# PKU-Alignment/omnisafe

Measured on AMD Instinct MI355X. Metric: env-steps/sec (rollout+update), PPO-Lag SafetyPointGoal1, higher is better.
Workload: dtype f32

## Files before the change

### include/omnisafe_amd.h

```cpp
#ifndef OMNISAFE_AMD_H
#define OMNISAFE_AMD_H

#include <stddef.h>
#include <stdint.h>

#ifdef __cplusplus
extern "C" {
#endif

#define OSA_OK 0
#define OSA_EINVAL (-1)
#define OSA_EHIP (-2)
#define OSA_EUNSUPPORTED (-3)

#define OSA_EST_GAE 0
#define OSA_EST_GAE_RTG 1
#define OSA_EST_PLAIN 2
#define OSA_EST_VTRACE 3

const char* osa_strerror(int code);
int osa_version(void);
const char* osa_build_arch(void);
const char* osa_abi_digest(void);


int osa_buffer_store_step(int t, int N, int obs_dim, int act_dim,
                          const float* obs, int ld_obs_src, const float* act, int ld_act_src,
                          const float* reward, const float* cost, const float* value_r,
                          const float* value_c, const float* logp,
                          float* buf_obs, int ld_obs_buf, float* buf_act, int ld_act_buf,
                          float* buf_reward, float* buf_cost, float* buf_value_r, float* buf_value_c,
                          float* buf_logp, void* stream);

int osa_gae_scan(const float* reward, const float* cost, const float* value_r, const float* value_c,
                 const uint8_t* path_end, const float* boot_r, const float* boot_c, int T, int N,
                 double gamma, double lam, double lam_c, float penalty_coef, int estimator,
                 float* adv_r, float* adv_c, float* target_value_r, float* target_value_c,
                 float* discounted_ret, void* stream);

int osa_gae_scan_tiled(const float* reward, const float* cost, const float* value_r, const float* value_c,
                       const uint8_t* path_end, const float* boot_r, const float* boot_c, int T, int N,
                       double gamma, double lam, double lam_c, float penalty_coef, int estimator,
                       float* adv_r, float* adv_c, float* target_value_r, float* target_value_c,
                       float* discounted_ret, void* stream);
size_t osa_gae_chained_ws_doubles(int T, int N);
int osa_gae_chained_timed_out(const double* ws, int T, int N, int* out);
int osa_gae_scan_chained(const float* reward, const float* cost, const float* value_r, const float* value_c,
                         const uint8_t* path_end, const float* boot_r, const float* boot_c, int T, int N,
                         double gamma, double lam, double lam_c, float penalty_coef, int estimator,
                         float* adv_r, float* adv_c, float* target_value_r, float* target_value_c,
                         float* discounted_ret, double* ws, void* stream);

size_t osa_reduce_ws_bytes(void);
int osa_adv_stats_phase1(const float* adv_r, const float* adv_c, long M, double* ws, double* stats,
                         void* stream);
int osa_adv_stats_phase2(const float* adv_r, long M, double* ws, double* stats, void* stream);

int osa_buffer_get(int T, int N, int obs_dim, int act_dim,
                   const float* obs, int ld_obs, const float* act, int ld_act, const float* logp,
                   const float* target_value_r, const float* target_value_c, const float* adv_r,
                   const float* adv_c, const float* discounted_ret, double* stats,
                   int standardize_r, int standardize_c,
                   float* out_obs, int ld_out_obs, float* out_act, int ld_out_act, float* out_logp,
                   float* out_target_value_r, float* out_target_value_c, float* out_adv_r,
                   float* out_adv_c, float* out_discounted_ret, void* stream);


int osa_mlp_layout(int obs_dim, int act_dim, int hidden, int* out12);

int osa_policy_step(int obs_dim, int act_dim, int hidden, const float* params, const float* obs,
                    int ld_obs, int N, const float* eps, unsigned long long seed,
                    unsigned long long offset, const unsigned long long* offset_base, int deterministic,
                    int nets_mask, float* act, int ld_act, float* value_r, float* value_c, float* logp,
                    float* mean_out, int ld_mean, void* stream);

int osa_policy_step_scaled(int obs_dim, int act_dim, int hidden, const float* params, const float* obs,
                           int ld_obs, int N, const float* eps, unsigned long long seed,
                           unsigned long long offset, const unsigned long long* offset_base, int deterministic,
                           int nets_mask, float* act, int ld_act, float* value_r, float* value_c, float* logp,
                           float* mean_out, int ld_mean, float* act_env, int ld_env, const float* old_min,
                           const float* old_max, float min_action, float max_action, void* stream);

typedef struct osa_ppo_hparams {
  float clip;
  float entropy_coef;
  float critic_norm_coef;
  float max_grad_norm;
  float lr_actor;
  float lr_critic;
  float beta1, beta2, adam_eps;
  int use_critic_norm;
  int use_max_grad_norm;
  int use_cost;
  const float* lr_device;
} osa_ppo_hparams;

size_t osa_minibatch_ws_floats(int obs_dim, int act_dim, int hidden, int max_blocks);
int osa_ppo_minibatch(int obs_dim, int act_dim, int hidden, float* params, float* adam_m,
                      float* adam_v, int* adam_step, float* grads, const float* obs, int ld_obs,
                      const float* act, int ld_act, const float* logp, const float* target_value_r,
                      const float* target_value_c, const float* adv_r, const float* adv_c,
                      const long* idx, int B, const float* lagrange, const osa_ppo_hparams* hp,
                      int loss_kind, int mode, int nets_mask, int max_blocks, float* ws,
                      float* step_stats, void* stream);

typedef struct osa_surrogate_ext {
  const float* old_mean;
  int ld_old_mean;
  const float* old_log_std;
  float kl_coef;
  float kl_mask_eta;
  float ratio_scale;
  float cost_kappa;
  float cost_excess;
} osa_surrogate_ext;
int osa_ppo_minibatch_ext(int obs_dim, int act_dim, int hidden, float* params, float* adam_m,
                          float* adam_v, int* adam_step, float* grads, const float* obs, int ld_obs,
                          const float* act, int ld_act, const float* logp,
                          const float* target_value_r, const float* target_value_c,
                          const float* adv_r, const float* adv_c, const long* idx, int B,
                          const float* lagrange, const osa_ppo_hparams* hp, int loss_kind, int mode,
                          int nets_mask, int max_blocks, float* ws, float* step_stats,
                          const osa_surrogate_ext* ext, void* stream);

int osa_ppo_pass_supported(int obs_dim, int act_dim, int hidden);
int osa_ppo_pass(int obs_dim, int act_dim, int hidden, float* params, float* adam_m, float* adam_v,
                 int* adam_step, const float* obs, int ld_obs, const float* act, int ld_act,
                 const float* logp, const float* target_value_r, const float* target_value_c,
                 const float* adv_r, const float* adv_c, const long* perm, long M, int B,
                 const float* lagrange, const osa_ppo_hparams* hp, int loss_kind, int nets_mask,
                 float* step_stats, void* stream);
int osa_ppo_wide_pass_supported(int obs_dim, int act_dim, int hidden);
size_t osa_ppo_wide_pass_ws_floats(int obs_dim, int act_dim, int hidden);
int osa_ppo_wide_pass(int obs_dim, int act_dim, int hidden, float* params, float* adam_m, float* adam_v,
                      int* adam_step, const float* obs, int ld_obs, const float* act, int ld_act,
                      const float* logp, const float* target_value_r, const float* target_value_c,
                      const float* adv_r, const float* adv_c, const long* perm, long M, int B,
                      const float* lagrange, const osa_ppo_hparams* hp, int loss_kind, int nets_mask,
                      float* ws, float* step_stats, void* stream);
int osa_ppo_split_pass_supported(int obs_dim, int act_dim, int hidden);
size_t osa_ppo_split_pass_xch_floats(int obs_dim, int act_dim, int hidden);
int osa_ppo_split_pass(int obs_dim, int act_dim, int hidden, float* params, float* adam_m, float* adam_v,
                       int* adam_step, const float* obs, int ld_obs, const float* act, int ld_act,
                       const float* logp, const float* target_value_r, const float* target_value_c,
                       const float* adv_r, const float* adv_c, const long* perm, long M, int B,
                       const float* lagrange, const osa_ppo_hparams* hp, int loss_kind, int nets_mask,
                       float* xch, int local, float* step_stats, void* stream);
int osa_ppo_split_pass_timed_out(const float* xch, int* out);
int osa_ppo_split_pass_clear_flag(float* xch);
size_t osa_ppo_split_dp_xch_floats(int obs_dim, int act_dim, int hidden, int world);
size_t osa_ppo_split_dp_dpx_floats(int obs_dim, int act_dim, int hidden, int world);
int osa_ppo_split_dp_pass(int obs_dim, int act_dim, int hidden, float* params, float* adam_m, float* adam_v,
                          int* adam_step, const float* obs, int ld_obs, const float* act, int ld_act,
                          const float* logp, const float* target_value_r, const float* target_value_c,
                          const float* adv_r, const float* adv_c, const long* perm, long M, int B, int world,
                          const float* lagrange, const osa_ppo_hparams* hp, int loss_kind, int nets_mask,
                          float* xch, float* dpx, int place, float* step_stats, void* stream);
int osa_ppo_pass_ext(int obs_dim, int act_dim, int hidden, float* params, float* adam_m, float* adam_v,
                 int* adam_step, const float* obs, int ld_obs, const float* act, int ld_act,
                 const float* logp, const float* target_value_r, const float* target_value_c,
                 const float* adv_r, const float* adv_c, const long* perm, long M, int B,
                 const float* lagrange, const osa_ppo_hparams* hp, int loss_kind, int nets_mask,
                 float* step_stats, const osa_surrogate_ext* ext, void* stream);
typedef struct osa_pass_member {
  float* params;
  float* adam_m;
  float* adam_v;
  int* adam_step;
  const float* obs;
  int ld_obs;
  const float* act;
  int ld_act;
  const float* logp;
  const float* target_value_r;
  const float* target_value_c;
  const float* adv_r;
  const float* adv_c;
  const long* perm;
  long M;
  int B;
  const float* lagrange;
  osa_ppo_hparams hp;
  int loss_kind;
  int nets_mask;
  float* step_stats;
  int has_ext;
  osa_surrogate_ext ext;
} osa_pass_member;
size_t osa_ppo_pass_group_ws_bytes(int n);
int osa_ppo_pass_group(int obs_dim, int act_dim, int hidden, const osa_pass_member* members, int n, void* workspace,
                       size_t workspace_bytes, void* stream);

size_t osa_ppo_dp_ws_floats(int obs_dim, int act_dim, int hidden, int world);
int osa_ppo_dp_step(int obs_dim, int act_dim, int hidden, float* params, float* adam_m, float* adam_v,
                    int* adam_step, const float* obs, int ld_obs, const float* act, int ld_act,
                    const float* logp, const float* target_value_r, const float* target_value_c,
                    const float* adv_r, const float* adv_c, const long* perm, long M, int B, int world,
                    int step_index, const float* lagrange, const osa_ppo_hparams* hp,
                    const float* lr_dev, int loss_kind, int nets_mask, float* slabs,
                    float* step_stats, void* stream);
int osa_ppo_dp_end_pass(int* adam_step, int nets_mask, int nsteps, void* stream);
int osa_ppo_dp_step_phase(int obs_dim, int act_dim, int hidden, float* params, float* adam_m, float* adam_v,
                          int* adam_step, const float* obs, int ld_obs, const float* act, int ld_act,
                          const float* logp, const float* target_value_r, const float* target_value_c,
                          const float* adv_r, const float* adv_c, const long* perm, long M, int B, int world,
                          int step_index, const float* lagrange, const osa_ppo_hparams* hp,
                          const float* lr_dev, int loss_kind, int nets_mask, float* slabs,
                          float* step_stats, int phase, void* stream);

int osa_dp_exchange_alloc(size_t floats, float** out);
int osa_dp_exchange_free(float* p);
size_t osa_ppo_dp_pass_ws_floats(int obs_dim, int act_dim, int hidden, int world);
int osa_ppo_dp_pass(int obs_dim, int act_dim, int hidden, float* params, float* adam_m, float* adam_v,
                    int* adam_step, const float* obs, int ld_obs, const float* act, int ld_act,
                    const float* logp, const float* target_value_r, const float* target_value_c,
                    const float* adv_r, const float* adv_c, const long* perm, long M, int B, int world,
                    const float* lagrange, const osa_ppo_hparams* hp, int loss_kind, int nets_mask,
                    float* exchange, int* sync, float* step_stats, void* stream);
int osa_ppo_dp_pass_placed(int obs_dim, int act_dim, int hidden, float* params, float* adam_m, float* adam_v,
                    int* adam_step, const float* obs, int ld_obs, const float* act, int ld_act,
                    const float* logp, const float* target_value_r, const float* target_value_c,
                    const float* adv_r, const float* adv_c, const long* perm, long M, int B, int world,
                    const float* lagrange, const osa_ppo_hparams* hp, int loss_kind, int nets_mask,
                    float* exchange, int* sync, int local, float* step_stats, void* stream);

size_t osa_p2p_exchange_floats(int obs_dim, int act_dim, int hidden, int world);
int osa_p2p_exchange_alloc(size_t floats, float** out, void* ipc_handle64);
int osa_p2p_exchange_open(const void* ipc_handle64, float** out);
int osa_p2p_exchange_release(float* p);
int osa_p2p_exchange_timed_out(const float* own, int* flag);
int osa_ppo_p2p_pass(int obs_dim, int act_dim, int hidden, float* params, float* adam_m, float* adam_v,
                     int* adam_step, const float* obs, int ld_obs, const float* act, int ld_act,
                     const float* logp, const float* target_value_r, const float* target_value_c,
                     const float* adv_r, const float* adv_c, const long* perm, long M, int B, int world, int rank,
                     float* const* peers, unsigned seq0, double timeout_s, const float* lagrange,
                     const osa_ppo_hparams* hp, int loss_kind, int nets_mask, float* step_stats, void* stream);

int osa_ppo_chunked_pass(int obs_dim, int act_dim, int hidden, float* params, float* adam_m, float* adam_v,
                         int* adam_step, const float* obs, int ld_obs, const float* act, int ld_act,
                         const float* logp, const float* target_value_r, const float* target_value_c,
                         const float* adv_r, const float* adv_c, const long* perm, long M, int B,
                         const float* lagrange, const osa_ppo_hparams* hp, int loss_kind, int nets_mask,
                         float* exchange, int* sync, int local, float* step_stats, void* stream);
size_t osa_ppo_dp_chunked_pass_ws_floats(int obs_dim, int act_dim, int hidden, int B, int world);
int osa_ppo_dp_chunked_pass(int obs_dim, int act_dim, int hidden, float* params, float* adam_m, float* adam_v,
                            int* adam_step, const float* obs, int ld_obs, const float* act, int ld_act,
                            const float* logp, const float* target_value_r, const float* target_value_c,
                            const float* adv_r, const float* adv_c, const long* perm, long M, int B, int world,
                            const float* lagrange, const osa_ppo_hparams* hp, int loss_kind, int nets_mask,
                            float* exchange, int* sync, int local, float* step_stats, void* stream);

int osa_debug_set_clock_buffer(long long* dev_ptr);
int osa_debug_set_pass_clock_buffer(long long* dev_ptr);
int osa_debug_set_part_clock_buffer(long long* dev_ptr);

#define OSA_GMLP_MAX_LAYERS 8
typedef struct osa_gmlp_desc {
  int obs_dim, act_dim;
  int n_layers[3];
  int width[3][OSA_GMLP_MAX_LAYERS];
  int activation[3];
} osa_gmlp_desc;
int osa_gmlp_layout(const osa_gmlp_desc* desc, int* out);
size_t osa_gmlp_ws_floats(const osa_gmlp_desc* desc, long rows);
int osa_gmlp_policy_step(const osa_gmlp_desc* desc, const float* params, const float* obs, int ld_obs, long N,
                         const float* eps, unsigned long long seed, unsigned long long offset,
                         const unsigned long long* offset_base, int deterministic, int nets_mask, float* act,
                         int ld_act, float* value_r, float* value_c, float* logp, float* mean_out, int ld_mean,
                         float* act_env, int ld_env, const float* old_min, const float* old_max, float min_action,
                         float max_action, float* ws, size_t ws_floats, void* stream);
int osa_gmlp_minibatch(const osa_gmlp_desc* desc, float* params, float* adam_m, float* adam_v, int* adam_step,
                       float* grads, const float* obs, int ld_obs, const float* act, int ld_act, const float* logp,
                       const float* target_value_r, const float* target_value_c, const float* adv_r,
                       const float* adv_c, const long* idx, long B, const float* lagrange, const osa_ppo_hparams* hp,
                       int loss_kind, int mode, int nets_mask, const float* vec, float fvp_scale, float* ws,
                       size_t ws_floats, float* step_stats, void* stream);
int osa_gmlp_minibatch_ext(const osa_gmlp_desc* desc, float* params, float* adam_m, float* adam_v, int* adam_step,
                           float* grads, const float* obs, int ld_obs, const float* act, int ld_act, const float* logp,
                           const float* target_value_r, const float* target_value_c, const float* adv_r,
                           const float* adv_c, const long* idx, long B, const float* lagrange,
                           const osa_ppo_hparams* hp, int loss_kind, int mode, int nets_mask, const float* vec,
                           float fvp_scale, float* ws, size_t ws_floats, float* step_stats,
                           const osa_surrogate_ext* ext, void* stream);
int osa_gmlp_adam_apply(const osa_gmlp_desc* desc, float* params, float* adam_m, float* adam_v, int* adam_step,
                        float* grads, const osa_ppo_hparams* hp, int nets_mask, float* fin8x3, void* stream);
int osa_gmlp_actor_stats(const osa_gmlp_desc* desc, const float* actor_params, const float* obs, int ld_obs, long M,
                         const float* old_mean, int ld_old, const float* old_log_std, int kind, int reduce_mode,
                         const float* act, int ld_act, const float* logp, const float* adv_r, const float* adv_c,
                         const float* lagrange, float* mean_out, int ld_mean, float* ws, size_t ws_floats, float* out,
                         void* stream);

int osa_adam_apply(int obs_dim, int act_dim, int hidden, float* params, float* adam_m, float* adam_v,
                   int* adam_step, float* grads, const osa_ppo_hparams* hp, int nets_mask,
                   void* stream);

int osa_actor_kl(int obs_dim, int act_dim, int hidden, const float* actor_params, const float* obs,
                 int ld_obs, long M, const float* old_mean, int ld_old, const float* old_log_std,
                 int reduce_mode, float* mean_out, int ld_mean, double* ws, float* kl_out,
                 void* stream);


size_t osa_normalizer_ws_doubles(int N, int D);
int osa_normalizer_push(const float* x, int ld, int N, int D, const uint8_t* mask, float* mean,
                        float* sumsq, float* var, float* std_, long* count, double* ws,
                        void* stream);

int osa_normalizer_apply(const float* x, int ld_x, float* y, int ld_y, int N, int D,
                         const uint8_t* mask, const float* mean, const float* std_, const long* count,
                         float clip, void* stream);

int osa_action_scale(const float* act, int ld_act, float* out, int ld_out, int N, int act_dim,
                     const float* old_min, const float* old_max, float min_action, float max_action,
                     void* stream);

int osa_rollout_post_step(int N, int epoch_end, const float* reward, const float* cost,
                          const uint8_t* terminated, const uint8_t* truncated, const float* vnext_r,
// ... 80 lines not shown
```

### omnisafe_amd/_lib.py

```python
from __future__ import annotations

import ctypes as C
import os

import torch

from . import build as _build

_LIB = None
OSA_OK, OSA_EUNSUPPORTED = 0, -3

c_f32p = C.c_void_p
c_ptr = C.c_void_p

_I, _L, _F, _D, _P, _U = C.c_int, C.c_long, C.c_float, C.c_double, C.c_void_p, C.c_ulonglong
SIGNATURES: dict[str, tuple] = {
    'osa_strerror': (C.c_char_p, [_I]),
    'osa_version': (_I, []),
    'osa_build_arch': (C.c_char_p, []),
    'osa_abi_digest': (C.c_char_p, []),
    'osa_buffer_store_step': (_I, [_I, _I, _I, _I, _P, _I, _P, _I, _P, _P, _P, _P, _P, _P, _I, _P, _I,
                                   _P, _P, _P, _P, _P, _P]),
    'osa_gae_scan': (_I, [_P, _P, _P, _P, _P, _P, _P, _I, _I, _D, _D, _D, _F, _I, _P, _P, _P, _P, _P, _P]),
    'osa_gae_scan_tiled': (_I, [_P, _P, _P, _P, _P, _P, _P, _I, _I, _D, _D, _D, _F, _I, _P, _P, _P, _P, _P, _P]),
    'osa_gae_chained_ws_doubles': (C.c_size_t, [_I, _I]),
    'osa_gae_chained_timed_out': (_I, [_P, _I, _I, _P]),
    'osa_gae_scan_chained': (_I, [_P, _P, _P, _P, _P, _P, _P, _I, _I, _D, _D, _D, _F, _I, _P, _P, _P, _P, _P, _P, _P]),
    'osa_reduce_ws_bytes': (C.c_size_t, []),
    'osa_adv_stats_phase1': (_I, [_P, _P, _L, _P, _P, _P]),
    'osa_adv_stats_phase2': (_I, [_P, _L, _P, _P, _P]),
    'osa_buffer_get': (_I, [_I, _I, _I, _I, _P, _I, _P, _I, _P, _P, _P, _P, _P, _P, _P, _I, _I,
                            _P, _I, _P, _I, _P, _P, _P, _P, _P, _P, _P]),
    'osa_mlp_layout': (_I, [_I, _I, _I, _P]),
    'osa_policy_step': (_I, [_I, _I, _I, _P, _P, _I, _I, _P, _U, _U, _P, _I, _I, _P, _I, _P, _P, _P, _P, _I,
                             _P]),
    'osa_policy_step_scaled': (_I, [_I, _I, _I, _P, _P, _I, _I, _P, _U, _U, _P, _I, _I, _P, _I, _P, _P, _P, _P, _I,
                                    _P, _I, _P, _P, _F, _F, _P]),
    'osa_minibatch_ws_floats': (C.c_size_t, [_I, _I, _I, _I]),
    'osa_gmlp_layout': (_I, [_P, _P]),
    'osa_gmlp_ws_floats': (C.c_size_t, [_P, _L]),
    'osa_gmlp_policy_step': (_I, [_P, _P, _P, _I, _L, _P, _U, _U, _P, _I, _I, _P, _I, _P, _P, _P, _P, _I, _P, _I, _P,
                                  _P, _F, _F, _P, C.c_size_t, _P]),
    'osa_gmlp_minibatch': (_I, [_P, _P, _P, _P, _P, _P, _P, _I, _P, _I, _P, _P, _P, _P, _P, _P, _L, _P, _P, _I, _I,
                                _I, _P, _F, _P, C.c_size_t, _P, _P]),
    'osa_gmlp_minibatch_ext': (_I, [_P, _P, _P, _P, _P, _P, _P, _I, _P, _I, _P, _P, _P, _P, _P, _P, _L, _P, _P, _I, _I,
                                    _I, _P, _F, _P, C.c_size_t, _P, _P, _P]),
    'osa_gmlp_adam_apply': (_I, [_P, _P, _P, _P, _P, _P, _P, _I, _P, _P]),
    'osa_gmlp_actor_stats': (_I, [_P, _P, _P, _I, _L, _P, _I, _P, _I, _I, _P, _I, _P, _P, _P, _P, _P, _I, _P,
                                  C.c_size_t, _P, _P]),
    'osa_ppo_minibatch': (_I, [_I, _I, _I, _P, _P, _P, _P, _P, _P, _I, _P, _I, _P, _P, _P, _P, _P, _P,
                               _I, _P, _P, _I, _I, _I, _I, _P, _P, _P]),
    'osa_ppo_minibatch_ext': (_I, [_I, _I, _I, _P, _P, _P, _P, _P, _P, _I, _P, _I, _P, _P, _P, _P, _P, _P,
                                   _I, _P, _P, _I, _I, _I, _I, _P, _P, _P, _P]),
    'osa_episode_flush_ws_doubles': (C.c_size_t, [_L]),
    'osa_episode_flush': (_I, [_P, _P, _P, _P, _P, _L, _P, _P, _P, _P, _P, _P, _P, _P]),
    'osa_gather_mean': (_I, [_P, _P, _L, _P, _P]),
    'osa_saute_step': (_I, [_I, _P, _P, _P, _P, _P, _P, _F, _F, _P, _P, _P, _I, _P, _I, _I, _P, _P, _P]),
    'osa_debug_set_clock_buffer': (_I, [_P]),
    'osa_debug_set_pass_clock_buffer': (_I, [_P]),
    'osa_debug_set_part_clock_buffer': (_I, [_P]),
    'osa_ppo_pass_supported': (_I, [_I, _I, _I]),
    'osa_ppo_dp_end_pass': (_I, [_P, _I, _I, _P]),
    'osa_ppo_dp_ws_floats': (C.c_size_t, [_I, _I, _I, _I]),
    'osa_ppo_dp_pass_ws_floats': (C.c_size_t, [_I, _I, _I, _I]),
    'osa_shuffle_rows': (_I, [_P, _I, _L, _P, _P]),
    'osa_dp_exchange_alloc': (_I, [C.c_size_t, C.POINTER(C.c_void_p)]),
    'osa_dp_exchange_free': (_I, [_P]),
    'osa_ppo_dp_pass': (_I, [_I, _I, _I, _P, _P, _P, _P, _P, _I, _P, _I, _P, _P, _P, _P, _P, _P, _L, _I, _I,
                        _P, _P, _I, _I, _P, _P, _P, _P]),
    'osa_ppo_dp_pass_placed': (_I, [_I, _I, _I, _P, _P, _P, _P, _P, _I, _P, _I, _P, _P, _P, _P, _P, _P, _L, _I, _I,
                               _P, _P, _I, _I, _P, _P, _I, _P, _P]),
    'osa_ppo_chunked_pass': (_I, [_I, _I, _I, _P, _P, _P, _P, _P, _I, _P, _I, _P, _P, _P, _P, _P, _P, _L, _I,
                                  _P, _P, _I, _I, _P, _P, _I, _P, _P]),
    'osa_ppo_dp_chunked_pass_ws_floats': (C.c_size_t, [_I, _I, _I, _I, _I]),
    'osa_ppo_dp_chunked_pass': (_I, [_I, _I, _I, _P, _P, _P, _P, _P, _I, _P, _I, _P, _P, _P, _P, _P, _P, _L, _I, _I,
                                     _P, _P, _I, _I, _P, _P, _I, _P, _P]),
    'osa_p2p_exchange_floats': (C.c_size_t, [_I, _I, _I, _I]),
    'osa_p2p_exchange_alloc': (_I, [C.c_size_t, C.POINTER(C.c_void_p), _P]),
    'osa_p2p_exchange_open': (_I, [_P, C.POINTER(C.c_void_p)]),
    'osa_p2p_exchange_release': (_I, [_P]),
    'osa_p2p_exchange_timed_out': (_I, [_P, _P]),
    'osa_ppo_p2p_pass': (_I, [_I, _I, _I, _P, _P, _P, _P, _P, _I, _P, _I, _P, _P, _P, _P, _P, _P, _L, _I, _I, _I,
                              _P, C.c_uint, _D, _P, _P, _I, _I, _P, _P]),
    'osa_ppo_dp_step': (_I, [_I, _I, _I, _P, _P, _P, _P, _P, _I, _P, _I, _P, _P, _P, _P, _P, _P, _L, _I, _I,
                             _I, _P, _P, _P, _I, _I, _P, _P, _P]),
    'osa_ppo_dp_step_phase': (_I, [_I, _I, _I, _P, _P, _P, _P, _P, _I, _P, _I, _P, _P, _P, _P, _P, _P, _L, _I, _I, _I, _P, _P, _P, _I, _I, _P, _P, _I, _P]),
    'osa_ppo_pass': (_I, [_I, _I, _I, _P, _P, _P, _P, _P, _I, _P, _I, _P, _P, _P, _P, _P, _P, _L, _I,
                          _P, _P, _I, _I, _P, _P]),
    'osa_ppo_wide_pass_supported': (_I, [_I, _I, _I]),
    'osa_ppo_wide_pass_ws_floats': (C.c_size_t, [_I, _I, _I]),
    'osa_ppo_wide_pass': (_I, [_I, _I, _I, _P, _P, _P, _P, _P, _I, _P, _I, _P, _P, _P, _P, _P, _P, _L, _I,
                               _P, _P, _I, _I, _P, _P, _P]),
    'osa_ppo_split_pass_supported': (_I, [_I, _I, _I]),
    'osa_ppo_split_pass_xch_floats': (C.c_size_t, [_I, _I, _I]),
    'osa_ppo_split_pass': (_I, [_I, _I, _I, _P, _P, _P, _P, _P, _I, _P, _I, _P, _P, _P, _P, _P, _P, _L, _I,
                                _P, _P, _I, _I, _P, _I, _P, _P]),
    'osa_ppo_split_pass_timed_out': (_I, [_P, _P]),
    'osa_ppo_split_pass_clear_flag': (_I, [_P]),
    'osa_ppo_split_dp_xch_floats': (C.c_size_t, [_I, _I, _I, _I]),
    'osa_ppo_split_dp_dpx_floats': (C.c_size_t, [_I, _I, _I, _I]),
    'osa_ppo_split_dp_pass': (_I, [_I, _I, _I, _P, _P, _P, _P, _P, _I, _P, _I, _P, _P, _P, _P, _P, _P, _L, _I, _I,
                                   _P, _P, _I, _I, _P, _P, _I, _P, _P]),
    'osa_ppo_pass_ext': (_I, [_I, _I, _I, _P, _P, _P, _P, _P, _I, _P, _I, _P, _P, _P, _P, _P, _P, _L, _I,
                              _P, _P, _I, _I, _P, _P, _P]),
    'osa_ppo_pass_group_ws_bytes': (C.c_size_t, [_I]),
    'osa_ppo_pass_group': (_I, [_I, _I, _I, _P, _I, _P, C.c_size_t, _P]),
    'osa_adam_apply': (_I, [_I, _I, _I, _P, _P, _P, _P, _P, _P, _I, _P]),
    'osa_actor_fvp_raw': (_I, [_I, _I, _I, _P, _P, _P, _I, _L, _P, _I, _P, _P, _P]),
    'osa_fvp_finish': (_I, [_I, _P, _P, _F, _I, _I, _F, _P, _P]),
    'osa_cg_init': (_I, [_I, _P, _P, _P, _P, _P, _P]),
    'osa_cg_step': (_I, [_I, _P, _P, _P, _P, _P, _F, _F, _P]),
    'osa_vec_lincomb': (_I, [_I, _F, _P, _F, _P, _P, _P]),
    'osa_vec_dot': (_I, [_I, _P, _P, _P, _P]),
    'osa_actor_eval': (_I, [_I, _I, _I, _P, _P, _I, _L, _P, _I, _P, _P, _P, _P, _P, _I, _P, _P, _P, _P]),
    'osa_actor_kl': (_I, [_I, _I, _I, _P, _P, _I, _L, _P, _I, _P, _I, _P, _I, _P, _P, _P]),
    'osa_normalizer_ws_doubles': (C.c_size_t, [_I, _I]),
    'osa_normalizer_push': (_I, [_P, _I, _I, _I, _P, _P, _P, _P, _P, _P, _P, _P]),
    'osa_normalizer_apply': (_I, [_P, _I, _P, _I, _I, _I, _P, _P, _P, _P, _F, _P]),
    'osa_action_scale': (_I, [_P, _I, _P, _I, _I, _I, _P, _P, _F, _F, _P]),
    'osa_rollout_post_step': (_I, [_I, _I] + [_P] * 21),
    'osa_synth_env_step': (_I, [_U, _U, _P, _I, _I, _I, _F, _P, _P, _I, _P, _P, _P, _P, _P, _I, _I, _P]),
    'osa_reach_env_step': (_I, [_U, _U, _P, _I, _I, _I, _P, _P, _P, _I, _P, _I, _P, _P, _P, _P, _P, _I, _I, _P]),
    'osa_nav_env_step': (_I, [_U, _U, _P, _I, _I, _I, _I, _P, _P, _P, _I, _P, _I, _P, _P, _P, _P, _P, _I, _I, _P]),
    'osa_eval_episodes': (_I, [_I, _I, _I, _I, _I, _P, _P, _P, _P, _F, _P, _P, _F, _F, _U, _I, _F, _I, _I, _F, _F,
                               _I, _D, _D, _P, _P, _P, _P, _P]),
    'osa_eval_trace_floats': (_I, [_I, _I, _I, _I]),
}


class OsaError(RuntimeError):
    pass


def lib_path() -> str:
    return os.environ.get('OSA_LIB_PATH') or _build.LIB_PATH


def load(require_gpu: bool = False):
    global _LIB
    if _LIB is None:
        path = lib_path()
        own = path == _build.LIB_PATH

        def build(force: bool) -> None:
            try:
                _build.build_library(force=force, verbose=False)
            except Exception as exc:
                raise OsaError(
                    f'libomnisafe_amd.so is missing or stale and could not be built ({exc}); '
                    'run `python -m omnisafe_amd.build` -- there is no CPU fallback') from exc

        def digest(lib) -> str:
            try:
                lib.osa_abi_digest.restype = C.c_char_p
                return lib.osa_abi_digest().decode()
            except AttributeError:
                return 'none'

        if own and not os.path.exists(path):
            build(False)
        lib = C.CDLL(path)
        if own:
            want = _build.source_digest()
            if digest(lib) != want:
                import _ctypes

                _ctypes.dlclose(lib._handle)
                build(True)
                lib = C.CDLL(path)
                if digest(lib) != want:
                    raise OsaError(f'{path} was built from other sources (digest {digest(lib)}, expected '
                                   f'{want}); run `python -m omnisafe_amd.build --force`')
        for name, (res, args) in SIGNATURES.items():
            fn = getattr(lib, name)
            fn.restype = res
            fn.argtypes = args
        _LIB = lib
    if require_gpu and not torch.cuda.is_available():
        raise OsaError('omnisafe_amd needs an AMD GPU visible to torch (ROCm); there is no CPU fallback')
    return _LIB


def check(code: int, what: str = '') -> None:
    if code != 0:
        msg = load().osa_strerror(code).decode()
        raise OsaError(f'{what or "libomnisafe_amd"} failed: {msg} ({code})')


def ptr(t: torch.Tensor | None) -> int | None:
    if t is None:
        return None
    assert t.is_cuda, 'omnisafe_amd kernels take device tensors'
    return t.data_ptr()


_RAW_STREAM = getattr(torch._C, '_cuda_getCurrentRawStream', None)


def stream_ptr() -> int:
    if _RAW_STREAM is not None:
        return _RAW_STREAM(torch.cuda.current_device())
    return torch.cuda.current_stream().cuda_stream
```

### omnisafe_amd/csrc/buffer_kernels.hip

```cpp
#include "osa_common.h"

__global__ __launch_bounds__(256) void osa_store_step_kernel(
    int N, int obs_dim, int act_dim, const float* __restrict__ obs, int ld_os,
    const float* __restrict__ act, int ld_as, const float* __restrict__ reward,
    const float* __restrict__ cost, const float* __restrict__ value_r,
    const float* __restrict__ value_c, const float* __restrict__ logp, float* __restrict__ b_obs,
    int ld_ob, float* __restrict__ b_act, int ld_ab, float* __restrict__ b_reward,
    float* __restrict__ b_cost, float* __restrict__ b_value_r, float* __restrict__ b_value_c,
    float* __restrict__ b_logp) {
  const long gid = (long)blockIdx.x * blockDim.x + threadIdx.x;
  const long n_obs = (long)N * obs_dim, n_act = (long)N * act_dim;
  if (gid < n_obs) {
    const int n = (int)(gid / obs_dim), d = (int)(gid % obs_dim);
    b_obs[(long)n * ld_ob + d] = obs[(long)n * ld_os + d];
  }
  if (gid < n_act) {
    const int n = (int)(gid / act_dim), d = (int)(gid % act_dim);
    b_act[(long)n * ld_ab + d] = act[(long)n * ld_as + d];
  }
  if (gid < N) {
    b_reward[gid] = reward[gid];
    b_cost[gid] = cost[gid];
    b_value_r[gid] = value_r[gid];
    b_value_c[gid] = value_c[gid];
// ... 598 lines not shown
  __shared__ double red[17];
  double sa = 0.0, sb = 0.0;
  const long stride = (long)gridDim.x * blockDim.x;
  for (long i = (long)blockIdx.x * blockDim.x + threadIdx.x; i < M; i += stride) {
    sa += (double)a[i];
    sb += (double)b[i];
  }
  sa = osa_block_sum<OSA_RED_THREADS>(sa, red);
  sb = osa_block_sum<OSA_RED_THREADS>(sb, red);
  if (threadIdx.x == 0) {
    ws[2 * blockIdx.x] = sa;
    ws[2 * blockIdx.x + 1] = sb;
  }
}

__global__ __launch_bounds__(OSA_RED_THREADS) void osa_sum2_final_kernel(
    const double* __restrict__ ws, int nblk, long M, double* __restrict__ stats) {
  __shared__ double red[17];
  double sa = 0.0, sb = 0.0;
  for (int i = threadIdx.x; i < nblk; i += OSA_RED_THREADS) {
    sa += ws[2 * i];
    sb += ws[2 * i + 1];
  }
  sa = osa_block_sum<OSA_RED_THREADS>(sa, red);
  sb = osa_block_sum<OSA_RED_THREADS>(sb, red);
  if (threadIdx.x == 0) {
    stats[0] = sa;
    stats[1] = sb;
    stats[2] = (double)M;
  }
}

__global__ __launch_bounds__(OSA_RED_THREADS) void osa_sumsq_partial_kernel(
    const float* __restrict__ a, long M, const double* __restrict__ stats,
    double* __restrict__ ws) {
#pragma clang fp contract(off)
  __shared__ double red[17];
  const float mean = (float)stats[0] / (float)stats[2];
  double s = 0.0;
  const long stride = (long)gridDim.x * blockDim.x;
  for (long i = (long)blockIdx.x * blockDim.x + threadIdx.x; i < M; i += stride) {
    const float d = a[i] - mean;
    const float q = d * d;
    s += (double)q;
  }
  s = osa_block_sum<OSA_RED_THREADS>(s, red);
  if (threadIdx.x == 0) ws[blockIdx.x] = s;
}

__global__ __launch_bounds__(OSA_RED_THREADS) void osa_sumsq_final_kernel(
    const double* __restrict__ ws, int nblk, double* __restrict__ stats) {
  __shared__ double red[17];
  double s = 0.0;
  for (int i = threadIdx.x; i < nblk; i += OSA_RED_THREADS) s += ws[i];
  s = osa_block_sum<OSA_RED_THREADS>(s, red);
  if (threadIdx.x == 0) {
    stats[3] = s;
    stats[4] = (double)((float)stats[0] / (float)stats[2]);
    stats[5] = (double)((float)stats[1] / (float)stats[2]);
  }
}

struct OsaGetScalars {
  const float* src[6];
  float* dst[6];
  int op[6];
};

__global__ __launch_bounds__(256) void osa_get_scalars_kernel(OsaGetScalars p, int T, int N,
                                                              double* __restrict__ stats) {
#pragma clang fp contract(off)
  __shared__ float tile[64][65];
  const int n0 = blockIdx.x * 64, t0 = blockIdx.y * 64;
  const int tx = threadIdx.x & 63, ty = threadIdx.x >> 6;
  const float mean_r = (float)stats[4], mean_c = (float)stats[5];
  const float std_r = sqrtf((float)stats[3] / (float)stats[2]);
  if (blockIdx.x == 0 && blockIdx.y == 0 && threadIdx.x == 0) stats[6] = (double)std_r;
  const float denom = std_r + 1e-8f;
  float pre[6][16];
#pragma unroll
  for (int k = 0; k < 6; ++k) {
    const bool have = p.src[k] != nullptr && p.dst[k] != nullptr;
    const float* __restrict__ src = have ? p.src[k] : reinterpret_cast<const float*>(stats);
#pragma unroll
    for (int u = 0; u < 16; ++u) {
      const int t = t0 + ty + 4 * u, n = n0 + tx;
      const bool ok = have && t < T && n < N;
      pre[k][u] = src[ok ? (long)t * N + n : 0];
    }
  }
#pragma unroll
  for (int k = 0; k < 6; ++k) {
    const float* __restrict__ src = p.src[k];
    float* __restrict__ dst = p.dst[k];
    if (src == nullptr || dst == nullptr) continue;
    const int op = p.op[k];
    __syncthreads();
#pragma unroll
    for (int u = 0; u < 16; ++u) {
      const int tt = ty + 4 * u;
      const int t = t0 + tt, n = n0 + tx;
      if (t < T && n < N) {
        float v = pre[k][u];
        if (op == 1) v = (v - mean_r) / denom;
        else if (op == 2) v = v - mean_c;
        tile[tt][tx] = v;
      }
    }
    __syncthreads();
    for (int nn = ty; nn < 64; nn += 4) {
      const int n = n0 + nn, t = t0 + tx;
      if (t < T && n < N) dst[(long)n * T + t] = tile[tx][nn];
    }
  }
}

__global__ __launch_bounds__(256) void osa_get_rows_kernel(const float* __restrict__ src, int ld_src,
                                                           float* __restrict__ dst, int ld_dst,
                                                           int T, int N, int dim) {
  const long gid = (long)blockIdx.x * blockDim.x + threadIdx.x;
  const long total = (long)T * N * dim;
  if (gid >= total) return;
  const long row = gid / dim;
  const int d = (int)(gid - row * dim);
  const int n = (int)(row / T), t = (int)(row - (long)n * T);
  dst[row * ld_dst + d] = src[((long)t * N + n) * ld_src + d];
}

__global__ __launch_bounds__(256) void osa_get_rows_vec4_kernel(const float* __restrict__ src, int ld_src,
                                                                float* __restrict__ dst, int ld_dst,
                                                                unsigned T, unsigned N, unsigned dim4,
                                                                unsigned total4) {
  const unsigned gid = blockIdx.x * 256u + threadIdx.x;
  if (gid >= total4) return;
  const unsigned row = gid / dim4, q = gid - row * dim4;
  const unsigned n = row / T, t = row - n * T;
  const float4 v = *reinterpret_cast<const float4*>(src + ((size_t)t * N + n) * ld_src + 4 * q);
  *reinterpret_cast<float4*>(dst + (size_t)row * ld_dst + 4 * q) = v;
}

static void osa_launch_get_rows(const float* src, int ld_src, float* dst, int ld_dst, int T, int N, int dim,
                                hipStream_t st) {
  const long total = (long)T * N * dim;
  const bool vec = dim % 4 == 0 && ld_src % 4 == 0 && ld_dst % 4 == 0 && total / 4 < 2147483647L &&
                   (reinterpret_cast<uintptr_t>(src) & 15) == 0 && (reinterpret_cast<uintptr_t>(dst) & 15) == 0;
  if (vec) {
    const unsigned total4 = (unsigned)(total / 4);
    hipLaunchKernelGGL(osa_get_rows_vec4_kernel, dim3((total4 + 255) / 256), dim3(256), 0, st, src, ld_src, dst,
                       ld_dst, (unsigned)T, (unsigned)N, (unsigned)(dim / 4), total4);
  } else {
    hipLaunchKernelGGL(osa_get_rows_kernel, dim3((unsigned)((total + 255) / 256)), dim3(256), 0, st, src, ld_src,
                       dst, ld_dst, T, N, dim);
  }
}

extern "C" {

const char* osa_strerror(int code) {
  switch (code) {
    case OSA_OK: return "ok";
    case OSA_EINVAL: return "invalid argument";
    case OSA_EHIP: return "HIP runtime error";
    case OSA_EUNSUPPORTED: return "not implemented in libomnisafe_amd";
    default: return "unknown error";
  }
}
int osa_version(void) { return 1; }
const char* osa_build_arch(void) { return "gfx950"; }

int osa_buffer_store_step(int t, int N, int obs_dim, int act_dim, const float* obs, int ld_obs_src,
                          const float* act, int ld_act_src, const float* reward, const float* cost,
                          const float* value_r, const float* value_c, const float* logp,
                          float* buf_obs, int ld_obs_buf, float* buf_act, int ld_act_buf,
                          float* buf_reward, float* buf_cost, float* buf_value_r, float* buf_value_c,
                          float* buf_logp, void* stream) {
  OSA_REQUIRE(t >= 0 && N > 0 && obs_dim > 0 && act_dim > 0);
  OSA_REQUIRE(obs && act && reward && cost && value_r && value_c && logp);
  OSA_REQUIRE(buf_obs && buf_act && buf_reward && buf_cost && buf_value_r && buf_value_c && buf_logp);
  OSA_REQUIRE(ld_obs_src >= obs_dim && ld_obs_buf >= obs_dim && ld_act_src >= act_dim &&
              ld_act_buf >= act_dim);
  const long row = (long)t * N;
  const long work = (long)N * (obs_dim > act_dim ? obs_dim : act_dim);
  const int blocks = (int)((work + 255) / 256);
  hipLaunchKernelGGL(osa_store_step_kernel, dim3(blocks), dim3(256), 0, osa_stream(stream), N,
                     obs_dim, act_dim, obs, ld_obs_src, act, ld_act_src, reward, cost, value_r,
                     value_c, logp, buf_obs + row * ld_obs_buf, ld_obs_buf,
                     buf_act + row * ld_act_buf, ld_act_buf, buf_reward + row, buf_cost + row,
                     buf_value_r + row, buf_value_c + row, buf_logp + row);
  OSA_CHECK_LAUNCH();
  return OSA_OK;
}

int osa_gae_scan(const float* reward, const float* cost, const float* value_r, const float* value_c,
                 const uint8_t* path_end, const float* boot_r, const float* boot_c, int T, int N,
                 double gamma, double lam, double lam_c, float penalty_coef, int estimator,
                 float* adv_r, float* adv_c, float* target_value_r, float* target_value_c,
                 float* discounted_ret, void* stream) {
  OSA_REQUIRE(T > 0 && N > 0);
  OSA_REQUIRE(reward && cost && value_r && value_c && path_end && boot_r && boot_c);
  OSA_REQUIRE(adv_r && adv_c && target_value_r && target_value_c && discounted_ret);
  if (estimator < OSA_EST_GAE || estimator > OSA_EST_VTRACE) return OSA_EUNSUPPORTED;
  const float g32 = (float)gamma;
  const double d_g = gamma, d_r = gamma * lam, d_c = gamma * lam_c;
  const int threads = N >= 256 ? 256 : 64;
  const int blocks = (N + threads - 1) / threads;
  constexpr int U = 8;
#define OSA_GAE_LAUNCH(E)                                                                         \
  hipLaunchKernelGGL((osa_gae_scan_kernel<E, U>), dim3(blocks), dim3(threads), 0,                 \
                     osa_stream(stream), reward, cost, value_r, value_c, path_end, boot_r, boot_c, \
                     T, N, g32, d_g, d_r, d_c, penalty_coef, adv_r, adv_c, target_value_r,        \
                     target_value_c, discounted_ret)
  if (estimator == OSA_EST_GAE) OSA_GAE_LAUNCH(OSA_EST_GAE);
  else if (estimator == OSA_EST_GAE_RTG) OSA_GAE_LAUNCH(OSA_EST_GAE_RTG);
  else if (estimator == OSA_EST_PLAIN) OSA_GAE_LAUNCH(OSA_EST_PLAIN);
  else OSA_GAE_LAUNCH(OSA_EST_VTRACE);
#undef OSA_GAE_LAUNCH
  OSA_CHECK_LAUNCH();
  return OSA_OK;
}

int osa_gae_scan_tiled(const float* reward, const float* cost, const float* value_r, const float* value_c,
                       const uint8_t* path_end, const float* boot_r, const float* boot_c, int T, int N,
                       double gamma, double lam, double lam_c, float penalty_coef, int estimator,
                       float* adv_r, float* adv_c, float* target_value_r, float* target_value_c,
                       float* discounted_ret, void* stream) {
  OSA_REQUIRE(T > 0 && N > 0);
  OSA_REQUIRE(reward && cost && value_r && value_c && path_end && boot_r && boot_c);
  OSA_REQUIRE(adv_r && adv_c && target_value_r && target_value_c && discounted_ret);
  if (estimator < OSA_EST_GAE || estimator > OSA_EST_PLAIN) return OSA_EUNSUPPORTED;
  const float g32 = (float)gamma;
  const double d_g = gamma, d_r = gamma * lam, d_c = gamma * lam_c;
  constexpr int NB = 16;
  const int blocks = (N + NB - 1) / NB;
  int cus = 256, dev = 0;
  if (hipGetDevice(&dev) == hipSuccess) (void)hipDeviceGetAttribute(&cus, hipDeviceAttributeMultiprocessorCount, dev);
  bool wide_wg = blocks <= 2 * cus;
  if (const char* e = getenv("OSA_GAE_TILE_WAVES")) wide_wg = e[0] == '1';
#define OSA_GAE_TILE_LAUNCH(E)                                                                            \
  do {                                                                                                    \
    if (wide_wg)                                                                                          \
      hipLaunchKernelGGL((osa_gae_tile_scan_kernel<E, NB, 16>), dim3(blocks), dim3(1024), 0,              \
                         osa_stream(stream), reward, cost, value_r, value_c, path_end, boot_r, boot_c, T, \
                         N, g32, d_g, d_r, d_c, penalty_coef, adv_r, adv_c, target_value_r,               \
                         target_value_c, discounted_ret);                                                 \
    else                                                                                                  \
      hipLaunchKernelGGL((osa_gae_tile_scan_kernel<E, NB, 4>), dim3(blocks), dim3(256), 0,                \
                         osa_stream(stream), reward, cost, value_r, value_c, path_end, boot_r, boot_c, T, \
                         N, g32, d_g, d_r, d_c, penalty_coef, adv_r, adv_c, target_value_r,               \
                         target_value_c, discounted_ret);                                                 \
  } while (0)
  if (estimator == OSA_EST_GAE) OSA_GAE_TILE_LAUNCH(OSA_EST_GAE);
  else if (estimator == OSA_EST_GAE_RTG) OSA_GAE_TILE_LAUNCH(OSA_EST_GAE_RTG);
  else OSA_GAE_TILE_LAUNCH(OSA_EST_PLAIN);
#undef OSA_GAE_TILE_LAUNCH
  OSA_CHECK_LAUNCH();
  return OSA_OK;
}

size_t osa_gae_chained_ws_doubles(int T, int N) {
  if (T < 1 || N < 1) return 0;
  return (size_t)((T + OSA_GC_LEV - 1) / OSA_GC_LEV) * 10 * (size_t)N + 2;
}

int osa_gae_chained_timed_out(const double* ws, int T, int N, int* out) {
  OSA_REQUIRE(ws && out && T > 0 && N > 0);
  const size_t nws = osa_gae_chained_ws_doubles(T, N);
  return hipMemcpy(out, ws + (nws - 1), sizeof(int), hipMemcpyDeviceToHost) == hipSuccess ? OSA_OK : OSA_EHIP;
}

int osa_gae_scan_chained(const float* reward, const float* cost, const float* value_r, const float* value_c,
                         const uint8_t* path_end, const float* boot_r, const float* boot_c, int T, int N,
                         double gamma, double lam, double lam_c, float penalty_coef, int estimator,
                         float* adv_r, float* adv_c, float* target_value_r, float* target_value_c,
                         float* discounted_ret, double* ws, void* stream) {
  OSA_REQUIRE(T > 0 && N > 0 && ws);
  OSA_REQUIRE(reward && cost && value_r && value_c && path_end && boot_r && boot_c);
  OSA_REQUIRE(adv_r && adv_c && target_value_r && target_value_c && discounted_ret);
  if (estimator < OSA_EST_GAE || estimator > OSA_EST_PLAIN) return OSA_EUNSUPPORTED;
  const float g32 = (float)gamma;
  const double d_g = gamma, d_r = gamma * lam, d_c = gamma * lam_c;
  const int nlev = (T + OSA_GC_LEV - 1) / OSA_GC_LEV, nenvb = (N + 63) / 64;
  if ((long)nlev * nenvb > 2147483647L) return OSA_EUNSUPPORTED;
  hipStream_t st = osa_stream(stream);
  const size_t nws = osa_gae_chained_ws_doubles(T, N);
  if (hipMemsetAsync(ws, 0xFF, (nws - 2) * sizeof(double), st) != hipSuccess) return OSA_EHIP;
  unsigned int* ticket = reinterpret_cast<unsigned int*>(ws + (nws - 2));
  if (hipMemsetAsync(ticket, 0, sizeof(double), st) != hipSuccess) return OSA_EHIP;
#define OSA_GAE_CHAIN_LAUNCH(E)                                                                             \
  hipLaunchKernelGGL((osa_gae_chain_scan_kernel<E>), dim3(nlev * nenvb), dim3(64 * OSA_GC_NW), 0, st, reward, \
                     cost, value_r, value_c, path_end, boot_r, boot_c, T, N, g32, d_g, d_r, d_c, penalty_coef, \
                     adv_r, adv_c, target_value_r, target_value_c, discounted_ret, ws, nenvb, ticket)
  if (estimator == OSA_EST_GAE) OSA_GAE_CHAIN_LAUNCH(OSA_EST_GAE);
  else if (estimator == OSA_EST_GAE_RTG) OSA_GAE_CHAIN_LAUNCH(OSA_EST_GAE_RTG);
  else OSA_GAE_CHAIN_LAUNCH(OSA_EST_PLAIN);
#undef OSA_GAE_CHAIN_LAUNCH
  OSA_CHECK_LAUNCH();
  return OSA_OK;
}

size_t osa_reduce_ws_bytes(void) { return (size_t)OSA_RED_BLOCKS * 2 * sizeof(double); }

static int osa_red_blocks(long M) {
  long b = (M + (long)OSA_RED_THREADS * 4 - 1) / ((long)OSA_RED_THREADS * 4);
  if (b < 1) b = 1;
  if (b > OSA_RED_BLOCKS) b = OSA_RED_BLOCKS;
  return (int)b;
}

int osa_adv_stats_phase1(const float* adv_r, const float* adv_c, long M, double* ws, double* stats,
                         void* stream) {
  OSA_REQUIRE(adv_r && adv_c && ws && stats && M > 0);
  const int nblk = osa_red_blocks(M);
  hipLaunchKernelGGL(osa_sum2_partial_kernel, dim3(nblk), dim3(OSA_RED_THREADS), 0,
                     osa_stream(stream), adv_r, adv_c, M, ws);
  hipLaunchKernelGGL(osa_sum2_final_kernel, dim3(1), dim3(OSA_RED_THREADS), 0, osa_stream(stream),
                     ws, nblk, M, stats);
  OSA_CHECK_LAUNCH();
  return OSA_OK;
}

int osa_adv_stats_phase2(const float* adv_r, long M, double* ws, double* stats, void* stream) {
  OSA_REQUIRE(adv_r && ws && stats && M > 0);
  const int nblk = osa_red_blocks(M);
  hipLaunchKernelGGL(osa_sumsq_partial_kernel, dim3(nblk), dim3(OSA_RED_THREADS), 0,
                     osa_stream(stream), adv_r, M, stats, ws);
  hipLaunchKernelGGL(osa_sumsq_final_kernel, dim3(1), dim3(OSA_RED_THREADS), 0, osa_stream(stream),
                     ws, nblk, stats);
  OSA_CHECK_LAUNCH();
  return OSA_OK;
}

int osa_buffer_get(int T, int N, int obs_dim, int act_dim, const float* obs, int ld_obs,
                   const float* act, int ld_act, const float* logp, const float* target_value_r,
                   const float* target_value_c, const float* adv_r, const float* adv_c,
                   const float* discounted_ret, double* stats, int standardize_r, int standardize_c,
                   float* out_obs, int ld_out_obs, float* out_act, int ld_out_act, float* out_logp,
                   float* out_target_value_r, float* out_target_value_c, float* out_adv_r,
                   float* out_adv_c, float* out_discounted_ret, void* stream) {
  OSA_REQUIRE(T > 0 && N > 0 && stats);
  OsaGetScalars p;
  const float* srcs[6] = {logp, target_value_r, target_value_c, adv_r, adv_c, discounted_ret};
  float* dsts[6] = {out_logp, out_target_value_r, out_target_value_c, out_adv_r, out_adv_c,
                    out_discounted_ret};
  const int ops[6] = {0, 0, 0, standardize_r ? 1 : 0, standardize_c ? 2 : 0, 0};
  for (int k = 0; k < 6; ++k) {
    p.src[k] = srcs[k];
    p.dst[k] = dsts[k];
    p.op[k] = ops[k];
  }
  hipLaunchKernelGGL(osa_get_scalars_kernel, dim3((N + 63) / 64, (T + 63) / 64), dim3(256), 0,
                     osa_stream(stream), p, T, N, stats);
  if (obs && out_obs) {
    OSA_REQUIRE(obs_dim > 0 && ld_obs >= obs_dim && ld_out_obs >= obs_dim);
    osa_launch_get_rows(obs, ld_obs, out_obs, ld_out_obs, T, N, obs_dim, osa_stream(stream));
  }
  if (act && out_act) {
    OSA_REQUIRE(act_dim > 0 && ld_act >= act_dim && ld_out_act >= act_dim);
    osa_launch_get_rows(act, ld_act, out_act, ld_out_act, T, N, act_dim, osa_stream(stream));
  }
  OSA_CHECK_LAUNCH();
  return OSA_OK;
}

}
```

### omnisafe_amd/csrc/ppo_pass_body.h

```cpp
#pragma once
#include "mlp_device.h"

#ifndef OSA_PART_MARK
#define OSA_PART_MARK(k) do { } while (0)
#endif

#ifndef PSLD
#define PSLD 68
#endif
#define PSPAD (PSLD - 64)
#define PNSTAT 16

struct OsaPassArgs {
  OsaNet nd;
  float* params;
  float* adam_m;
  float* adam_v;
  int* adam_step;
  const float* obs;
  int ld_obs;
  const float* act;
  int ld_act;
  const float* logp;
  const float* tgt_r;
  const float* tgt_c;
  const float* adv_r;
  const float* adv_c;
  const long* perm;
  long M;
  int B;
  int nmb;
  const float* lagrange;
  OsaPassHp hp;
  int loss_kind;
  int nets_mask;
  float* stats;
  float* dp_slabs;
  int dp_world;
  int mb0;
  int* dp_sync;
  int part_stride;
  int part_tpw;
  const float* old_mean;
  int ld_old_mean;
  const float* old_log_std;
  float ext_kl_coef, ext_mask_eta, ext_ratio_scale, ext_cost_kappa, ext_cost_excess;
  int dp_uncached;
  int dp_local;
  int dp_chunk;
  int dp_ranks;
  int one_xcc;
  long long* dbg;
  float* p2p_peer[16];
  int p2p_rank;
  unsigned p2p_seq0;
  long long p2p_timeout;
  int p2p_fence;
};
#define OSA_P2P_HDR 256
#define OSA_P2P_STICKY 240

#ifdef OSA_PASS_CLOCKS
#define PTICK(k)                                      \
  do {                                                \
    if (a.dbg && tid == 0) {                          \
      const long long now_ = clock64();               \
      dbg_acc[k] += now_ - dbg_last;                  \
      dbg_last = now_;                                \
    }                                                 \
  } while (0)
#else
#define PTICK(k) do { } while (0)
#endif

__device__ __forceinline__ f32x4 osa_sym_sum(f32x4 a, float sa, f32x4 b, float sb) {
#pragma clang fp contract(off)
  const f32x4 pa = a * sa;
  const f32x4 pb = b * sb;
  return pa + pb;
}
__device__ __forceinline__ float osa_sym_sum1(float a, float sa, float b, float sb) {
#pragma clang fp contract(off)
  const float pa = a * sa;
  const float pb = b * sb;
  return pa + pb;
}

__device__ __forceinline__ void osa_store_sys(f32x4* p, f32x4 v) {
  asm volatile("global_store_dwordx4 %0, %1, off sc0 sc1" : : "v"(p), "v"(v) : "memory");
}
__device__ __forceinline__ void osa_store_sys(float* p, float v) {
  asm volatile("global_store_dword %0, %1, off sc0 sc1" : : "v"(p), "v"(v) : "memory");
}

__host__ __device__ constexpr int osa_pass_lds_floats(int KB, int OT) {
  return 64 * (16 * KB + PSPAD) + 64 * PSLD + 16 * OT * PSLD + 2 * 64 + 2 * 16 * OT + 4 * 64 * PSLD + 16 * KB * PSLD +
         2 * 16 * OT * PSLD + 64;
}
#ifndef OSA_PASS_W2T
#define OSA_PASS_W2T 1
#endif
__host__ __device__ constexpr bool osa_pass_has_w2t(int KB, int OT) {
  return OSA_PASS_W2T != 0 && (osa_pass_lds_floats(KB, OT) + 64 * PSLD) * 4 <= 160 * 1024;
}

template <int KB, int OT, bool MULTI, bool COOP, bool EXT, bool HIER, bool DPS, bool SO, bool P2P = false>
__device__ __forceinline__ void osa_ppo_pass_body(const OsaPassArgs& a, const int net, const int rk, const int pc0 = 0,
                                                  const int pn = 0) {
  static_assert(!P2P || (COOP && !HIER && !DPS && !EXT), "P2P is a form of the cooperative pass");
  extern __shared__ __attribute__((aligned(16))) float smem[];
  const OsaNet& nd = a.nd;
  constexpr bool coop = COOP;
#ifdef OSA_BODY_PART_ONLY
  constexpr bool dp = true, part = true, contig = true;
#else
  const bool dp = DPS && a.dp_slabs != nullptr && !coop;
  const bool part = DPS && MULTI && a.part_stride != 0;
  const bool contig = part && a.part_stride < 0;
#endif
  const bool chunked = COOP && a.dp_chunk != 0;
  const int nranks = (HIER && chunked && a.dp_ranks > 1) ? a.dp_ranks : 1;
  const int cw = chunked ? a.dp_world / nranks : 1;
  const int crank = chunked ? rk / cw : 0, cchunk = chunked ? rk - crank * cw : 0;
  const long roff = (part || P2P) ? 0 : (chunked ? (long)crank * a.M : (long)rk * a.M);
  const float* __restrict__ obs_p = a.obs + roff * a.ld_obs;
  const float* __restrict__ act_p = a.act + roff * a.ld_act;
  const float* __restrict__ logp_p = a.logp + roff;
  const float* __restrict__ advr_p = a.adv_r + roff;
  const float* __restrict__ advc_p = a.adv_c + roff;
  const long* __restrict__ perm_p = a.perm ? a.perm + roff : nullptr;
  constexpr int H = 64, HT = 4, OUTP = 16 * OT, INP = 16 * KB, W1LD = INP + PSPAD;
  float* sW1 = smem;
  float* sW2 = sW1 + H * W1LD;
  float* sW3 = sW2 + H * PSLD;
  float* sB1 = sW3 + OUTP * PSLD;
  float* sB2 = sB1 + H;
  float* sB3 = sB2 + H;
  float* sLS = sB3 + OUTP;
  float* sH1 = sLS + OUTP;
  float* sH2 = sH1 + H * PSLD;
  float* sZ1 = sH2 + H * PSLD;
  float* sZ2 = sZ1 + H * PSLD;
  float* sX = sZ2 + H * PSLD;
  float* sDO = sX + INP * PSLD;
  float* sDL = sDO + OUTP * PSLD;
  float* red = sDL + OUTP * PSLD;
  constexpr bool W2T = osa_pass_has_w2t(KB, OT);
  float* sW2T = red + 64;

#ifdef OSA_BODY_OPAQUE_TID
  int tid_ = threadIdx.x;
  asm volatile("" : "+v"(tid_));
  const int tid = tid_, lane = tid & 63, wave = tid >> 6, j = lane & 15, g = lane >> 4;
#else
  const int tid = threadIdx.x, lane = tid & 63, wave = tid >> 6, j = lane & 15, g = lane >> 4;
#endif
  const int i = j, cc = j;
  const int nchunk_all = MULTI ? (a.B + 63) / 64 : 1;
  const bool strided = part;
  const int cstride = part ? (contig ? 1 : a.part_stride) : 1;
  const int cfirst = part ? (contig ? pc0 : rk) : (chunked ? cchunk : 0);
  const int nchunk = strided ? (contig ? pn : (nchunk_all - cfirst + cstride - 1) / cstride) : nchunk_all;
  auto pos_ok = [&](long cidx) -> bool {
    const long mb = cidx / nchunk, ch = cfirst + (cidx - mb * nchunk) * cstride;
    const long inb = ch * 64 + 16 * wave + j;
    return (mb < a.mb0 + a.nmb) && (inb < a.B) && (mb * a.B + inb < a.M);
  };
  auto row_of = [&](long cidx) -> long {
    const long mb = cidx / nchunk, ch = cfirst + (cidx - mb * nchunk) * cstride;
    const long pc = pos_ok(cidx) ? mb * a.B + ch * 64 + 16 * wave + j : 0;
    return perm_p ? perm_p[pc] : pc;
  };
  const long cidx_first = (long)a.mb0 * nchunk;
  const long r0_first = row_of(cidx_first);
  const long r1_first = row_of(cidx_first + 1);
  const bool leader = tid == 192;
  const int P = nd.P;
  float* __restrict__ gp = a.params + (long)net * P;
  float* __restrict__ gm = a.adam_m + (long)net * P;
  float* __restrict__ gv = a.adam_v + (long)net * P;
  const bool critic = net != 0;
  const bool is_actor = !critic;
  const int out_dim = critic ? 1 : nd.act_dim;
  const bool small_out = SO || ((OT == 1) && out_dim <= 2);

#ifdef OSA_BODY_PART_ONLY
  constexpr bool VPRO = true;
#else
  constexpr bool VPRO = DPS;
#endif
  f32x4 w1v_[VPRO ? KB : 1], w2v_[VPRO ? 4 : 1], w3v_[VPRO ? OT : 1];
  float b1v_ = 0.f, b2v_ = 0.f, b3v_ = 0.f, lsv_ = 0.f;
  if constexpr (VPRO) {
#pragma unroll
    for (int q = 0; q < KB; ++q) w1v_[q] = *reinterpret_cast<const f32x4*>(gp + nd.oW1 + 4 * (tid + 256 * q));
#pragma unroll
    for (int q = 0; q < 4; ++q) w2v_[q] = *reinterpret_cast<const f32x4*>(gp + nd.oW2 + 4 * (tid + 256 * q));
#pragma unroll
    for (int q = 0; q < OT; ++q) w3v_[q] = *reinterpret_cast<const f32x4*>(gp + nd.oW3 + 4 * (tid + 256 * q));
    if (tid < H) {
      b1v_ = gp[nd.ob1 + tid];
      b2v_ = gp[nd.ob2 + tid];
    }
    if (tid < OUTP) {
      b3v_ = gp[nd.ob3 + tid];
      lsv_ = gp[nd.oLS + tid];
    }
  } else {
    for (int e = tid; e < H * INP; e += 256) sW1[(e / INP) * W1LD + (e % INP)] = gp[nd.oW1 + e];
    if (tid < H) {
      sB1[tid] = gp[nd.ob1 + tid];
      sB2[tid] = gp[nd.ob2 + tid];
    }
    if (tid < OUTP) {
      sB3[tid] = gp[nd.ob3 + tid];
      sLS[tid] = gp[nd.oLS + tid];
    }
  }
  OSA_PART_MARK(8);
  f32x4 m2[HT], v2[HT], m1[KB], v1[KB], m3[OT], v3[OT];
  float mb_ = 0.f, vb_ = 0.f;
  int boff = -1;
  float* sbias = sB1;
  if (tid < H) { boff = nd.ob1 + tid; sbias = sB1 + tid; }
  else if (tid < 2 * H) { boff = nd.ob2 + tid - H; sbias = sB2 + tid - H; }
  else if (tid < 2 * H + OUTP) { boff = nd.ob3 + tid - 2 * H; sbias = sB3 + tid - 2 * H; }
  else if (tid < 2 * H + 2 * OUTP) { boff = nd.oLS + tid - 2 * H - OUTP; sbias = sLS + tid - 2 * H - OUTP; }
  if (critic && boff >= nd.oLS) boff = -1;
#pragma unroll
  for (int ti = 0; ti < HT; ++ti)
#pragma unroll
    for (int r = 0; r < 4; ++r) {
      const int off = nd.oW2 + (16 * wave + 4 * g + r) * H + 16 * ti + cc;
      m2[ti][r] = dp ? 0.f : gm[off];
      v2[ti][r] = dp ? 0.f : gv[off];
    }
#pragma unroll
  for (int kb = 0; kb < KB; ++kb)
#pragma unroll
    for (int r = 0; r < 4; ++r) {
      const int off = nd.oW1 + (16 * wave + 4 * g + r) * INP + 16 * kb + cc;
      m1[kb][r] = dp ? 0.f : gm[off];
      v1[kb][r] = dp ? 0.f : gv[off];
    }
#pragma unroll
  for (int o = 0; o < OT; ++o)
#pragma unroll
    for (int r = 0; r < 4; ++r) {
      const int off = nd.oW3 + (16 * o + 4 * g + r) * H + 16 * wave + cc;
      m3[o][r] = dp ? 0.f : gm[off];
      v3[o][r] = dp ? 0.f : gv[off];
    }
  if (boff >= 0 && !dp) {
    mb_ = gm[boff];
    vb_ = gv[boff];
  }
  OSA_PART_MARK(9);
  const int step0 = dp ? 0 : a.adam_step[net];
  const float lr = critic ? a.hp.lr_critic : a.hp.lr_actor;
  const float beta1 = a.hp.beta1, beta2 = a.hp.beta2, aeps = a.hp.adam_eps;
  if (!dp) {
    for (int k = tid; k < a.nmb; k += 256) {
      const double t = (double)(step0 + k + 1);
      float* row = a.stats + (long)k * PNSTAT;
      row[10 + 2 * net] = (float)((double)lr / (1.0 - pow((double)beta1, t)));
      row[11 + 2 * net] = (float)(1.0 / sqrt(1.0 - pow((double)beta2, t)));
    }
  }
  const bool own_terms = !(chunked && cchunk != 0);
  const bool l2 = critic && a.hp.use_critic_norm && !part && own_terms;
  const float c2 = 2.f * a.hp.critic_norm_coef;
  float lam = 0.f;
  if (is_actor && a.lagrange) lam = *a.lagrange;
  const float inv_1p_lam = 1.f / (1.f + lam);
  constexpr bool vec_ok = true;
  const float* __restrict__ tgt = ((net == 1) ? a.tgt_r : a.tgt_c) + roff;

  struct Pre {
    f32x4 x[KB];
    float act[4 * OT];
    float logp, adv_r, adv_c, tgt;
    float old[EXT ? 4 * OT : 1];
    bool valid;
  };
  auto fetch_x = [&](long rr, Pre& q) {
    const float* xrow = obs_p + (int)rr * a.ld_obs;
#pragma unroll
    for (int kb = 0; kb < KB; ++kb) {
      const int col0 = 16 * kb + 4 * g;
      if (vec_ok) {
        const int cl = (col0 + 4 <= a.ld_obs) ? col0 : a.ld_obs - 4;
        q.x[kb] = *reinterpret_cast<const f32x4*>(xrow + cl);
      } else {
        const int last = nd.obs_dim - 1;
        q.x[kb].x = xrow[min(col0, last)];
        q.x[kb].y = xrow[min(col0 + 1, last)];
        q.x[kb].z = xrow[min(col0 + 2, last)];
        q.x[kb].w = xrow[min(col0 + 3, last)];
      }
    }
  };
  auto fetch_s = [&](long rr, Pre& q) {
    const int ri = (int)rr;
    if (is_actor) {
      const float* arow = act_p + ri * a.ld_act;
#pragma unroll
      for (int o = 0; o < OT; ++o)
#pragma unroll
        for (int r = 0; r < 4; ++r) q.act[4 * o + r] = arow[min(16 * o + 4 * g + r, nd.act_dim - 1)];
      q.logp = logp_p[ri];
      q.adv_r = advr_p[ri];
      q.adv_c = advc_p[ri];
      q.tgt = 0.f;
      if constexpr (EXT) {
        const float* orow = a.old_mean + roff * a.ld_old_mean + ri * a.ld_old_mean;
#pragma unroll
        for (int o = 0; o < OT; ++o)
#pragma unroll
          for (int r = 0; r < 4; ++r) q.old[4 * o + r] = orow[min(16 * o + 4 * g + r, nd.act_dim - 1)];
      }
    } else {
#pragma unroll
      for (int k = 0; k < 4 * OT; ++k) q.act[k] = 0.f;
      q.logp = q.adv_r = q.adv_c = 0.f;
      q.tgt = tgt[ri];
    }
  };
  bool cm[KB][4];
#pragma unroll
  for (int kb = 0; kb < KB; ++kb)
#pragma unroll
    for (int r = 0; r < 4; ++r) cm[kb][r] = (16 * kb + 4 * g + r) < nd.obs_dim;
  float dm[OT][4];
#pragma unroll
  for (int o = 0; o < OT; ++o)
#pragma unroll
    for (int r = 0; r < 4; ++r) dm[o][r] = (16 * o + 4 * g + r) < nd.act_dim ? 1.f : 0.f;
  OSA_PART_MARK(10);
  Pre cur;
  long cidx = cidx_first;
  {
    const long r0 = r0_first;
    fetch_x(r0, cur);
    fetch_s(r0, cur);
    cur.valid = pos_ok(cidx);
  }
  long row_nxt = r1_first;
  OSA_PART_MARK(11);
  if constexpr (VPRO) {
    if (tid < H) {
      sB1[tid] = b1v_;
      sB2[tid] = b2v_;
    }
    if (tid < OUTP) {
      sB3[tid] = b3v_;
      sLS[tid] = lsv_;
    }
#pragma unroll
    for (int q = 0; q < KB; ++q) {
      const int e4 = tid + 256 * q;
      *reinterpret_cast<f32x4*>(sW1 + (e4 / (INP / 4)) * W1LD + 4 * (e4 % (INP / 4))) = w1v_[q];
    }
#pragma unroll
    for (int q = 0; q < 4; ++q) {
      const int e4 = tid + 256 * q, row = e4 >> 4, c4 = e4 & 15;
      *reinterpret_cast<f32x4*>(sW2 + row * PSLD + 4 * c4) = w2v_[q];
      if constexpr (W2T) {
#pragma unroll
        for (int k = 0; k < 4; ++k) sW2T[(4 * c4 + k) * PSLD + row] = w2v_[q][k];
      }
    }
#pragma unroll
    for (int q = 0; q < OT; ++q) {
      const int e4 = tid + 256 * q;
      *reinterpret_cast<f32x4*>(sW3 + (e4 >> 4) * PSLD + 4 * (e4 & 15)) = w3v_[q];
    }
  } else {
    for (int e = tid; e < H * H; e += 256) sW2[(e >> 6) * PSLD + (e & 63)] = gp[nd.oW2 + e];
    if constexpr (W2T)
      for (int e = tid; e < H * H; e += 256) sW2T[(e & 63) * PSLD + (e >> 6)] = gp[nd.oW2 + e];
    for (int e = tid; e < OUTP * H; e += 256) sW3[(e >> 6) * PSLD + (e & 63)] = gp[nd.oW3 + e];
  }
  OSA_PART_MARK(12);
  __syncthreads();
  OSA_PART_MARK(4);
#ifdef OSA_PASS_CLOCKS
  long long dbg_acc[13] = {0, 0, 0, 0, 0, 0, 0, 0, 0, 0, 0, 0, 0};
  long long dbg_last = clock64();
#endif
  bool coop_dead = false;
  if constexpr (COOP) {
    if (a.dp_local) {
      if (threadIdx.x == 0) {
        const int xcc = __builtin_amdgcn_s_getreg(20 | (0 << 6) | (3 << 11)) & 7;
        __hip_atomic_fetch_or(a.dp_sync + 4 + net, 1 << xcc, __ATOMIC_RELAXED, __HIP_MEMORY_SCOPE_AGENT);
        const int expect = a.dp_world * __builtin_popcount(a.nets_mask & 7);
        int v = __hip_atomic_fetch_add(a.dp_sync + 7, 1, __ATOMIC_RELEASE, __HIP_MEMORY_SCOPE_AGENT) + 1;
        int spins = 0, why = 0;
        while (v < expect) {
          __builtin_amdgcn_s_sleep(1);
          v = __hip_atomic_load(a.dp_sync + 7, __ATOMIC_RELAXED, __HIP_MEMORY_SCOPE_AGENT);
          if (++spins > (1 << 21)) { why = 1; break; }
        }
        for (int n = 0; n < 3 && why == 0; ++n) {
          const int mask = __hip_atomic_load(a.dp_sync + 4 + n, __ATOMIC_ACQUIRE, __HIP_MEMORY_SCOPE_AGENT);
          if ((mask & (mask - 1)) != 0) why = 2;
        }
        if (why) __hip_atomic_store(a.dp_sync + 3, why, __ATOMIC_RELAXED, __HIP_MEMORY_SCOPE_AGENT);
        if (!why) why = __hip_atomic_load(a.dp_sync + 3, __ATOMIC_RELAXED, __HIP_MEMORY_SCOPE_AGENT);
        red[0] = (float)why;
      }
      __syncthreads();
      const bool bad_placement = red[0] != 0.f;
      __syncthreads();
      if (bad_placement) return;
    }
  }

  const float invB_full = 1.f / (float)a.B;
  for (int mb = a.mb0; mb < a.mb0 + a.nmb; ++mb) {
    const long mb_lo = (long)mb * a.B;
    const int Bcur = (int)(min(mb_lo + a.B, a.M) - mb_lo);
    float invB = invB_full;
    if (Bcur != a.B) invB = 1.f / (float)Bcur;
    f32x4 g2[HT], g1[KB], g3[OT];
#pragma unroll
    for (int ti = 0; ti < HT; ++ti) g2[ti] = (f32x4){0.f, 0.f, 0.f, 0.f};
#pragma unroll
    for (int kb = 0; kb < KB; ++kb) g1[kb] = (f32x4){0.f, 0.f, 0.f, 0.f};
#pragma unroll
    for (int o = 0; o < OT; ++o) g3[o] = (f32x4){0.f, 0.f, 0.f, 0.f};
    const float* __restrict__ bc_row = dp ? gp : a.stats + (long)(mb - a.mb0) * PNSTAT + 10 + 2 * net;
    const float step_size = bc_row[0], inv_bc2_sqrt = bc_row[1];
    float gb = 0.f, loss_part = 0.f, ratio_part = 0.f, ent_pre = 0.f;
    float cost_pen = 0.f;
    if (is_actor && leader) {
      for (int d = 0; d < nd.act_dim; ++d) ent_pre += 1.41893853320467274178f + sLS[d];
      ent_pre /= (float)nd.act_dim;
    }
    for (int ch = 0; ch < nchunk; ++ch, ++cidx) {
    PTICK(0);
    const bool valid = cur.valid;
    const int c = 16 * wave + j;
#define PUT_TILE(S, V, T)                                                           \
  _Pragma("unroll") for (int r_ = 0; r_ < 4; ++r_) (S)[(16 * (T) + 4 * g + r_) * PSLD + c] = (V)[r_]
#pragma unroll
    for (int r = 0; r < 4; ++r) cur.x[KB - 1][r] = cm[KB - 1][r] ? cur.x[KB - 1][r] : 0.f;
#pragma unroll
    for (int kb = 0; kb < KB; ++kb) PUT_TILE(sX, cur.x[kb], kb);
    f32x4 h1[HT], h2[HT], out[OT];
#pragma unroll
    for (int t = 0; t < HT; ++t) h1[t] = *reinterpret_cast<const f32x4*>(sB1 + 16 * t + 4 * g);
#pragma unroll
    for (int t = 0; t < HT; ++t) h2[t] = *reinterpret_cast<const f32x4*>(sB2 + 16 * t + 4 * g);
#pragma unroll
    for (int o = 0; o < OT; ++o) out[o] = *reinterpret_cast<const f32x4*>(sB3 + 16 * o + 4 * g);
#define OSA_SB() __builtin_amdgcn_sched_barrier(0)
    constexpr int NG1 = 2 * KB, NG = NG1 + 8 + 4;
    auto load_group = [&](int gi, f32x4 (&dst)[2]) {
      if (gi < NG1) {
        const int T0 = 2 * (gi / KB), kb = gi % KB;
        dst[0] = *reinterpret_cast<const f32x4*>(sW1 + (16 * T0 + i) * W1LD + 16 * kb + 4 * g);
        dst[1] = *reinterpret_cast<const f32x4*>(sW1 + (16 * (T0 + 1) + i) * W1LD + 16 * kb + 4 * g);
      } else if (gi < NG1 + 8) {
        const int q = gi - NG1, T0 = 2 * ((q >> 1) & 1), kb = 2 * (q >> 2) + (q & 1);
        dst[0] = *reinterpret_cast<const f32x4*>(sW2 + (16 * T0 + i) * PSLD + 16 * kb + 4 * g);
        dst[1] = *reinterpret_cast<const f32x4*>(sW2 + (16 * (T0 + 1) + i) * PSLD + 16 * kb + 4 * g);
      } else if (!small_out) {
        const int kb = gi - NG1 - 8;
#pragma unroll
        for (int o = 0; o < OT; ++o)
          dst[o] = *reinterpret_cast<const f32x4*>(sW3 + (16 * o + i) * PSLD + 16 * kb + 4 * g);
      }
    };
    auto mm_group = [&](int gi, const f32x4 (&w)[2]) {
      if (gi < NG1) {
        const int T0 = 2 * (gi / KB), kb = gi % KB;
#pragma unroll
        for (int s = 0; s < 4; ++s) {
          h1[T0] = OSA_MFMA(w[0][s], cur.x[kb][s], h1[T0]);
          h1[T0 + 1] = OSA_MFMA(w[1][s], cur.x[kb][s], h1[T0 + 1]);
        }
      } else if (gi < NG1 + 8) {
        const int q = gi - NG1, T0 = 2 * ((q >> 1) & 1), kb = 2 * (q >> 2) + (q & 1);
#pragma unroll
        for (int s = 0; s < 4; ++s) {
          h2[T0] = OSA_MFMA(w[0][s], h1[kb][s], h2[T0]);
          h2[T0 + 1] = OSA_MFMA(w[1][s], h1[kb][s], h2[T0 + 1]);
        }
      } else if (!small_out) {
        const int kb = gi - NG1 - 8;
#pragma unroll
        for (int o = 0; o < OT; ++o)
#pragma unroll
          for (int s = 0; s < 4; ++s) out[o] = OSA_MFMA(w[o][s], h2[kb][s], out[o]);
      }
    };
    f32x4 wq[2][2];
    load_group(0, wq[0]);
#pragma unroll
    for (int gi = 0; gi < NG; ++gi) {
      if (gi + 1 < NG) load_group(gi + 1, wq[(gi + 1) & 1]);
      OSA_SB();
      mm_group(gi, wq[gi & 1]);
      OSA_SB();
      if (gi == KB) {
        h1[0] = osa_tanh4(h1[0]);
        h1[1] = osa_tanh4(h1[1]);
      }
      if (gi == NG1 - 1) fetch_x(row_nxt, cur);
      if (gi == NG1 + 1) {
        PUT_TILE(sH1, h1[0], 0);
        PUT_TILE(sH1, h1[1], 1);
        h1[2] = osa_tanh4(h1[2]);
        h1[3] = osa_tanh4(h1[3]);
      }
      if (gi == NG1 + 6) {
        PUT_TILE(sH1, h1[2], 2);
        PUT_TILE(sH1, h1[3], 3);
        h2[0] = osa_tanh4(h2[0]);
        h2[1] = osa_tanh4(h2[1]);
      }
      if (gi == NG1 + 8) {
        PUT_TILE(sH2, h2[0], 0);
        PUT_TILE(sH2, h2[1], 1);
        h2[2] = osa_tanh4(h2[2]);
        h2[3] = osa_tanh4(h2[3]);
      }
    }
    PUT_TILE(sH2, h2[2], 2);
    PUT_TILE(sH2, h2[3], 3);
    if (small_out) {
      float p0 = 0.f, p1 = 0.f;
      f32x4 w0[HT], w1[HT];
#pragma unroll
      for (int t = 0; t < HT; ++t) {
        w0[t] = *reinterpret_cast<const f32x4*>(sW3 + 16 * t + 4 * g);
        w1[t] = *reinterpret_cast<const f32x4*>(sW3 + PSLD + 16 * t + 4 * g);
      }
      __builtin_amdgcn_sched_barrier(0);
#pragma unroll
      for (int t = 0; t < HT; ++t) {
#pragma unroll
        for (int r = 0; r < 4; ++r) {
          p0 = fmaf(w0[t][r], h2[t][r], p0);
          p1 = fmaf(w1[t][r], h2[t][r], p1);
        }
      }
      p0 = osa_sum_over_groups(p0);
      p1 = osa_sum_over_groups(p1);
      if (g == 0) {
        out[0][0] += p0;
        out[0][1] += p1;
      }
    }

    PTICK(1);
    f32x4 dO[OT], dLS[OT];
#pragma unroll
    for (int o = 0; o < OT; ++o) {
      dO[o] = (f32x4){0.f, 0.f, 0.f, 0.f};
      dLS[o] = (f32x4){0.f, 0.f, 0.f, 0.f};
    }
    if (is_actor) {
      float lp = 0.f;
      f32x4 zv[OT], ivar[OT];
#pragma unroll
      for (int o = 0; o < OT; ++o) {
        const f32x4 ls = *reinterpret_cast<const f32x4*>(sLS + 16 * o + 4 * g);
#pragma unroll
        for (int r = 0; r < 4; ++r) {
          const float dmr = dm[o][r];
          const float iv = __builtin_amdgcn_exp2f(ls[r] * -2.88539008177792681472f) * dmr;
          const float z = cur.act[4 * o + r] - out[o][r];
          zv[o][r] = z;
          ivar[o][r] = iv;
          lp += -0.5f * (z * z) * iv - ls[r] * dmr - 0.91893853320467274178f * dmr;
        }
      }
      lp = osa_sum_over_groups(lp);
      float kl = 0.f, mask = 1.f, mask_mean = 1.f, cost_w = 0.f;
      f32x4 dkl_mu[OT], dkl_ls[OT];
      if constexpr (EXT) {
#pragma unroll
        for (int o = 0; o < OT; ++o) {
          const f32x4 ls = *reinterpret_cast<const f32x4*>(sLS + 16 * o + 4 * g);
#pragma unroll
          for (int r = 0; r < 4; ++r) {
            const int d = min(16 * o + 4 * g + r, nd.act_dim - 1);
            const float ls0 = a.old_log_std[d], dl = ls[r] - ls0;
            const float q = __builtin_amdgcn_exp2f(dl * 1.44269504088896340736f), var_ratio = q * q;
            const float isd0 = __builtin_amdgcn_exp2f(ls0 * -1.44269504088896340736f);
            const float dmu = out[o][r] - cur.old[4 * o + r];
            const float u = dmu * isd0;
            kl += 0.5f * (var_ratio + u * u - 1.f - 2.f * dl) * dm[o][r];
            dkl_mu[o][r] = u * isd0 * dm[o][r];
            dkl_ls[o][r] = (var_ratio - 1.f) * dm[o][r];
          }
        }
        kl = osa_sum_over_groups(kl);
      }
      const float ratio = valid ? __builtin_amdgcn_exp2f((lp - cur.logp) * 1.44269504088896340736f) : 0.f;
      if constexpr (EXT) {
        if (a.ext_mask_eta >= 0.f || a.ext_cost_kappa > 0.f) {
          mask = (a.ext_mask_eta < 0.f || (valid && kl <= a.ext_mask_eta)) ? 1.f : 0.f;
          float pm = (valid && g == 0) ? mask : 0.f;
          float pc = (valid && g == 0) ? ratio * cur.adv_c : 0.f;
          pm = osa_wave_sum_dpp(pm);
          pc = osa_wave_sum_dpp(pc);
          __syncthreads();
          if (lane == 0) {
            red[4 * wave + 0] = pm;
            red[4 * wave + 1] = pc;
          }
          __syncthreads();
          const float tm = red[0] + red[4] + red[8] + red[12], tc = red[1] + red[5] + red[9] + red[13];
          if (a.ext_mask_eta >= 0.f) mask_mean = tm * invB;
          if (a.ext_cost_kappa > 0.f) {
            const float pen = tc * invB + a.ext_cost_excess;
            if (pen > 0.f) cost_w = a.ext_cost_kappa;
            cost_pen = a.ext_cost_kappa * fmaxf(pen, 0.f);
          }
          __syncthreads();
        }
      }
      {
        const float adv = (cur.adv_r - lam * cur.adv_c) * inv_1p_lam;
        float dratio, li;
        if (a.loss_kind == 0) {
          const float lo = 1.f - a.hp.clip, hi = 1.f + a.hp.clip;
          const float rc = fminf(fmaxf(ratio, lo), hi);
          const float s1 = ratio * adv, s2 = rc * adv;
          const bool inrange = ratio >= lo && ratio <= hi;
          li = -fminf(s1, s2);
          dratio = (s1 < s2 || inrange) ? -adv : 0.f;
        } else {
          li = -(ratio * adv);
          dratio = -adv;
        }
        float dklw = 0.f;
        if constexpr (EXT) {
          const float rs = a.ext_ratio_scale * mask_mean;
          li = li * rs + a.ext_kl_coef * kl * mask;
          dratio = dratio * rs + cost_w * cur.adv_c;
          dklw = valid ? a.ext_kl_coef * mask * invB : 0.f;
        }
        const float dlogp = valid ? dratio * ratio * invB : 0.f;
        if (g == 0 && valid) {
          loss_part += li;
          ratio_part += ratio;
        }
#pragma unroll
        for (int o = 0; o < OT; ++o) {
#pragma unroll
          for (int r = 0; r < 4; ++r) {
            const float z = zv[o][r], iv = ivar[o][r];
            dO[o][r] = dlogp * z * iv;
            dLS[o][r] = dlogp * (z * z * iv - dm[o][r]);
            if constexpr (EXT) {
              dO[o][r] += dklw * dkl_mu[o][r];
              dLS[o][r] += dklw * dkl_ls[o][r];
            }
          }
        }
      }
    } else if (valid) {
      const float diff = out[0][0] - cur.tgt;
      if (g == 0) {
        loss_part += diff * diff;
        dO[0][0] = 2.f * diff * invB;
      }
    }

    PTICK(2);
    fetch_s(row_nxt, cur);
    cur.valid = pos_ok(cidx + 1);
    row_nxt = row_of(cidx + 2);
#pragma unroll
    for (int o = 0; o < OT; ++o) {
      PUT_TILE(sDO, dO[o], o);
      PUT_TILE(sDL, dLS[o], o);
    }
    f32x4 z2[HT], z1[HT];
#pragma unroll
    for (int t = 0; t < HT; ++t) z2[t] = (f32x4){0.f, 0.f, 0.f, 0.f};
    float wt[2][4][HT];
    auto load_w2t = [&](int kb, float (&dst)[4][HT]) {
      if constexpr (W2T) {
#pragma unroll
        for (int t = 0; t < HT; ++t) {
          const f32x4 v = *reinterpret_cast<const f32x4*>(sW2T + (16 * t + i) * PSLD + 16 * kb + 4 * g);
#pragma unroll
          for (int s = 0; s < 4; ++s) dst[s][t] = v[s];
        }
      } else {
#pragma unroll
        for (int s = 0; s < 4; ++s)
#pragma unroll
          for (int t = 0; t < HT; ++t) dst[s][t] = sW2[(16 * kb + 4 * g + s) * PSLD + 16 * t + i];
      }
    };
    if (small_out) {
      const float d0 = __shfl(dO[0][0], j, 64), d1 = __shfl(dO[0][1], j, 64);
      load_w2t(0, wt[0]);
#pragma unroll
      for (int t = 0; t < HT; ++t) {
        const f32x4 w0 = *reinterpret_cast<const f32x4*>(sW3 + 16 * t + 4 * g);
        const f32x4 w1 = *reinterpret_cast<const f32x4*>(sW3 + PSLD + 16 * t + 4 * g);
        z2[t] = w0 * d0 + w1 * d1;
      }
    } else {
      float w3t[OT][4][HT];
#pragma unroll
      for (int o = 0; o < OT; ++o)
#pragma unroll
        for (int s = 0; s < 4; ++s)
#pragma unroll
          for (int t = 0; t < HT; ++t) w3t[o][s][t] = sW3[(16 * o + 4 * g + s) * PSLD + 16 * t + i];
      load_w2t(0, wt[0]);
      __builtin_amdgcn_sched_barrier(0);
#pragma unroll
      for (int o = 0; o < OT; ++o)
#pragma unroll
        for (int s = 0; s < 4; ++s)
#pragma unroll
          for (int t = 0; t < HT; ++t) z2[t] = OSA_MFMA(w3t[o][s][t], dO[o][s], z2[t]);
    }
#pragma unroll
    for (int t = 0; t < HT; ++t) {
      z2[t] = z2[t] * (1.f - h2[t] * h2[t]);
      PUT_TILE(sZ2, z2[t], t);
    }
#pragma unroll
    for (int t = 0; t < HT; ++t) z1[t] = (f32x4){0.f, 0.f, 0.f, 0.f};
#pragma unroll
    for (int kb = 0; kb < HT; ++kb) {
      if (kb + 1 < HT) load_w2t(kb + 1, wt[(kb + 1) & 1]);
      __builtin_amdgcn_sched_barrier(0);
#pragma unroll
      for (int s = 0; s < 4; ++s)
#pragma unroll
        for (int t = 0; t < HT; ++t) z1[t] = OSA_MFMA(wt[kb & 1][s][t], z2[kb][s], z1[t]);
      __builtin_amdgcn_sched_barrier(0);
    }
#pragma unroll
    for (int t = 0; t < HT; ++t) {
      z1[t] = z1[t] * (1.f - h1[t] * h1[t]);
      PUT_TILE(sZ1, z1[t], t);
    }
#undef PUT_TILE
    PTICK(3);
    __syncthreads();
    PTICK(4);
    {
      f32x4 a2[4], a1[4];
#pragma unroll
      for (int sb = 0; sb < 4; ++sb) {
        a2[sb] = *reinterpret_cast<const f32x4*>(sZ2 + (16 * wave + i) * PSLD + 16 * sb + 4 * g);
        a1[sb] = *reinterpret_cast<const f32x4*>(sZ1 + (16 * wave + i) * PSLD + 16 * sb + 4 * g);
      }
#pragma unroll
      for (int sb = 0; sb < 4; ++sb) {
        f32x4 b[HT];
#pragma unroll
        for (int ti = 0; ti < HT; ++ti)
          b[ti] = *reinterpret_cast<const f32x4*>(sH1 + (16 * ti + i) * PSLD + 16 * sb + 4 * g);
#pragma unroll
        for (int s = 0; s < 4; ++s)
#pragma unroll
          for (int ti = 0; ti < HT; ++ti) g2[ti] = OSA_MFMA(a2[sb][s], b[ti][s], g2[ti]);
      }
#pragma unroll
      for (int sb = 0; sb < 4; ++sb) {
        f32x4 b[KB];
#pragma unroll
        for (int kb = 0; kb < KB; ++kb)
          b[kb] = *reinterpret_cast<const f32x4*>(sX + (16 * kb + i) * PSLD + 16 * sb + 4 * g);
#pragma unroll
        for (int s = 0; s < 4; ++s)
#pragma unroll
          for (int kb = 0; kb < KB; ++kb) g1[kb] = OSA_MFMA(a1[sb][s], b[kb][s], g1[kb]);
      }
      if (small_out) {
        float q0 = 0.f, q1 = 0.f;
#pragma unroll
        for (int k = 0; k < 4; ++k) {
          const f32x4 hv = *reinterpret_cast<const f32x4*>(sH2 + (16 * wave + i) * PSLD + 16 * g + 4 * k);
          const f32x4 a0 = *reinterpret_cast<const f32x4*>(sDO + 16 * g + 4 * k);
          const f32x4 a1 = *reinterpret_cast<const f32x4*>(sDO + PSLD + 16 * g + 4 * k);
#pragma unroll
          for (int r = 0; r < 4; ++r) {
            q0 = fmaf(a0[r], hv[r], q0);
            q1 = fmaf(a1[r], hv[r], q1);
          }
        }
        q0 = osa_sum_over_groups(q0);
        q1 = osa_sum_over_groups(q1);
        if (g == 0) {
          g3[0][0] += q0;
          g3[0][1] += q1;
        }
      } else {
#pragma unroll
        for (int o = 0; o < OT; ++o) {
#pragma unroll
          for (int sb = 0; sb < 4; ++sb) {
            const f32x4 av = *reinterpret_cast<const f32x4*>(sDO + (16 * o + i) * PSLD + 16 * sb + 4 * g);
            const f32x4 b = *reinterpret_cast<const f32x4*>(sH2 + (16 * wave + i) * PSLD + 16 * sb + 4 * g);
            g3[o] = OSA_MFMA(av.x, b.x, g3[o]);
            g3[o] = OSA_MFMA(av.y, b.y, g3[o]);
            g3[o] = OSA_MFMA(av.z, b.z, g3[o]);
            g3[o] = OSA_MFMA(av.w, b.w, g3[o]);
          }
        }
      }
    }
    PTICK(5);
    {
      const float* srow = (tid < H) ? sZ1 + tid * PSLD
                          : (tid < 2 * H) ? sZ2 + (tid - H) * PSLD
                          : (tid < 2 * H + OUTP) ? sDO + (tid - 2 * H) * PSLD
                          : (tid < 2 * H + 2 * OUTP) ? sDL + (tid - 2 * H - OUTP) * PSLD
                                                     : sZ1;
      f32x4 q[16];
#pragma unroll
      for (int k = 0; k < 16; ++k) q[k] = *reinterpret_cast<const f32x4*>(srow + 4 * k);
      __builtin_amdgcn_sched_barrier(0);
      float rs = 0.f;
#pragma unroll
      for (int k = 0; k < 16; ++k) {
        rs += q[k].x;
        rs += q[k].y;
        rs += q[k].z;
        rs += q[k].w;
      }
      gb = (boff >= 0) ? ((MULTI && ch > 0) ? gb + rs : rs) : 0.f;
    }
    if (ch + 1 < nchunk) __syncthreads();
    if (ch == 0) OSA_PART_MARK(5);
    }
    OSA_PART_MARK(6);
    if (boff >= 0 && is_actor && boff >= nd.oLS && (boff - nd.oLS) < nd.act_dim && a.hp.entropy_coef != 0.f && own_terms &&
        !part)
      gb -= a.hp.entropy_coef / (float)nd.act_dim;
    f32x4 w2r[HT], w1r[KB], w3r[OT];
#pragma unroll
    for (int ti = 0; ti < HT; ++ti)
#pragma unroll
      for (int r = 0; r < 4; ++r) w2r[ti][r] = sW2[(16 * wave + 4 * g + r) * PSLD + 16 * ti + cc];
#pragma unroll
    for (int kb = 0; kb < KB; ++kb)
#pragma unroll
      for (int r = 0; r < 4; ++r) w1r[kb][r] = sW1[(16 * wave + 4 * g + r) * W1LD + 16 * kb + cc];
#pragma unroll
    for (int o = 0; o < OT; ++o)
#pragma unroll
      for (int r = 0; r < 4; ++r) w3r[o][r] = sW3[(16 * o + 4 * g + r) * PSLD + 16 * wave + cc];
    float wb = *sbias;
    wb = (boff >= 0) ? wb : 0.f;
    __builtin_amdgcn_sched_barrier(0);
    constexpr int NT = HT + KB + OT, XS = NT * 1024 + 256 + PNSTAT;
    float* __restrict__ xbase = nullptr;
    f32x4* __restrict__ xs4 = nullptr;
    const long p2p_off = P2P ? (long)OSA_P2P_HDR + (((long)((a.p2p_seq0 + (unsigned)(mb - a.mb0)) & 1u) * 3 + net) * a.dp_world) * XS : 0;
    if constexpr (P2P) {
      xbase = a.p2p_peer[a.p2p_rank] + p2p_off;
      xs4 = reinterpret_cast<f32x4*>(xbase + (long)rk * XS);
    } else if constexpr (coop) {
      xbase = a.dp_slabs + (((long)((mb - a.mb0) & 1) * 3 + net) * a.dp_world + (chunked ? crank * cw : 0)) * XS;
      xs4 = reinterpret_cast<f32x4*>(xbase + (long)(chunked ? cchunk : rk) * XS);
    }
    f32x4 acc_g = {0.f, 0.f, 0.f, 0.f}, acc_p = {0.f, 0.f, 0.f, 0.f};
#pragma unroll
    for (int ti = 0; ti < HT; ++ti) {
      const f32x4 w = w2r[ti];
      if (l2) g2[ti] = g2[ti] + w * c2;
      if constexpr (coop && !P2P) xs4[ti * 256 + tid] = g2[ti];
      acc_p = acc_p + w * w;
      acc_g = acc_g + g2[ti] * g2[ti];
    }
#pragma unroll
    for (int kb = 0; kb < KB; ++kb) {
      const f32x4 w = w1r[kb];
      if (l2) g1[kb] = g1[kb] + w * c2;
      if constexpr (coop && !P2P) xs4[(HT + kb) * 256 + tid] = g1[kb];
      acc_p = acc_p + w * w;
      acc_g = acc_g + g1[kb] * g1[kb];
    }
#pragma unroll
    for (int o = 0; o < OT; ++o) {
      const f32x4 w = w3r[o];
      if (l2) g3[o] = g3[o] + w * c2;
      if constexpr (coop && !P2P) xs4[(HT + KB + o) * 256 + tid] = g3[o];
      acc_p = acc_p + w * w;
      acc_g = acc_g + g3[o] * g3[o];
    }
    float gsq = (acc_g.x + acc_g.y) + (acc_g.z + acc_g.w);
    float psq = (acc_p.x + acc_p.y) + (acc_p.z + acc_p.w);
    if (boff >= 0) {
      if (l2) gb += c2 * wb;
      psq += wb * wb;
      gsq += gb * gb;
    }
    if constexpr (coop && !P2P) reinterpret_cast<float*>(xs4)[NT * 1024 + tid] = (boff >= 0) ? gb : 0.f;
    if constexpr (P2P) {
      for (int q = 1; q < a.dp_world; ++q) {
        int pr = a.p2p_rank + q;
        pr = pr >= a.dp_world ? pr - a.dp_world : pr;
        f32x4* __restrict__ d4 = reinterpret_cast<f32x4*>(a.p2p_peer[pr] + p2p_off + (long)rk * XS);
#pragma unroll
        for (int ti = 0; ti < HT; ++ti) osa_store_sys(d4 + ti * 256 + tid, g2[ti]);
#pragma unroll
        for (int kb = 0; kb < KB; ++kb) osa_store_sys(d4 + (HT + kb) * 256 + tid, g1[kb]);
#pragma unroll
        for (int o = 0; o < OT; ++o) osa_store_sys(d4 + (HT + KB + o) * 256 + tid, g3[o]);
        osa_store_sys(reinterpret_cast<float*>(d4) + NT * 1024 + tid, (boff >= 0) ? gb : 0.f);
      }
    }
    gsq = osa_wave_sum_dpp(gsq);
    psq = osa_wave_sum_dpp(psq);
    loss_part = osa_wave_sum_dpp(loss_part);
    ratio_part = osa_wave_sum_dpp(ratio_part);
    if (lane == 0) {
      red[4 * wave + 0] = gsq;
      red[4 * wave + 1] = psq;
      red[4 * wave + 2] = loss_part;
      red[4 * wave + 3] = ratio_part;
    }
    PTICK(6);
    __syncthreads();
    PTICK(7);
    const float t_gsq = red[0] + red[4] + red[8] + red[12];
    const float t_psq = red[1] + red[5] + red[9] + red[13];
    const float t_loss = red[2] + red[6] + red[10] + red[14];
    const float t_ratio = red[3] + red[7] + red[11] + red[15];
    const float total_norm = sqrtf(t_gsq);
    float coef = 1.f;
    if (a.hp.use_max_grad_norm) {
      coef = a.hp.max_grad_norm / (total_norm + 1e-6f);
      coef = coef > 1.f ? 1.f : coef;
    }
    if (dp) {
      float* __restrict__ slab = a.dp_slabs + ((long)net * a.dp_world + rk) * (P + PNSTAT);
      const float gs = (a.hp.use_max_grad_norm && !part) ? coef : 1.f;
#pragma unroll
      for (int ti = 0; ti < HT; ++ti)
#pragma unroll
        for (int r = 0; r < 4; ++r) slab[nd.oW2 + (16 * wave + 4 * g + r) * H + 16 * ti + cc] = g2[ti][r] * gs;
#pragma unroll
      for (int kb = 0; kb < KB; ++kb)
#pragma unroll
        for (int r = 0; r < 4; ++r) slab[nd.oW1 + (16 * wave + 4 * g + r) * INP + 16 * kb + cc] = g1[kb][r] * gs;
#pragma unroll
      for (int o = 0; o < OT; ++o)
#pragma unroll
        for (int r = 0; r < 4; ++r) slab[nd.oW3 + (16 * o + 4 * g + r) * H + 16 * wave + cc] = g3[o][r] * gs;
      if (boff >= 0) slab[boff] = gb * gs;
      if (critic && tid < OUTP) slab[nd.oLS + tid] = 0.f;
      if (leader && part) {
        slab[P + 0] = t_loss;
        slab[P + 1] = t_ratio;
      } else if (leader) {
        slab[P + 0] = t_loss * invB - (is_actor ? a.hp.entropy_coef * ent_pre : 0.f);
        slab[P + 1] = t_ratio * invB;
        slab[P + 2] = t_psq;
        slab[P + 3] = total_norm;
        slab[P + 4] = ent_pre;
      }
      return;
    }
    float st_loss = t_loss * invB, st_ratio = t_ratio * invB, st_psq = t_psq, st_norm = total_norm,
          st_ent = ent_pre;
    if (is_actor && own_terms) st_loss -= a.hp.entropy_coef * ent_pre;
    bool apply_clip = a.hp.use_max_grad_norm != 0;
    if constexpr (coop) {
      const int W = chunked ? cw : a.dp_world;
      const float gs = (apply_clip && !chunked) ? coef : 1.f;
      if constexpr (P2P) {
        if (wave == 3) {
          const float l_loss = __int_as_float(__builtin_amdgcn_readfirstlane(__float_as_int(st_loss)));
          const float l_ent = __int_as_float(__builtin_amdgcn_readfirstlane(__float_as_int(st_ent)));
          if (lane < a.dp_world) {
            float* tq = a.p2p_peer[lane] + p2p_off + (long)rk * XS + NT * 1024 + 256;
            osa_store_sys(reinterpret_cast<f32x4*>(tq), (f32x4){l_loss, st_ratio, st_psq, st_norm});
            osa_store_sys(tq + 4, l_ent);
            osa_store_sys(tq + 5, gs);
          }
        }
      } else if (leader) {
        float* t = reinterpret_cast<float*>(xs4) + NT * 1024 + 256;
        t[0] = st_loss; t[1] = st_ratio; t[2] = st_psq; t[3] = st_norm; t[4] = st_ent; t[5] = gs;
      }
      if constexpr (P2P) {
        if (a.p2p_fence) {
          __builtin_amdgcn_fence(__ATOMIC_RELEASE, "");
        } else {
          __builtin_amdgcn_fence(__ATOMIC_RELEASE, "workgroup");
          __builtin_amdgcn_s_waitcnt(0);
        }
        __syncthreads();
        PTICK(12);
        const unsigned target = a.p2p_seq0 + (unsigned)(mb - a.mb0) + 1u;
        if (tid < a.dp_world) {
          unsigned* theirs = reinterpret_cast<unsigned*>(a.p2p_peer[tid]) + 64 * net + a.p2p_rank;
          __hip_atomic_store(theirs, target, __ATOMIC_RELAXED, __HIP_MEMORY_SCOPE_SYSTEM);
          unsigned* own = reinterpret_cast<unsigned*>(a.p2p_peer[a.p2p_rank]);
          unsigned* mine = own + 64 * net + tid;
          if (!coop_dead) {
            long long t0 = 0;
            int spins = 0;
            while ((int)(__hip_atomic_load(mine, __ATOMIC_RELAXED, __HIP_MEMORY_SCOPE_SYSTEM) - target) < 0) {
              __builtin_amdgcn_s_sleep(1);
              if ((++spins & 1023) == 0) {
                const long long now = wall_clock64();
                if (t0 == 0) t0 = now;
                if (now - t0 > a.p2p_timeout ||
                    __hip_atomic_load(own + OSA_P2P_STICKY, __ATOMIC_RELAXED, __HIP_MEMORY_SCOPE_SYSTEM) != 0u) {
                  __hip_atomic_store(own + OSA_P2P_STICKY, 1u, __ATOMIC_RELAXED, __HIP_MEMORY_SCOPE_SYSTEM);
                  break;
                }
              }
            }
          }
        }
        __syncthreads();
        if (!coop_dead) coop_dead = __hip_atomic_load(reinterpret_cast<unsigned*>(a.p2p_peer[a.p2p_rank]) + OSA_P2P_STICKY,
                                                       __ATOMIC_RELAXED, __HIP_MEMORY_SCOPE_SYSTEM) != 0u;
        if (a.p2p_fence) __builtin_amdgcn_fence(__ATOMIC_ACQUIRE, "");
        else __builtin_amdgcn_fence(__ATOMIC_ACQUIRE, "agent");
      } else {
      if (a.dp_uncached || a.dp_local) {
        __builtin_amdgcn_fence(__ATOMIC_RELEASE, "workgroup");
        __builtin_amdgcn_s_waitcnt(0);
      } else {
        __builtin_amdgcn_fence(__ATOMIC_RELEASE, "agent");
      }
      __syncthreads();
      PTICK(12);
      if (tid == 0) {
        int* cnt = (nranks > 1) ? a.dp_sync + 8 + 16 * net + crank : a.dp_sync + net;
        const int target = W * (mb - a.mb0 + 1);
        int seen = __hip_atomic_fetch_add(cnt, 1, __ATOMIC_RELAXED, __HIP_MEMORY_SCOPE_AGENT) + 1;
        if (!coop_dead) {
          int spins = 0;
          while (seen < target) {
            __builtin_amdgcn_s_sleep(1);
            seen = __hip_atomic_load(cnt, __ATOMIC_RELAXED, __HIP_MEMORY_SCOPE_AGENT);
            if (++spins > (1 << 21)) {
              __hip_atomic_store(a.dp_sync + 3, 1, __ATOMIC_RELAXED, __HIP_MEMORY_SCOPE_AGENT);
              coop_dead = true;
              break;
            }
          }
        }
      }
      __syncthreads();
      __builtin_amdgcn_fence(__ATOMIC_ACQUIRE, "agent");
      }
      PTICK(10);
      f32x4 s2[HT], s1[KB], s3[OT];
      float sb_ = 0.f;
#pragma unroll
      for (int ti = 0; ti < HT; ++ti) s2[ti] = (f32x4){0.f, 0.f, 0.f, 0.f};
#pragma unroll
      for (int kb = 0; kb < KB; ++kb) s1[kb] = (f32x4){0.f, 0.f, 0.f, 0.f};
#pragma unroll
      for (int o = 0; o < OT; ++o) s3[o] = (f32x4){0.f, 0.f, 0.f, 0.f};
      if (W == 2) {
        const float* __restrict__ xr = xbase + (long)((chunked ? cchunk : rk) ^ 1) * XS;
        const f32x4* __restrict__ x4 = reinterpret_cast<const f32x4*>(xr);
        f32x4 t[NT];
#pragma unroll
        for (int q = 0; q < NT; ++q) t[q] = x4[q * 256 + tid];
        const float tb = xr[NT * 1024 + tid], tg = xr[NT * 1024 + 256 + 5];
#pragma unroll
        for (int ti = 0; ti < HT; ++ti) s2[ti] = osa_sym_sum(g2[ti], gs, t[ti], tg);
#pragma unroll
        for (int kb = 0; kb < KB; ++kb) s1[kb] = osa_sym_sum(g1[kb], gs, t[HT + kb], tg);
#pragma unroll
        for (int o = 0; o < OT; ++o) s3[o] = osa_sym_sum(g3[o], gs, t[HT + KB + o], tg);
        sb_ = osa_sym_sum1((boff >= 0) ? gb : 0.f, gs, tb, tg);
      } else {
      constexpr int RU = 4;
      for (int r0 = 0; r0 < W; r0 += RU) {
        f32x4 t[RU][NT];
        float tb[RU], tg[RU];
#pragma unroll
        for (int u = 0; u < RU; ++u) {
          int src = min(r0 + u, W - 1);
          if (P2P && src == rk) src = (src > 0) ? src - 1 : (W > 1 ? 1 : 0);
          const float* __restrict__ xr = xbase + (long)src * XS;
          const f32x4* __restrict__ x4 = reinterpret_cast<const f32x4*>(xr);
#pragma unroll
// ... 71 lines not shown
          const float* t0 = xbase + NT * 1024 + 256;
          st_loss = acc[0]; st_ratio = acc[1]; st_psq = t0[2]; st_norm = chunk_norm; st_ent = t0[4];
        } else {
          st_loss = acc[0] * invW; st_ratio = acc[1] * invW; st_psq = acc[2] * invW;
          st_norm = acc[3] * invW; st_ent = acc[4] * invW;
        }
      }
      if constexpr (HIER) {
        float* x2 = a.dp_slabs + (long)2 * 3 * a.dp_world * XS + (((long)((mb - a.mb0) & 1) * 3 + net) * nranks) * XS;
        f32x4* o4 = reinterpret_cast<f32x4*>(x2 + (long)crank * XS);
#pragma unroll
        for (int ti = 0; ti < HT; ++ti)
          if (ti % cw == cchunk) o4[ti * 256 + tid] = g2[ti];
#pragma unroll
        for (int kb = 0; kb < KB; ++kb)
          if ((HT + kb) % cw == cchunk) o4[(HT + kb) * 256 + tid] = g1[kb];
#pragma unroll
        for (int o = 0; o < OT; ++o)
          if ((HT + KB + o) % cw == cchunk) o4[(HT + KB + o) * 256 + tid] = g3[o];
        if (cchunk == 0) {
          float* row = x2 + (long)crank * XS + NT * 1024;
          row[tid] = (boff >= 0) ? gb : 0.f;
          if (leader) {
            float* t = row + 256;
            t[0] = st_loss; t[1] = st_ratio; t[2] = st_psq; t[3] = st_norm; t[4] = st_ent;
            t[5] = apply_clip ? coef : 1.f;
          }
        }
        if (a.dp_uncached || a.dp_local) {
          __builtin_amdgcn_fence(__ATOMIC_RELEASE, "workgroup");
          __builtin_amdgcn_s_waitcnt(0);
        } else {
          __builtin_amdgcn_fence(__ATOMIC_RELEASE, "agent");
        }
        __syncthreads();
        if (tid == 0) {
          int* cnt = a.dp_sync + net;
          const int target = a.dp_world * (mb - a.mb0 + 1);
          int seen = __hip_atomic_fetch_add(cnt, 1, __ATOMIC_RELAXED, __HIP_MEMORY_SCOPE_AGENT) + 1;
          if (!coop_dead) {
            int spins = 0;
            while (seen < target) {
              __builtin_amdgcn_s_sleep(1);
              seen = __hip_atomic_load(cnt, __ATOMIC_RELAXED, __HIP_MEMORY_SCOPE_AGENT);
              if (++spins > (1 << 21)) {
                __hip_atomic_store(a.dp_sync + 3, 1, __ATOMIC_RELAXED, __HIP_MEMORY_SCOPE_AGENT);
                coop_dead = true;
                break;
              }
            }
          }
        }
        __syncthreads();
        __builtin_amdgcn_fence(__ATOMIC_ACQUIRE, "agent");
#pragma unroll
        for (int ti = 0; ti < HT; ++ti) s2[ti] = (f32x4){0.f, 0.f, 0.f, 0.f};
#pragma unroll
        for (int kb = 0; kb < KB; ++kb) s1[kb] = (f32x4){0.f, 0.f, 0.f, 0.f};
#pragma unroll
        for (int o = 0; o < OT; ++o) s3[o] = (f32x4){0.f, 0.f, 0.f, 0.f};
        sb_ = 0.f;
        constexpr int RU2 = 4;
        for (int r0 = 0; r0 < nranks; r0 += RU2) {
          f32x4 t[RU2][NT];
          float tb[RU2], tg[RU2];
#pragma unroll
          for (int u = 0; u < RU2; ++u) {
            const float* __restrict__ xr = x2 + (long)min(r0 + u, nranks - 1) * XS;
            const f32x4* __restrict__ x4 = reinterpret_cast<const f32x4*>(xr);
#pragma unroll
            for (int q = 0; q < NT; ++q) t[u][q] = x4[q * 256 + tid];
            tb[u] = xr[NT * 1024 + tid];
            tg[u] = xr[NT * 1024 + 256 + 5];
          }
#pragma unroll
          for (int u = 0; u < RU2; ++u) {
            if (r0 + u < nranks) {
#pragma unroll
              for (int ti = 0; ti < HT; ++ti) s2[ti] = s2[ti] + t[u][ti] * tg[u];
#pragma unroll
              for (int kb = 0; kb < KB; ++kb) s1[kb] = s1[kb] + t[u][HT + kb] * tg[u];
#pragma unroll
              for (int o = 0; o < OT; ++o) s3[o] = s3[o] + t[u][HT + KB + o] * tg[u];
              sb_ += tb[u] * tg[u];
            }
          }
        }
        const float invR = 1.f / (float)nranks;
#pragma unroll
        for (int ti = 0; ti < HT; ++ti) g2[ti] = s2[ti] * invR;
#pragma unroll
        for (int kb = 0; kb < KB; ++kb) g1[kb] = s1[kb] * invR;
#pragma unroll
        for (int o = 0; o < OT; ++o) g3[o] = s3[o] * invR;
        gb = sb_ * invR;
        apply_clip = false;
        if (leader && rk == 0) {
          float acc[5] = {0.f, 0.f, 0.f, 0.f, 0.f};
          for (int r = 0; r < nranks; ++r) {
            const float* t = x2 + (long)r * XS + NT * 1024 + 256;
            for (int k = 0; k < 5; ++k) acc[k] += t[k];
          }
          st_loss = acc[0] * invR; st_ratio = acc[1] * invR; st_psq = acc[2] * invR;
          st_norm = acc[3] * invR; st_ent = acc[4] * invR;
        }
      }
    }
    const float gscale = apply_clip ? coef : 1.f;
    auto put_w2 = [&](int ti, f32x4 w) {
#pragma unroll
      for (int r = 0; r < 4; ++r) sW2[(16 * wave + 4 * g + r) * PSLD + 16 * ti + cc] = w[r];
      if constexpr (W2T) *reinterpret_cast<f32x4*>(sW2T + (16 * ti + cc) * PSLD + 16 * wave + 4 * g) = w;
    };
    auto put_w1 = [&](int kb, f32x4 w) {
#pragma unroll
      for (int r = 0; r < 4; ++r) sW1[(16 * wave + 4 * g + r) * W1LD + 16 * kb + cc] = w[r];
    };
    auto put_w3 = [&](int o, f32x4 w) {
#pragma unroll
      for (int r = 0; r < 4; ++r) sW3[(16 * o + 4 * g + r) * PSLD + 16 * wave + cc] = w[r];
    };
#pragma unroll
    for (int ti = 0; ti < HT; ++ti) {
      {
        f32x4 w = w2r[ti];
        w = osa_adam_update4(g2[ti] * gscale, m2[ti], v2[ti], w, beta1, beta2, step_size, inv_bc2_sqrt, aeps);
        put_w2(ti, w);
      }
    }
#pragma unroll
    for (int kb = 0; kb < KB; ++kb) {
      {
        f32x4 w = w1r[kb];
        w = osa_adam_update4(g1[kb] * gscale, m1[kb], v1[kb], w, beta1, beta2, step_size, inv_bc2_sqrt, aeps);
        put_w1(kb, w);
      }
    }
#pragma unroll
    for (int o = 0; o < OT; ++o) {
      {
        f32x4 w = w3r[o];
        w = osa_adam_update4(g3[o] * gscale, m3[o], v3[o], w, beta1, beta2, step_size, inv_bc2_sqrt, aeps);
        put_w3(o, w);
      }
    }
    {
      float nb = wb;
      if (boff >= 0) {
        float mv_ = mb_, vv_ = vb_;
        nb = osa_adam_update(gb * gscale, mv_, vv_, wb, beta1, beta2, step_size, inv_bc2_sqrt, aeps);
        *sbias = nb;
        mb_ = mv_;
        vb_ = vv_;
      }
    }
    PTICK(8);
    if (leader && (P2P || rk == 0)) {
      float* st = a.stats + (long)(mb - a.mb0) * PNSTAT;
      if (is_actor) {
        st[2] = st_loss;
        st[3] = st_ratio;
        st[4] = st_ent;
        st[7] = st_norm;
        if constexpr (EXT) {
          if (a.ext_cost_kappa > 0.f) st[10] = cost_pen;
        }
      } else {
        st[net - 1] = st_loss;
        st[4 + net] = st_psq;
        st[7 + net] = st_norm;
      }
    }
    __syncthreads();
    PTICK(9);
  }
#ifdef OSA_PASS_CLOCKS
  if (a.dbg && tid == 0 && (P2P || rk == 0))
    for (int k = 0; k < 13; ++k) a.dbg[net * 16 + k] = dbg_acc[k];
#endif
  if (!P2P && rk != 0) return;
  for (int e = tid; e < H * INP; e += 256) gp[nd.oW1 + e] = sW1[(e / INP) * W1LD + (e % INP)];
  for (int e = tid; e < H * H; e += 256) gp[nd.oW2 + e] = sW2[(e >> 6) * PSLD + (e & 63)];
  for (int e = tid; e < OUTP * H; e += 256) gp[nd.oW3 + e] = sW3[(e >> 6) * PSLD + (e & 63)];
  if (tid < H) {
    gp[nd.ob1 + tid] = sB1[tid];
    gp[nd.ob2 + tid] = sB2[tid];
  }
  if (tid < OUTP) {
    gp[nd.ob3 + tid] = sB3[tid];
    if (!critic) gp[nd.oLS + tid] = sLS[tid];
  }
#pragma unroll
  for (int ti = 0; ti < HT; ++ti)
#pragma unroll
      for (int r = 0; r < 4; ++r) {
        const int off = nd.oW2 + (16 * wave + 4 * g + r) * H + 16 * ti + cc;
        gm[off] = m2[ti][r];
        gv[off] = v2[ti][r];
      }
#pragma unroll
  for (int kb = 0; kb < KB; ++kb)
#pragma unroll
      for (int r = 0; r < 4; ++r) {
        const int off = nd.oW1 + (16 * wave + 4 * g + r) * INP + 16 * kb + cc;
        gm[off] = m1[kb][r];
        gv[off] = v1[kb][r];
      }
#pragma unroll
  for (int o = 0; o < OT; ++o)
#pragma unroll
      for (int r = 0; r < 4; ++r) {
        const int off = nd.oW3 + (16 * o + 4 * g + r) * H + 16 * wave + cc;
        gm[off] = m3[o][r];
        gv[off] = v3[o][r];
      }
  if (boff >= 0) {
    gm[boff] = mb_;
    gv[boff] = vb_;
  }
  if (tid == 0) a.adam_step[net] = step0 + a.nmb;
  (void)out_dim;
}


#include <type_traits>

static inline size_t osa_pass_lds_bytes(int KB, int OT) {
  const size_t fl = (size_t)osa_pass_lds_floats(KB, OT) + (osa_pass_has_w2t(KB, OT) ? 64 * PSLD : 0);
  return fl * sizeof(float);
}

template <int I = 0, class F>
static int osa_pass_shapes(int KB, int OT, F&& f) {
  if constexpr (I == 12) {
    return OSA_EUNSUPPORTED;
  } else {
    constexpr int K = I % 6 + 1, O = I / 6 + 1;
    if (KB == K && OT == O) return f(std::integral_constant<int, K>{}, std::integral_constant<int, O>{});
    return osa_pass_shapes<I + 1>(KB, OT, f);
  }
}

template <int OT, class F>
static int osa_pass_so(const OsaNet& nd, F&& f) {
  if constexpr (OT == 1) {
    if (nd.act_dim <= 2) return f(std::true_type{});
  }
  return f(std::false_type{});
}

template <auto K, bool COOP = false, class A>
static int osa_launch_pass_kernel(const A& a, const OsaNet& nd, dim3 grid, hipStream_t stream) {
  static OsaPerDeviceOnce attr_set;
  const size_t lds = osa_pass_lds_bytes(nd.KB, nd.OUTP / 16);
  if (lds > 160 * 1024) return OSA_EUNSUPPORTED;
  if (attr_set.need()) {
    if (hipFuncSetAttribute(reinterpret_cast<const void*>(K), hipFuncAttributeMaxDynamicSharedMemorySize,
                            160 * 1024) != hipSuccess)
      return OSA_EHIP;
    attr_set.set();
  }
  if constexpr (COOP) {
    static bool coop_refused = getenv("OSA_DP_PLAIN_LAUNCH") != nullptr && getenv("OSA_DP_PLAIN_LAUNCH")[0] == '1';
    if (!coop_refused) {
      A arg = a;
      void* kargs[] = {&arg};
      const hipError_t e =
          hipLaunchCooperativeKernel(reinterpret_cast<const void*>(K), grid, dim3(256), kargs, (unsigned)lds, stream);
      if (e == hipSuccess) return OSA_OK;
      (void)hipGetLastError();
      if (e == hipErrorCooperativeLaunchTooLarge) return OSA_EUNSUPPORTED;
      coop_refused = true;
    }
    int per_cu = 0, dev = 0, cus = 0;
    if (hipOccupancyMaxActiveBlocksPerMultiprocessor(&per_cu, reinterpret_cast<const void*>(K), 256, lds) !=
            hipSuccess ||
        hipGetDevice(&dev) != hipSuccess ||
        hipDeviceGetAttribute(&cus, hipDeviceAttributeMultiprocessorCount, dev) != hipSuccess)
      return OSA_EHIP;
    if ((long)per_cu * cus < (long)grid.x * grid.y) return OSA_EUNSUPPORTED;
  }
  hipLaunchKernelGGL(K, grid, dim3(256), lds, stream, a);
  return hipGetLastError() == hipSuccess ? OSA_OK : OSA_EHIP;
}

template <auto K, bool COOP = false>
static int osa_launch_pass_kernel(const OsaPassArgs& a, dim3 grid, hipStream_t stream) {
  return osa_launch_pass_kernel<K, COOP>(a, a.nd, grid, stream);
}

static inline int osa_plain_pass_args(OsaPassArgs& a, bool* extended, int obs_dim, int act_dim, int hidden,
                                      float* params, float* adam_m, float* adam_v, int* adam_step, const float* obs,
                                      int ld_obs, const float* act, int ld_act, const float* logp,
                                      const float* target_value_r, const float* target_value_c, const float* adv_r,
                                      const float* adv_c, const long* perm, long M, int B, const float* lagrange,
                                      const osa_ppo_hparams* hp, int loss_kind, int nets_mask, float* step_stats,
                                      const osa_surrogate_ext* ext) {
  OSA_REQUIRE(params && adam_m && adam_v && adam_step && obs && act && logp && hp && step_stats);
  OSA_REQUIRE(target_value_r && target_value_c && adv_r && adv_c && M > 0 && B > 0);
  OSA_REQUIRE(ld_obs >= obs_dim && ld_act >= act_dim);
  if (!osa_rows_ok(obs, ld_obs, (double)M, ld_act)) return OSA_EUNSUPPORTED;
  a = OsaPassArgs{};
  a.ext_ratio_scale = 1.f; a.ext_mask_eta = -1.f;
  osa_fill_operands(a, obs_dim, act_dim, hidden, params, adam_m, adam_v, adam_step, obs, ld_obs, act, ld_act, logp,
                    target_value_r, target_value_c, adv_r, adv_c, lagrange, hp, loss_kind, nets_mask, step_stats);
  a.perm = perm; a.M = M; a.B = B; a.nmb = (int)((M + B - 1) / B);
  a.dp_world = 1;
  *extended = false;
  if (ext) {
    if (B > 64) return OSA_EUNSUPPORTED;
    const bool need_old = ext->kl_coef != 0.f || ext->kl_mask_eta >= 0.f;
// ... 12 lines not shown
```

### omnisafe_amd/csrc/ppo_pass_kernel.hip

```cpp
#include "ppo_pass_body.h"

template <int KB, int OT, bool MULTI, bool COOP, bool EXT, bool HIER = false, bool DPS = false, bool SO = false>
__global__ __launch_bounds__(256, 1) void osa_ppo_pass_kernel(OsaPassArgs a) {
  int net_ = blockIdx.x, rk_ = blockIdx.y;
  if constexpr (!COOP) {
    if (a.one_xcc) {
      if (blockIdx.x & 7) return;
      net_ = blockIdx.x >> 3;
    }
  }
  if constexpr (COOP) {
    if (a.dp_local == 1) {
      net_ = blockIdx.x & 7;
      rk_ = blockIdx.x >> 3;
      if (net_ >= 3) return;
    }
  }
  const int net = net_, rk = rk_;
  if (!((a.nets_mask >> net) & 1)) return;
  osa_ppo_pass_body<KB, OT, MULTI, COOP, EXT, HIER, DPS, SO>(a, net, rk);
}

static long long* g_osa_pass_dbg = nullptr;

long long* osa_pass_dbg_ptr() { return g_osa_pass_dbg; }

template <int KB, int OT, bool MULTI, bool COOP = false, bool EXT = false, bool HIER = false, bool DPS = false,
          bool SO = false>
static int osa_launch_pass(const OsaPassArgs& a, hipStream_t stream, int grid_y = 1) {
  const dim3 grid = (COOP && a.dp_local == 1) ? dim3(8 * grid_y) : ((!COOP && a.one_xcc) ? dim3(17) : dim3(3, grid_y));
  return osa_launch_pass_kernel<osa_ppo_pass_kernel<KB, OT, MULTI, COOP, EXT, HIER, DPS, SO>, COOP>(a, grid, stream);
}

template <int KB, int OT, bool MULTI, bool COOP = false, bool EXT = false, bool HIER = false>
static int osa_launch_pass_so(const OsaPassArgs& a, hipStream_t stream, int grid_y = 1) {
  return osa_pass_so<OT>(a.nd, [&](auto SO) {
    return osa_launch_pass<KB, OT, MULTI, COOP, EXT, HIER, false, SO>(a, stream, grid_y);
  });
}

extern "C" {

int osa_debug_set_pass_clock_buffer(long long* dev_ptr) {
  g_osa_pass_dbg = dev_ptr;
  return OSA_OK;
}

int osa_ppo_pass_supported(int obs_dim, int act_dim, int hidden) {
  if (hidden != 64 || obs_dim < 1 || act_dim < 1 || act_dim > 32) return 0;
  const int KB = (obs_dim + 15) / 16, OT = (act_dim + 15) / 16;
  return (KB <= 6 && OT <= 2 && osa_pass_lds_bytes(KB, OT) <= 160 * 1024) ? 1 : 0;
}

int osa_ppo_pass(int obs_dim, int act_dim, int hidden, float* params, float* adam_m, float* adam_v,
                 int* adam_step, const float* obs, int ld_obs, const float* act, int ld_act,
                 const float* logp, const float* target_value_r, const float* target_value_c,
                 const float* adv_r, const float* adv_c, const long* perm, long M, int B,
                 const float* lagrange, const osa_ppo_hparams* hp, int loss_kind, int nets_mask,
                 float* step_stats, void* stream) {
  return osa_ppo_pass_ext(obs_dim, act_dim, hidden, params, adam_m, adam_v, adam_step, obs, ld_obs, act, ld_act,
                          logp, target_value_r, target_value_c, adv_r, adv_c, perm, M, B, lagrange, hp,
                          loss_kind, nets_mask, step_stats, nullptr, stream);
}

int osa_ppo_pass_ext(int obs_dim, int act_dim, int hidden, float* params, float* adam_m, float* adam_v,
                 int* adam_step, const float* obs, int ld_obs, const float* act, int ld_act,
                 const float* logp, const float* target_value_r, const float* target_value_c,
                 const float* adv_r, const float* adv_c, const long* perm, long M, int B,
                 const float* lagrange, const osa_ppo_hparams* hp, int loss_kind, int nets_mask,
                 float* step_stats, const osa_surrogate_ext* ext, void* stream) {
  if (!osa_ppo_pass_supported(obs_dim, act_dim, hidden)) return OSA_EUNSUPPORTED;
  OsaPassArgs a;
  bool extended = false;
  const int rc = osa_plain_pass_args(a, &extended, obs_dim, act_dim, hidden, params, adam_m, adam_v, adam_step, obs,
                                     ld_obs, act, ld_act, logp, target_value_r, target_value_c, adv_r, adv_c, perm, M,
                                     B, lagrange, hp, loss_kind, nets_mask, step_stats, ext);
  if (rc != OSA_OK) return rc;
  a.dbg = g_osa_pass_dbg;
  {
    static const bool one = !(getenv("OSA_PASS_ONE_XCC") && getenv("OSA_PASS_ONE_XCC")[0] == '0');
    a.one_xcc = one ? 1 : 0;
  }
  const int KB = a.nd.KB, OT = a.nd.OUTP / 16;
  hipStream_t st = osa_stream(stream);
  if (extended)
    return osa_pass_shapes(KB, OT, [&](auto K, auto O) { return osa_launch_pass_so<K, O, false, false, true>(a, st); });
  return osa_pass_shapes(KB, OT, [&](auto K, auto O) {
    return (B > 64) ? osa_launch_pass_so<K, O, true>(a, st) : osa_launch_pass_so<K, O, false>(a, st);
  });
}

}

__global__ __launch_bounds__(256) void osa_dp_apply_kernel(OsaNet nd, float* params, float* adam_m,
                                                           float* adam_v, const int* adam_step,
                                                           const float* slabs, int W, OsaPassHp hp,
                                                           const float* lr_dev, int nets_mask,
                                                           float* stats, int step_index) {
  const int net = blockIdx.y;
  if (!((nets_mask >> net) & 1)) return;
  const int P = nd.P, SW = P + PNSTAT;
  const bool critic = net != 0;
  const float* __restrict__ sl = slabs + (long)net * W * SW;
  const int e = blockIdx.x * blockDim.x + threadIdx.x;
  const int step = adam_step[net] + step_index + 1;
  const float lr = lr_dev ? lr_dev[critic ? 1 : 0] : (critic ? hp.lr_critic : hp.lr_actor);
  const double bc1 = -expm1((double)step * log((double)hp.beta1));
  const double bc2 = -expm1((double)step * log((double)hp.beta2));
  const float step_size = (float)((double)lr / bc1);
  const float inv_bc2_sqrt = (float)(1.0 / sqrt(bc2));
  const float invW = 1.f / (float)W;
  if (e < P) {
    float g = 0.f;
    for (int r = 0; r < W; ++r) g += sl[(long)r * SW + e];
    g *= invW;
    if (critic && e >= nd.oLS) g = 0.f;
    const long o = (long)net * P + e;
    float mv = adam_m[o], vv = adam_v[o];
    params[o] = osa_adam_update(g, mv, vv, params[o], hp.beta1, hp.beta2, step_size, inv_bc2_sqrt, hp.adam_eps);
    adam_m[o] = mv;
    adam_v[o] = vv;
  }
  if (blockIdx.x == 0 && threadIdx.x < 5) {
    const int k = threadIdx.x;
    float t = 0.f;
    for (int r = 0; r < W; ++r) t += sl[(long)r * SW + P + k];
    t *= invW;
    if (net == 0) {
      if (k == 0) stats[2] = t;
      if (k == 1) stats[3] = t;
      if (k == 4) stats[4] = t;
      if (k == 3) stats[7] = t;
    } else {
      if (k == 0) stats[net - 1] = t;
      if (k == 2) stats[4 + net] = t;
      if (k == 3) stats[7 + net] = t;
    }
  }
}

__global__ void osa_dp_step_count_kernel(int* adam_step, int nets_mask, int nsteps) {
  const int net = threadIdx.x;
  if (net < 3 && ((nets_mask >> net) & 1)) adam_step[net] += nsteps;
}

extern "C" {

size_t osa_ppo_dp_ws_floats(int obs_dim, int act_dim, int hidden, int world) {
  if (!osa_ppo_pass_supported(obs_dim, act_dim, hidden) || world < 1) return 0;
  const OsaNet nd = osa_make_net(obs_dim, act_dim, hidden);
  return (size_t)3 * world * (nd.P + PNSTAT);
}

int osa_ppo_dp_step(int obs_dim, int act_dim, int hidden, float* params, float* adam_m, float* adam_v,
                    int* adam_step, const float* obs, int ld_obs, const float* act, int ld_act,
                    const float* logp, const float* target_value_r, const float* target_value_c,
                    const float* adv_r, const float* adv_c, const long* perm, long M, int B, int world,
                    int step_index, const float* lagrange, const osa_ppo_hparams* hp,
                    const float* lr_dev, int loss_kind, int nets_mask, float* slabs,
                    float* step_stats, void* stream) {
  return osa_ppo_dp_step_phase(obs_dim, act_dim, hidden, params, adam_m, adam_v, adam_step, obs, ld_obs, act, ld_act,
                               logp, target_value_r, target_value_c, adv_r, adv_c, perm, M, B, world, step_index,
                               lagrange, hp, lr_dev, loss_kind, nets_mask, slabs, step_stats, 0, stream);
}

int osa_ppo_dp_step_phase(int obs_dim, int act_dim, int hidden, float* params, float* adam_m, float* adam_v,
                          int* adam_step, const float* obs, int ld_obs, const float* act, int ld_act,
                          const float* logp, const float* target_value_r, const float* target_value_c,
                          const float* adv_r, const float* adv_c, const long* perm, long M, int B, int world,
                          int step_index, const float* lagrange, const osa_ppo_hparams* hp,
                          const float* lr_dev, int loss_kind, int nets_mask, float* slabs,
                          float* step_stats, int phase, void* stream) {
  if (!osa_ppo_pass_supported(obs_dim, act_dim, hidden)) return OSA_EUNSUPPORTED;
  OSA_REQUIRE(phase >= 0 && phase <= 2);
  if (phase == 2) {
    OSA_REQUIRE(params && adam_m && adam_v && adam_step && hp && step_stats && slabs && world >= 1 && step_index >= 0);
    const OsaNet nd = osa_make_net(obs_dim, act_dim, hidden);
    OsaPassHp h = {};
    osa_copy_hparams(h, hp);
    hipLaunchKernelGGL(osa_dp_apply_kernel, dim3((nd.P + 255) / 256, 3), dim3(256), 0, osa_stream(stream), nd, params,
                       adam_m, adam_v, adam_step, slabs, world, h, lr_dev, nets_mask & (hp->use_cost ? 7 : 3), step_stats,
                       step_index);
    return hipGetLastError() == hipSuccess ? OSA_OK : OSA_EHIP;
  }
  OSA_REQUIRE(params && adam_m && adam_v && adam_step && obs && act && logp && hp && step_stats && slabs);
  OSA_REQUIRE(target_value_r && target_value_c && adv_r && adv_c && M > 0 && B > 0 && world >= 1);
  OSA_REQUIRE(ld_obs >= obs_dim && ld_act >= act_dim && step_index >= 0 && (long)step_index * B < M);
  if (!osa_rows_ok(obs, ld_obs, (double)M * world)) return OSA_EUNSUPPORTED;
  OsaPassArgs a = {};
  a.ext_ratio_scale = 1.f; a.ext_mask_eta = -1.f;
  osa_fill_operands(a, obs_dim, act_dim, hidden, params, adam_m, adam_v, adam_step, obs, ld_obs, act, ld_act, logp,
                    target_value_r, target_value_c, adv_r, adv_c, lagrange, hp, loss_kind, nets_mask, step_stats);
  a.perm = perm; a.M = M; a.B = B; a.nmb = 1;
  a.dp_slabs = slabs; a.dp_world = world; a.mb0 = step_index;
  const int KB = a.nd.KB, OT = a.nd.OUTP / 16;
  hipStream_t st = osa_stream(stream);
  const int rc = osa_pass_shapes(KB, OT, [&](auto K, auto O) {
    return (B > 64) ? osa_launch_pass<K, O, true, false, false, false, true>(a, st, world)
                    : osa_launch_pass<K, O, false, false, false, false, true>(a, st, world);
  });
  if (rc != OSA_OK || phase == 1) return rc;
  hipLaunchKernelGGL(osa_dp_apply_kernel, dim3((a.nd.P + 255) / 256, 3), dim3(256), 0, st, a.nd, params,
                     adam_m, adam_v, adam_step, slabs, world, a.hp, lr_dev, a.nets_mask, step_stats,
                     step_index);
  return hipGetLastError() == hipSuccess ? OSA_OK : OSA_EHIP;
}

static const int OSA_MAX_XCH = 1024;
static char* g_xch_base[OSA_MAX_XCH];
static size_t g_xch_bytes[OSA_MAX_XCH];

bool osa_is_exchange_ptr(const void* p) {
  const char* c = static_cast<const char*>(p);
  for (int k = 0; k < OSA_MAX_XCH; ++k)
    if (g_xch_base[k] && c >= g_xch_base[k] && c < g_xch_base[k] + g_xch_bytes[k]) return true;
  return false;
}

int osa_dp_exchange_alloc(size_t floats, float** out) {
  OSA_REQUIRE(out != nullptr && floats > 0);
  void* p = nullptr;
  if (hipExtMallocWithFlags(&p, floats * sizeof(float), hipDeviceMallocUncached) != hipSuccess || !p) {
    (void)hipGetLastError();
    return OSA_EUNSUPPORTED;
  }
  if (hipMemset(p, 0, floats * sizeof(float)) != hipSuccess) return OSA_EHIP;
  for (int k = 0; k < OSA_MAX_XCH; ++k)
    if (!g_xch_base[k]) {
      g_xch_base[k] = static_cast<char*>(p);
      g_xch_bytes[k] = floats * sizeof(float);
      *out = static_cast<float*>(p);
      return OSA_OK;
    }
  (void)hipFree(p);
  return OSA_EUNSUPPORTED;
}

// ... 154 lines not shown
```

### omnisafe_amd/update.py

```python
from __future__ import annotations

import ctypes as C
import os

import numpy as np
import torch

from . import _lib
from . import distributed as dist
from .models import ConstraintActorCritic, HParams, PassMember, SurrogateExt

NSTAT = 16


_PLACEMENT = {'local_ok': None}


def _local_arg() -> int:
    return 3 if os.environ.get('OSA_DEBUG_PLACEMENT') == 'wrong' else 1


class PPOUpdater:
    def __init__(self, ac: ConstraintActorCritic, *, batch_size: int, update_iters: int,
                 target_kl: float, kl_early_stop: bool, clip: float = 0.2, entropy_coef: float = 0.0,
                 use_critic_norm: bool = True, critic_norm_coef: float = 0.001,
                 use_max_grad_norm: bool = True, max_grad_norm: float = 40.0, use_cost: bool = True,
                 loss_kind: int = 0, max_blocks: int = 256, update_actor: bool = True,
                 persistent: bool = True, dp_mode: str = 'replicated', seed: int = 0,
                 update_critics: bool = True, ext: SurrogateExt | None = None) -> None:
        self.ac = ac
        self.ext = ext
        self.general = bool(getattr(ac, 'general', False))
        if self.general and ext is not None and int(batch_size) > 256 and (ext.kl_mask_eta >= 0 or ext.cost_kappa > 0):
            raise NotImplementedError('FOCOPS / P3O on general networks: batch_size <= 256')
        self.update_critics = update_critics
        self.lib = _lib.load(require_gpu=True)
        self.batch_size, self.update_iters = int(batch_size), int(update_iters)
        self.target_kl, self.kl_early_stop = float(target_kl), bool(kl_early_stop)
        self.loss_kind = loss_kind
        self.update_actor = update_actor
        self.persistent = persistent
        self.persistent_max_batch = 512
        self.dp_mode = dp_mode
        self._mode = 'allreduce' if dp_mode == 'p2p' else dp_mode
        self._p2p: dict = {}
        self.seed = int(seed)
        self._dp: dict = {}
        self._ar_k = 0
        self.hp = HParams(clip=clip, entropy_coef=entropy_coef, critic_norm_coef=critic_norm_coef,
                          max_grad_norm=max_grad_norm, lr_actor=0.0, lr_critic=0.0, beta1=0.9,
                          beta2=0.999, adam_eps=1e-8, use_critic_norm=int(use_critic_norm),
                          use_max_grad_norm=int(use_max_grad_norm), use_cost=int(use_cost))
        self.max_blocks = int(max_blocks)
        dev = ac.device
        nws = self.lib.osa_minibatch_ws_floats(ac.obs_dim, ac.act_dim, ac.hidden, self.max_blocks)
        self._ws = torch.zeros(max(nws, 1), dtype=torch.float32, device=dev)
        self._kl_ws = torch.empty(1024, dtype=torch.float64, device=dev)
        self._kl = torch.zeros(1, dtype=torch.float32, device=dev)
        self._old_mean: torch.Tensor | None = None
        self._old_log_std = torch.zeros(ac.layout.OUTP, dtype=torch.float32, device=dev)
        self._stats: torch.Tensor | None = None
        self.profile_events: list | None = None
        self.last_path: str | None = None
        self.generator: torch.Generator | None = None
        self.pass_submit = None
        self.last_group = 0
        self._graphed_pass = False
        self._use_wide = False
        self._split_xch: int | None = None
        self._split_tried = False
        self._chunk: dict = {}
        self._ug: dict = {}
        self._split_local = False
        self._split_verified = False
        self._split_buf = None
        self._repl_wide = False

    def _chunk_ok(self, data: dict) -> bool:
        B = self.batch_size
        ck = self._chunk
        if ck.get('off') or self.ext is not None or B <= 64 or os.environ.get('OSA_CHUNKED_PASS', '1') == '0':
            return False
        W = (B + 63) // 64
        if ck.get('W') != W:
            ac = self.ac
            cus = torch.cuda.get_device_properties(ac.device).multi_processor_count
            if W > cus // 8:
                ck['off'] = True
                return False
            n = self.lib.osa_ppo_dp_pass_ws_floats(ac.obs_dim, ac.act_dim, ac.hidden, W)
            ck.update(W=W, xch=torch.zeros(max(n, 1), dtype=torch.float32, device=ac.device),
                      sync=torch.zeros(8, dtype=torch.int32, device=ac.device),
                      local=0 if _PLACEMENT['local_ok'] is False else 1, verified=False)
        return True

    def check_chunk_sync(self) -> None:
        ck = self._chunk
        if 'sync' in ck and int(ck['sync'][3]) != 0:
            raise _lib.OsaError('osa_ppo_chunked_pass: ' + (
                'the workgroups of a network were not placed on one XCC' if int(ck['sync'][3]) == 2
                else 'a cooperating workgroup never arrived') + ' (results invalid); set OSA_CHUNKED_PASS=0')

    def _split_alloc(self) -> None:
        if self._split_tried:
            return
        self._split_tried = True
        ac = self.ac
        if os.environ.get('OSA_WIDE_SPLIT', '1') == '0' or not bool(
                self.lib.osa_ppo_split_pass_supported(ac.obs_dim, ac.act_dim, ac.hidden)):
            return
        n = self.lib.osa_ppo_split_pass_xch_floats(ac.obs_dim, ac.act_dim, ac.hidden)
        self._split_local = os.environ.get('OSA_WIDE_SPLIT', 'local') != 'spread' and _PLACEMENT['local_ok'] is not False
        if self._split_local:
            self._split_buf = torch.zeros(max(n, 1), dtype=torch.float32, device=ac.device)
            self._split_xch = self._split_buf.data_ptr()
            return
        p = C.c_void_p()
        if self.lib.osa_dp_exchange_alloc(max(n, 1), C.byref(p)) == _lib.OSA_OK and p.value:
            self._split_xch = p.value

    def _split_free(self) -> None:
        if self._split_xch and not getattr(self, '_split_local', False):
            self.lib.osa_dp_exchange_free(C.c_void_p(self._split_xch))
        self._split_xch = None
        self._split_buf = None

    def check_split_sync(self) -> None:
        if self._split_xch:
            flag = C.c_int(0)
            _lib.check(self.lib.osa_ppo_split_pass_timed_out(C.c_void_p(self._split_xch), C.byref(flag)),
                       'osa_ppo_split_pass_timed_out')
            if flag.value:
                raise _lib.OsaError('osa_ppo_split_pass: ' + (
                    'the workgroups of a network were not placed on one XCC; set OSA_WIDE_SPLIT=spread'
                    if flag.value == 2 else 'a cooperating workgroup never arrived') + ' (results invalid)')

    def _nets_mask(self) -> int:
        m = (0b110 if self.hp.use_cost else 0b010) if self.update_critics else 0
        return m | (1 if self.update_actor else 0)

    def _operands(self, data: dict, perm: torch.Tensor | None, M: int | None, B: int) -> tuple:
        ac = self.ac
        head = (ac.obs_dim, ac.act_dim, ac.hidden, _lib.ptr(ac.params), _lib.ptr(ac.adam_m), _lib.ptr(ac.adam_v),
                _lib.ptr(ac.adam_step))
        rows = (_lib.ptr(data['obs']), data['obs'].stride(0), _lib.ptr(data['act']), data['act'].stride(0),
                _lib.ptr(data['logp']), _lib.ptr(data['target_value_r']), _lib.ptr(data['target_value_c']),
                _lib.ptr(data['adv_r']), _lib.ptr(data['adv_c']), _lib.ptr(perm))
        if M is None:
            return head + (_lib.ptr(ac.grads),) + rows + (B,)
        return head + rows + (M, B)

    def _profile_begin(self) -> tuple | None:
        if self.profile_events is None:
            return None
        ev = (torch.cuda.Event(enable_timing=True), torch.cuda.Event(enable_timing=True))
        ev[0].record()
        return ev

    def _profile_end(self, ev: tuple | None, name: str, rows: int) -> None:
        if ev is not None:
            ev[1].record()
            self.profile_events.append((name, rows, ev))

    @staticmethod
    def _placement_verified(read_flag, timeout_msg: str) -> bool:
        torch.cuda.synchronize()
        flag = read_flag()
        if flag == 1:
            raise _lib.OsaError(timeout_msg)
        if flag != 0:
            _PLACEMENT['local_ok'] = False
            return False
        return True

    def shuffles(self, rows: int, M: int, out: torch.Tensor | None = None,
                 generator: torch.Generator | None = None) -> torch.Tensor:
        dev = self.ac.device
        if generator is None:
            generator = self.generator
        if os.environ.get('OSA_SHUFFLE', 'bijection') == 'sort':
            keys = torch.randint(0, 1 << 62, (rows, M), generator=generator, device=dev, dtype=torch.int64)
            p = keys.argsort(dim=1)
            if out is None:
                return p
            out.copy_(p.reshape(out.shape))
            return out
        seeds = torch.randint(0, 1 << 62, (rows,), generator=generator, device=dev, dtype=torch.int64)
        if out is None:
            out = torch.empty((rows, M), dtype=torch.int64, device=dev)
        assert out.is_contiguous() and out.numel() == rows * M
        _lib.check(self.lib.osa_shuffle_rows(_lib.ptr(seeds), rows, M, _lib.ptr(out), _lib.stream_ptr()),
                   'osa_shuffle_rows')
        return out

    def _graph_pass_ok(self, M: int) -> bool:
        nmb = (M + self.batch_size - 1) // self.batch_size
        dp_graph = (dist.collectives_active() and self._mode == 'allreduce' and not self.general and nmb <= 1100
                    and dist.graph_capturable())
        return ((self.batch_size >= 2048 or (self.general and nmb <= 256) or dp_graph) and self.ext is None
                and (not dist.collectives_active() or dist.graph_capturable())
                and os.environ.get('OSA_UPDATE_GRAPH', '1') != '0' and not self._ug.get('failed', False))

    def _graph_pass(self, data: dict, perm: torch.Tensor | None, lagrange: torch.Tensor, stats_rows: torch.Tensor,
                    passes: int = 1) -> None:
        ac, B = self.ac, self.batch_size
        M = data['obs'].shape[0]
        nmb = (M + B - 1) // B
        hp = self.hp
        if dist.collectives_active() and self._allreduce_fast_ok(data, B):
            self._ar_slab()
        key = (M, B, passes, tuple(int(data[k].data_ptr()) for k in ('obs', 'act', 'logp', 'target_value_r',
                                                                     'target_value_c', 'adv_r', 'adv_c')),
               int(lagrange.data_ptr()),
               self._nets_mask(), self.loss_kind, self.max_blocks, dist.collectives_active(),
               tuple(int(t.data_ptr()) for t in (ac.params, ac.adam_m, ac.adam_v, ac.adam_step, ac.grads, self._ws)),
               int(ac.gmlp_ws(B)[0].data_ptr()) if self.general else 0,
               (self._mode, os.environ.get('OSA_ALLREDUCE_FAST', '1'),
                int(self._ar_slab_t.data_ptr()) if getattr(self, '_ar_slab_t', None) is not None else 0),
               (data['obs'].stride(0), data['act'].stride(0)),
# ... 47 lines not shown
                    st['failed'], st['graph'] = True, None
                    enqueue()
        finally:
            hp.lr_device = None
            self.profile_events = pe
        self._profile_end(ev, 'gm_gemm_kernel' if self.general else 'osa_mb_grad_kernel', passes * M)
        stats_rows.copy_(st['stats'])
        self._graphed_pass = st['graph'] is not None

    def _allreduce_fast_ok(self, data: dict, B: int) -> bool:
        obs = data['obs']
        return (self._mode == 'allreduce' and not self.general and self.ext is None and self.loss_kind in (0, 1)
                and self.batch_size <= self.persistent_max_batch and obs.stride(0) % 4 == 0 and obs.data_ptr() % 16 == 0
                and os.environ.get('OSA_ALLREDUCE_FAST', '1') != '0'
                and bool(self.lib.osa_ppo_pass_supported(self.ac.obs_dim, self.ac.act_dim, self.ac.hidden)))

    def _ar_slab(self) -> torch.Tensor:
        if getattr(self, '_ar_slab_t', None) is None:
            n = self.lib.osa_ppo_dp_ws_floats(self.ac.obs_dim, self.ac.act_dim, self.ac.hidden, 1)
            self._ar_slab_t = torch.zeros(n, dtype=torch.float32, device=self.ac.device)
        return self._ar_slab_t

    def _ar_end_pass(self) -> None:
        if self._ar_k:
            _lib.check(self.lib.osa_ppo_dp_end_pass(_lib.ptr(self.ac.adam_step),
                                                    self._nets_mask() & (7 if self.hp.use_cost else 3), self._ar_k,
                                                    _lib.stream_ptr()), 'osa_ppo_dp_end_pass')
            self._ar_k = 0

    def minibatch(self, data: dict, idx: torch.Tensor | None, B: int, lagrange: torch.Tensor,
                  stats_row: torch.Tensor) -> None:
        ac, lib, st = self.ac, self.lib, _lib.stream_ptr()
        dp = dist.collectives_active()
        mode = 1 if dp else 0
        ev = self._profile_begin()
        if self.general:
            ws, nws = ac.gmlp_ws(B)
            gext = None
            if self.ext is not None:
                self.ext.old_mean = self._old_mean.data_ptr()
                self.ext.ld_old_mean = self._old_mean.stride(0)
                self.ext.old_log_std = self._old_log_std.data_ptr()
                gext = C.byref(self.ext)
            _lib.check(lib.osa_gmlp_minibatch_ext(
                C.byref(ac.desc), _lib.ptr(ac.params), _lib.ptr(ac.adam_m), _lib.ptr(ac.adam_v),
                _lib.ptr(ac.adam_step), _lib.ptr(ac.grads), _lib.ptr(data['obs']), data['obs'].stride(0),
                _lib.ptr(data['act']), data['act'].stride(0), _lib.ptr(data['logp']),
                _lib.ptr(data['target_value_r']), _lib.ptr(data['target_value_c']), _lib.ptr(data['adv_r']),
                _lib.ptr(data['adv_c']), _lib.ptr(idx), B, _lib.ptr(lagrange), C.byref(self.hp), self.loss_kind,
                mode, self._nets_mask(), None, 0.0, _lib.ptr(ws), nws, _lib.ptr(stats_row), gext, st),
                'osa_gmlp_minibatch_ext')
            self._profile_end(ev, 'gm_gemm_kernel', B)
            if dp:
                dist.all_reduce_avg_(ac.grads)
                _lib.check(lib.osa_gmlp_adam_apply(C.byref(ac.desc), _lib.ptr(ac.params), _lib.ptr(ac.adam_m),
                                                   _lib.ptr(ac.adam_v), _lib.ptr(ac.adam_step), _lib.ptr(ac.grads),
                                                   C.byref(self.hp), self._nets_mask(), _lib.ptr(ac._gfin), st),
                           'osa_gmlp_adam_apply')
            return
        if dp and self._allreduce_fast_ok(data, B):
            slab = self._ar_slab()
            args = self._operands(data, idx, B, self.batch_size) + (1,)
            tail = (_lib.ptr(lagrange), C.byref(self.hp), self.hp.lr_device, self.loss_kind, self._nets_mask(),
                    _lib.ptr(slab), _lib.ptr(stats_row))
            _lib.check(lib.osa_ppo_dp_step_phase(*args, 0, *tail, 1, st), 'osa_ppo_dp_step_phase(grad)')
            self._profile_end(ev, 'osa_ppo_pass_kernel', B)
            dist.all_reduce_avg_(slab)
            _lib.check(lib.osa_ppo_dp_step_phase(*args, self._ar_k, *tail, 2, st), 'osa_ppo_dp_step_phase(apply)')
            self._ar_k += 1
            return
        ext = None
        if self.ext is not None:
            self.ext.old_mean = self._old_mean.data_ptr()
            self.ext.ld_old_mean = self._old_mean.stride(0)
            self.ext.old_log_std = self._old_log_std.data_ptr()
            ext = C.byref(self.ext)
        _lib.check(lib.osa_ppo_minibatch_ext(
            *self._operands(data, idx, None, B), _lib.ptr(lagrange), C.byref(self.hp), self.loss_kind, mode,
            self._nets_mask(), self.max_blocks, _lib.ptr(self._ws), _lib.ptr(stats_row), ext, st),
            'osa_ppo_minibatch_ext')
        self._profile_end(ev, 'osa_mb_grad_kernel', B)
        if dp:
            dist.all_reduce_avg_(ac.grads)
            _lib.check(lib.osa_adam_apply(ac.obs_dim, ac.act_dim, ac.hidden, _lib.ptr(ac.params),
                                          _lib.ptr(ac.adam_m), _lib.ptr(ac.adam_v),
                                          _lib.ptr(ac.adam_step), _lib.ptr(ac.grads), C.byref(self.hp),
                                          self._nets_mask(), st), 'osa_adam_apply')

    def run_pass(self, data: dict, perm: torch.Tensor, lagrange: torch.Tensor,
                 stats_rows: torch.Tensor) -> None:
        M = data['obs'].shape[0]
        ops = self._operands(data, perm, M, self.batch_size)
        ev = self._profile_begin()
        if self._use_wide and self._split_xch:
            rc = self.lib.osa_ppo_split_pass(
                *ops, _lib.ptr(lagrange), C.byref(self.hp), self.loss_kind, self._nets_mask(), C.c_void_p(self._split_xch),
                (1 if self._split_verified else _local_arg()) if self._split_local else 0, _lib.ptr(stats_rows),
                _lib.stream_ptr())
            if rc == _lib.OSA_EUNSUPPORTED:
                self._split_free()
            else:
                _lib.check(rc, 'osa_ppo_split_pass')
                if self._split_local and not self._split_verified:
                    if not self._placement_verified(
                            lambda: int(self._split_buf.view(torch.int32)[96]),
                            'osa_ppo_split_pass: a cooperating workgroup never arrived at the placement check '
                            '(device shared with another long-running kernel?)'):
                        self._split_free()
                        self._split_tried = False
                        self._split_alloc()
                        return self.run_pass(data, perm, lagrange, stats_rows)
                    self._split_verified = _PLACEMENT['local_ok'] = True
                self.last_path = 'persistent-wide-split'
                self._profile_end(ev, 'osa_wide_split_kernel', M)
                return
        if self._use_wide:
            _lib.check(self.lib.osa_ppo_wide_pass(
                *ops, _lib.ptr(lagrange), C.byref(self.hp), self.loss_kind, self._nets_mask(), _lib.ptr(self._wide_ws),
                _lib.ptr(stats_rows), _lib.stream_ptr()), 'osa_ppo_wide_pass')
            self._profile_end(ev, 'osa_wide_pass_kernel', M)
            return
        if self._chunk_ok(data):
            ck = self._chunk
            rc = self.lib.osa_ppo_chunked_pass(
                *ops, _lib.ptr(lagrange), C.byref(self.hp), self.loss_kind, self._nets_mask(), _lib.ptr(ck['xch']),
                _lib.ptr(ck['sync']),
                (1 if ck.get('verified') else _local_arg()) if ck.get('local', 1) else 0, _lib.ptr(stats_rows),
                _lib.stream_ptr())
            if rc == _lib.OSA_EUNSUPPORTED:
                ck['off'] = True
            else:
                _lib.check(rc, 'osa_ppo_chunked_pass')
                if ck.get('local', 1) and not ck.get('verified'):
                    if not self._placement_verified(
                            lambda: int(ck['sync'][3]),
                            'osa_ppo_chunked_pass: a cooperating workgroup never arrived at the placement check '
                            '(device shared with another long-running kernel?)'):
                        ck['sync'].zero_()
                        ck['local'] = 0
                        return self.run_pass(data, perm, lagrange, stats_rows)
                    ck['verified'] = _PLACEMENT['local_ok'] = True
                self.last_path = 'persistent-chunked'
                self._profile_end(ev, 'osa_ppo_pass_kernel', M)
                return
        ext = None
        if self.ext is not None:
            self.ext.old_mean = self._old_mean.data_ptr()
            self.ext.ld_old_mean = self._old_mean.stride(0)
            self.ext.old_log_std = self._old_log_std.data_ptr()
            ext = C.byref(self.ext)
        if self.pass_submit is not None:
            self.last_group = int(self.pass_submit(self, self._pass_member(ops, lagrange, stats_rows)))
        else:
            _lib.check(self.lib.osa_ppo_pass_ext(
                *ops, _lib.ptr(lagrange), C.byref(self.hp), self.loss_kind, self._nets_mask(), _lib.ptr(stats_rows),
                ext, _lib.stream_ptr()), 'osa_ppo_pass_ext')
        self._profile_end(ev, 'osa_ppo_pass_kernel', M)

    def _pass_member(self, ops: tuple, lagrange: torch.Tensor, stats_rows: torch.Tensor) -> PassMember:
        m = PassMember()
        (m.params, m.adam_m, m.adam_v, m.adam_step, m.obs, m.ld_obs, m.act, m.ld_act, m.logp, m.target_value_r,
         m.target_value_c, m.adv_r, m.adv_c, m.perm, m.M, m.B) = ops[3:]
        m.lagrange, m.loss_kind, m.nets_mask, m.step_stats = _lib.ptr(lagrange), self.loss_kind, self._nets_mask(), \
            _lib.ptr(stats_rows)
        C.memmove(C.byref(m.hp), C.byref(self.hp), C.sizeof(self.hp))
        m.has_ext = int(self.ext is not None)
        if self.ext is not None:
            C.memmove(C.byref(m.ext), C.byref(self.ext), C.sizeof(self.ext))
        return m

    def _p2p_ok(self, data: dict) -> bool:
        obs = data['obs']
        return (self.dp_mode == 'p2p' and not self.general and self.ext is None and self.loss_kind in (0, 1)
                and self.persistent and self.batch_size <= self.persistent_max_batch and dist.world_size() <= 16
                and obs.stride(0) % 4 == 0 and obs.data_ptr() % 16 == 0 and not self._p2p.get('off')
                and bool(self.lib.osa_ppo_pass_supported(self.ac.obs_dim, self.ac.act_dim, self.ac.hidden)))

    def _p2p_setup(self) -> bool:
        import torch.distributed as tdist

        ac, lib, st = self.ac, self.lib, self._p2p
        W, rank = dist.world_size(), dist.rank()
        if st.get('W') == W and st.get('peers') is not None:
            return True
        self._p2p_free()
        n = lib.osa_p2p_exchange_floats(ac.obs_dim, ac.act_dim, ac.hidden, W)
        own, handle = C.c_void_p(), (C.c_ubyte * 64)()
        ok = n > 0 and lib.osa_p2p_exchange_alloc(n, C.byref(own), handle) == _lib.OSA_OK and bool(own.value)
        handles: list = [None] * W
        if W > 1:
            tdist.all_gather_object(handles, bytes(handle) if ok else None)
        else:
            handles[0] = bytes(handle) if ok else None
        ok = all(h is not None for h in handles)
        ptrs = [None] * W
        opened = []
        if ok:
            for q in range(W):
                if q == rank:
                    ptrs[q] = own.value
                    continue
                pq = C.c_void_p()
                buf = (C.c_ubyte * 64).from_buffer_copy(handles[q])
                if lib.osa_p2p_exchange_open(buf, C.byref(pq)) != _lib.OSA_OK or not pq.value:
                    ok = False
                    break
                ptrs[q] = pq.value
                opened.append(pq.value)
        flag = torch.tensor([1.0 if ok else 0.0], device=ac.device if dist.graph_capturable() else 'cpu')
        if W > 1:
            tdist.all_reduce(flag, op=tdist.ReduceOp.MIN)
        if float(flag) < 1.0:
            for pq in opened:
                lib.osa_p2p_exchange_release(C.c_void_p(pq))
            if own.value:
                lib.osa_p2p_exchange_release(own)
            st['off'] = True
            import warnings

            warnings.warn('omnisafe_amd: the peer-exchange buffers could not be allocated / mapped on every rank '
                          '(hipIpc refused); dp_mode falls back to the per-step all-reduce', RuntimeWarning)
            return False
        st.update(W=W, own=own.value, opened=opened, peers=(C.c_void_p * W)(*ptrs), seq=0,
                  timeout=float(os.environ.get('OSA_P2P_TIMEOUT_S', '20')))
        return True

    def _p2p_free(self) -> None:
        st = self._p2p
        for pq in st.get('opened', []):
            self.lib.osa_p2p_exchange_release(C.c_void_p(pq))
        if st.get('own'):
            self.lib.osa_p2p_exchange_release(C.c_void_p(st['own']))
        for k in ('own', 'opened', 'peers', 'W'):
            st.pop(k, None)

    def check_p2p_sync(self) -> None:
        st = self._p2p
        if st.get('own'):
            flag = C.c_int(0)
            _lib.check(self.lib.osa_p2p_exchange_timed_out(C.c_void_p(st['own']), C.byref(flag)),
                       'osa_p2p_exchange_timed_out')
            if flag.value:
                raise _lib.OsaError('osa_ppo_p2p_pass: a peer rank never arrived at an optimiser step within '
                                    f"{st['timeout']} s (results invalid); set OSA_DP_MODE=allreduce")

    def run_pass_p2p(self, data: dict, perm: torch.Tensor, lagrange: torch.Tensor, stats_rows: torch.Tensor) -> None:
        st = self._p2p
        M = data['obs'].shape[0]
        nmb = (M + self.batch_size - 1) // self.batch_size
        ev = self._profile_begin()
        _lib.check(self.lib.osa_ppo_p2p_pass(
            *self._operands(data, perm, M, self.batch_size), st['W'], dist.rank(), st['peers'],
            st['seq'] & 0xFFFFFFFF, st['timeout'], _lib.ptr(lagrange), C.byref(self.hp), self.loss_kind,
            self._nets_mask(), _lib.ptr(stats_rows), _lib.stream_ptr()), 'osa_ppo_p2p_pass')
        st['seq'] += nmb
        self._profile_end(ev, 'osa_ppo_p2p_pass_kernel', M)

    _DP_KEYS = ('obs', 'act', 'logp', 'target_value_r', 'target_value_c', 'adv_r', 'adv_c')

    def gather_for_replicated(self, data: dict, W: int) -> dict:
        M = data['obs'].shape[0]
        st = self._dp
        if st.get('M') != M or st.get('W') != W:
            self._dp_free()
            st.clear()
            st.update(M=M, W=W, graph=None)
            st['data'] = {k: torch.empty((W * M,) + tuple(data[k].shape[1:]), dtype=torch.float32,
                                         device=self.ac.device) for k in self._DP_KEYS}
        for k in self._DP_KEYS:
            dist.all_gather_rows(data[k], out=st['data'][k])
        return st['data']

    def _dp_state(self, M: int, W: int, nmb: int) -> dict:
        ac, st = self.ac, self._dp
        if st.get('M') != M or st.get('W') != W:
            self._dp_free()
            st.clear()
            st.update(M=M, W=W, graph=None)
        if 'perm' not in st:
            dev = ac.device
            st['perm'] = torch.zeros(W, M, dtype=torch.int64, device=dev)
            st['pass_stats'] = torch.zeros(nmb, NSTAT, dtype=torch.float32, device=dev)
            st['slabs'] = torch.empty(self.lib.osa_ppo_dp_ws_floats(ac.obs_dim, ac.act_dim, ac.hidden, W),
                                      dtype=torch.float32, device=dev)
            st['lr'] = torch.zeros(2, dtype=torch.float32, device=dev)
            st['gen'] = torch.Generator(device=dev)
            st['gen'].manual_seed(self.seed + 7919)
            st['graph'] = None
        return st

    def _dp_enqueue_pass(self, data_all: dict, M: int, W: int, lagrange: torch.Tensor, st: dict, nmb: int) -> None:
        ac, lib = self.ac, self.lib
        ops = self._operands(data_all, st['perm'], M, self.batch_size)
        for k in range(nmb):
            _lib.check(lib.osa_ppo_dp_step(
                *ops, W, k, _lib.ptr(lagrange), C.byref(self.hp), _lib.ptr(st['lr']), self.loss_kind,
                self._nets_mask(), _lib.ptr(st['slabs']), _lib.ptr(st['pass_stats'][k]), _lib.stream_ptr()),
                'osa_ppo_dp_step')
        _lib.check(lib.osa_ppo_dp_end_pass(_lib.ptr(ac.adam_step), self._nets_mask() & (7 if self.hp.use_cost else 3),
                                           nmb, _lib.stream_ptr()), 'osa_ppo_dp_end_pass')

    def _dp_free(self) -> None:
        self._split_free()
        st = self._dp
        if st.get('xch') is None and st.get('xch_ptr'):
            self.lib.osa_dp_exchange_free(st['xch_ptr'])
        st.pop('xch_ptr', None)
        if st.get('wide_xch'):
            self.lib.osa_dp_exchange_free(C.c_void_p(st['wide_xch']))
        st.pop('wide_xch', None)
# ... 110 lines not shown
            flag = C.c_int(0)
            _lib.check(self.lib.osa_ppo_split_pass_timed_out(C.c_void_p(st['wide_xch']), C.byref(flag)),
                       'osa_ppo_split_pass_timed_out')
            if flag.value:
                raise _lib.OsaError('osa_ppo_split_dp_pass: a cooperating workgroup never arrived (results invalid); '
                                    'set OSA_DP_MODE=allreduce')

    def check_dp_sync(self) -> None:
        st = self._dp
        if 'sync' in st and int(st['sync'][3]) != 0:
            if int(st['sync'][3]) == 2:
                raise RuntimeError('osa_ppo_dp_pass_placed: the workgroups of a network were not placed on one XCC '
                                   '(results invalid); set OSA_DP_XCH=uncached')
            raise RuntimeError('osa_ppo_dp_pass: a peer workgroup timed out (workgroups not co-resident?); '
                               'set OSA_DP_MODE=replicated-steps')

    def check_reduce_sync(self) -> None:
        if int(self._ws.view(torch.int32)[-5]) != 0:
            raise RuntimeError('osa_ppo_minibatch: the workgroups of the slab reduction did not all arrive '
                               '(device shared with another long-running kernel?)')

    def run_pass_replicated(self, data_all: dict, M: int, W: int, lagrange: torch.Tensor,
                            stats_rows: torch.Tensor, perms_all: torch.Tensor | None = None,
                            use_graph: bool = True, coop: bool | None = None) -> None:
        ac = self.ac
        nmb = (M + self.batch_size - 1) // self.batch_size
        st = self._dp_state(M, W, nmb)
        if perms_all is not None:
            st['perm'].copy_(perms_all.reshape(W, M))
        else:
            self.shuffles(W, M, out=st['perm'], generator=st['gen'])
        if self._repl_wide:
            ev = self._profile_begin()
            self._wide_dp_pass(data_all, M, W, lagrange, st)
            self._profile_end(ev, 'osa_wide_split_kernel', W * M)
            stats_rows.copy_(st['pass_stats'][:stats_rows.shape[0]])
            return
        if coop is None:
            coop = self.dp_mode != 'replicated-steps'
        if coop:
            ev = self._profile_begin()
            if self._dp_coop_pass(data_all, M, W, lagrange, st):
                self._profile_end(ev, 'osa_ppo_dp_pass', W * M)
                stats_rows.copy_(st['pass_stats'][:stats_rows.shape[0]])
                return
        st['lr'][0] = float(self.hp.lr_actor)
        st['lr'][1] = float(self.hp.lr_critic)
        key = (M, W, nmb, self._nets_mask(), int(lagrange.data_ptr()), data_all['obs'].data_ptr())
        ev = self._profile_begin()
        graph_ok = use_graph and not st.get('graph_failed', False) and st.get('warm', False)
        if graph_ok and (st.get('graph') is None or st.get('graph_key') != key):
            try:
                g = torch.cuda.CUDAGraph()
                with torch.cuda.graph(g):
                    self._dp_enqueue_pass(data_all, M, W, lagrange, st, nmb)
                st['graph'], st['graph_key'] = g, key
            except Exception:
                st['graph_failed'], st['graph'] = True, None
                graph_ok = False
        if graph_ok and st.get('graph') is not None:
            st['graph'].replay()
        else:
            self._dp_enqueue_pass(data_all, M, W, lagrange, st, nmb)
            st['warm'] = True
        self._profile_end(ev, 'osa_ppo_dp_step', W * M)
        stats_rows.copy_(st['pass_stats'][:stats_rows.shape[0]])

    def _aligned_rows(self, data: dict) -> dict:
        obs = data['obs']
        if obs.stride(0) % 4 == 0 and obs.data_ptr() % 16 == 0 and obs.stride(1) == 1:
            return data
        M, D = obs.shape
        pad = torch.zeros(M, (D + 3) // 4 * 4, dtype=torch.float32, device=obs.device)
        pad[:, :D].copy_(obs)
        out = dict(data)
        out['obs'] = pad[:, :D]
        return out

    def snapshot_old_distribution(self, obs: torch.Tensor) -> None:
        ac, M = self.ac, obs.shape[0]
        if self._old_mean is None or self._old_mean.shape[0] != M:
            self._old_mean = torch.empty(M, ac.act_dim, dtype=torch.float32, device=ac.device)
        if self.general:
            ws, nws = ac.gmlp_ws(M)
            _lib.check(self.lib.osa_gmlp_actor_stats(
                C.byref(ac.desc), _lib.ptr(ac.params[0]), _lib.ptr(obs), obs.stride(0), M, None, 0, None, 0, 0, None, 0,
                None, None, None, None, _lib.ptr(self._old_mean), ac.act_dim, _lib.ptr(ws), nws, None,
                _lib.stream_ptr()), 'osa_gmlp_actor_stats(snapshot)')
        else:
            _lib.check(self.lib.osa_actor_kl(ac.obs_dim, ac.act_dim, ac.hidden, _lib.ptr(ac.params[0]),
                                             _lib.ptr(obs), obs.stride(0), M, None, 0, None, 0,
                                             _lib.ptr(self._old_mean), ac.act_dim, None, None,
                                             _lib.stream_ptr()), 'osa_actor_kl(snapshot)')
        lay = ac.layout
        self._old_log_std[:lay.act_dim].copy_(ac.params[0, lay.oLS:lay.oLS + lay.act_dim])

    def kl(self, obs: torch.Tensor, reduce_mode: int = 0) -> torch.Tensor:
        ac, M = self.ac, obs.shape[0]
        if self.general:
            ws, nws = ac.gmlp_ws(M)
            _lib.check(self.lib.osa_gmlp_actor_stats(
                C.byref(ac.desc), _lib.ptr(ac.params[0]), _lib.ptr(obs), obs.stride(0), M, _lib.ptr(self._old_mean),
                ac.act_dim, _lib.ptr(self._old_log_std), 0, reduce_mode, None, 0, None, None, None, None, None, 0,
                _lib.ptr(ws), nws, _lib.ptr(self._kl), _lib.stream_ptr()), 'osa_gmlp_actor_stats(kl)')
            dist.all_reduce_avg_(self._kl)
            return self._kl
        _lib.check(self.lib.osa_actor_kl(ac.obs_dim, ac.act_dim, ac.hidden, _lib.ptr(ac.params[0]),
                                         _lib.ptr(obs), obs.stride(0), M, _lib.ptr(self._old_mean),
                                         ac.act_dim, _lib.ptr(self._old_log_std), reduce_mode, None, 0,
                                         _lib.ptr(self._kl_ws), _lib.ptr(self._kl), _lib.stream_ptr()),
                   'osa_actor_kl')
        dist.all_reduce_avg_(self._kl)
        return self._kl

    def run(self, data: dict, lagrange: torch.Tensor, perms=None, actor_lr: float | None = None,
            critic_lr: float | None = None) -> dict:
        ac = self.ac
        self.hp.lr_actor = float(actor_lr if actor_lr is not None else (ac.actor_lr or 0.0))
        self.hp.lr_critic = float(critic_lr if critic_lr is not None else ac.critic_lr)
        obs = data['obs']
        M, B = obs.shape[0], self.batch_size
        nmb = (M + B - 1) // B
        total = self.update_iters * nmb
        if self._stats is None or self._stats.shape[0] < total:
            self._stats = torch.zeros(total, NSTAT, dtype=torch.float32, device=ac.device)
        stats = self._stats
        if self.update_actor:
            self.snapshot_old_distribution(obs)
        update_counts, final_kl, step = 0, 0.0, 0
        kl_dev = None
        self.last_group = 0
        self._pass_fn = None
        self._graphed_pass = False
        pmb = self.persistent_max_batch if self._chunk.get('off') or self.ext is not None or os.environ.get(
            'OSA_CHUNKED_PASS', '1') == '0' else max(self.persistent_max_batch, 1024)
        if (self.persistent and not self.general and (self.ext is None or B <= 64) and not dist.collectives_active()
                and B <= pmb and bool(
                self.lib.osa_ppo_pass_supported(ac.obs_dim, ac.act_dim, ac.hidden))):
            self._pass_fn = ('osa_ppo_pass_kernel', self.lib.osa_ppo_pass)
        self._use_wide = False
        if (self._pass_fn is None and self.persistent and not self.general and self.ext is None
                and not dist.collectives_active() and B <= 64 and self.loss_kind in (0, 1)
                and bool(self.lib.osa_ppo_wide_pass_supported(ac.obs_dim, ac.act_dim, ac.hidden))):
            self._pass_fn = ('osa_wide_pass_kernel', self.lib.osa_ppo_wide_pass)
            self._use_wide = True
            if getattr(self, '_wide_ws', None) is None:
                n = self.lib.osa_ppo_wide_pass_ws_floats(ac.obs_dim, ac.act_dim, ac.hidden)
                self._wide_ws = torch.empty(n, dtype=torch.float32, device=ac.device)
            self._split_alloc()
        use_pass = self._pass_fn is not None
        W = dist.world_size()
        if not self.general:
            data = self._aligned_rows(data)
        use_p2p = dist.collectives_active() and self._p2p_ok(data) and self._p2p_setup()
        self._mode = 'allreduce' if self.dp_mode == 'p2p' else self.dp_mode
        use_repl = (dist.collectives_active() and not self.general and self.ext is None and self.update_critics
                    and self.dp_mode in ('replicated', 'replicated-steps') and B <= self.persistent_max_batch and bool(
            self.lib.osa_ppo_pass_supported(ac.obs_dim, ac.act_dim, ac.hidden)))
        self._repl_wide = (not use_repl and not self.general and dist.collectives_active() and self.update_critics
                           and self.dp_mode in ('replicated', 'replicated-steps') and self._wide_dp_fits(W))
        use_repl = use_repl or self._repl_wide
        if use_repl:
            gathered = self._aligned_rows(self.gather_for_replicated(data, W))
        self.last_path = ('replicated-wide-split' if self._repl_wide else 'replicated') if use_repl else (
            ('persistent-wide' if self._use_wide else 'persistent') if use_pass else ('p2p' if use_p2p else 'per-step'))
        all_perms = None
        whole = (perms is None and not use_repl and not use_pass and not use_p2p and self._graph_pass_ok(M)
                 and not (self.update_actor and self.kl_early_stop)
                 and self.update_iters * nmb * (16 if self.general else 1) <= 1024
                 and os.environ.get('OSA_UPDATE_GRAPH_WHOLE', '1') != '0')
        if whole:
            self._graph_pass(data, None, lagrange, stats[:total], passes=self.update_iters)
            step, update_counts = total, self.update_iters
            last_perm = self._ug['perm'][(self.update_iters - 1) * M:]
            if self.update_actor:
                kl_dev = self.kl(obs)
        elif perms is None and not use_repl:
            all_perms = self.shuffles(self.update_iters, M)
        for i in range(0 if whole else self.update_iters):
            if use_repl:
                perm = None
            elif perms is not None:
                perm = torch.as_tensor(perms[i]).to(ac.device, torch.int64)
            else:
                perm = all_perms[i]
            if use_repl:
                pa = None if perms is None else torch.as_tensor(perms[i]).to(ac.device, torch.int64)
                self.run_pass_replicated(gathered, M, W, lagrange, stats[step:step + nmb], perms_all=pa)
                step += nmb
            elif use_pass:
                self.run_pass(data, perm, lagrange, stats[step:step + nmb])
                step += nmb
            elif use_p2p:
                self.run_pass_p2p(data, perm, lagrange, stats[step:step + nmb])
                step += nmb
            elif self._graph_pass_ok(M):
                self._graph_pass(data, perm, lagrange, stats[step:step + nmb])
                step += nmb
            else:
                for s in range(0, M, B):
                    nb = min(B, M - s)
                    self.minibatch(data, perm[s:s + nb], nb, lagrange, stats[step])
                    step += 1
                self._ar_end_pass()
            update_counts += 1
            last_perm = self._dp['perm'][dist.rank()] if use_repl else perm
            if self.update_actor and (self.kl_early_stop or i == self.update_iters - 1):
                kl_dev = self.kl(obs)
                if self.kl_early_stop:
                    final_kl = float(kl_dev)
                    if use_repl:
                        self.check_dp_sync()
                        self.check_wide_dp_sync()
                    if use_p2p:
                        self.check_p2p_sync()
                    if final_kl > self.target_kl:
                        break
        if use_repl:
            self.check_dp_sync()
            self.check_wide_dp_sync()
        if use_p2p:
            self.check_p2p_sync()
        if not use_repl and not use_pass and not use_p2p and B > 64 and not self.general:
            self.check_reduce_sync()
        if use_p2p:
            pass
        elif not use_repl and not use_pass and B >= 2048 and dist.collectives_active() and self.ext is None:
            self.last_path = 'dp-large-batch-graph' if getattr(self, '_graphed_pass', False) else 'dp-large-batch'
        elif (not use_repl and not use_pass and dist.collectives_active() and self._mode == 'allreduce'
              and getattr(self, '_graphed_pass', False)):
            self.last_path = 'allreduce-graph'
        if self.general:
            self.last_path = 'general-' + self.last_path
        if self._use_wide:
            self.check_split_sync()
        if self.last_path == 'persistent-chunked':
            self.check_chunk_sync()
        used = stats[:step]
        out = {'stop_iter': update_counts, 'steps': step, 'stats': used,
               'last_minibatch': last_perm[(nmb - 1) * B:M]}
        if self.update_actor:
            out['kl'] = float(kl_dev) if kl_dev is not None else final_kl
        return out

    @staticmethod
    def summarize(run_out: dict, critic_norm_coef: float, use_critic_norm: bool) -> dict:
        s = run_out['stats'].cpu().numpy().astype(np.float64)
        coef = critic_norm_coef if use_critic_norm else 0.0
        loss_r = s[:, 0] + coef * s[:, 5]
        loss_c = s[:, 1] + coef * s[:, 6]
        return {
            'Loss/Loss_reward_critic': float(loss_r.mean()), 'Loss/Loss_cost_critic': float(loss_c.mean()),
            'Loss/Loss_pi': float(s[:, 2].mean()), 'Train/PolicyRatio': float(s[:, 3].mean()),
            'Train/PolicyRatio/Std': float(s[:, 3].std()) if len(s) > 1 else 0.0,
            'Train/Entropy': float(s[:, 4].mean()),
            'per_step': {'loss_r': loss_r, 'loss_c': loss_c, 'loss_pi': s[:, 2], 'ratio_mean': s[:, 3],
                         'entropy': s[:, 4]},
        }
```

Baseline: 177,900.

## Pack per-row PPO pass inputs into aligned records and add fast-path bias/logstd handling

Adds a pack kernel that gathers obs, action, logp, advantages and targets into one 16-byte-aligned record per row. The persistent PPO pass kernel gets a REC variant that reads these records with vector loads instead of several scattered arrays. For the single-chunk small-output path it also precomputes log-std terms in shared memory, computes bias gradients with register tree reductions instead of a shared-memory row sweep, and skips the sqrt in grad-norm clipping when the squared norm is clearly below the threshold. This costs one extra pack launch and buffer per update, and adds template variants and code complexity.

```diff
diff --git a/include/omnisafe_amd.h b/include/omnisafe_amd.h
--- a/include/omnisafe_amd.h
+++ b/include/omnisafe_amd.h
@@ -162,6 +162,17 @@
                  const float* adv_r, const float* adv_c, const long* perm, long M, int B,
                  const float* lagrange, const osa_ppo_hparams* hp, int loss_kind, int nets_mask,
                  float* step_stats, const osa_surrogate_ext* ext, void* stream);
+int osa_pass_record_ld(int obs_dim, int act_dim);
+int osa_pack_pass_rows(int obs_dim, int act_dim, const float* obs, int ld_obs, const float* act, int ld_act,
+                       const float* logp, const float* adv_r, const float* adv_c, const float* target_value_r,
+                       const float* target_value_c, long M, float* rec, int ld_rec, void* stream);
+int osa_ppo_pass_packed(int obs_dim, int act_dim, int hidden, float* params, float* adam_m, float* adam_v,
+                        int* adam_step, const float* obs, int ld_obs, const float* act, int ld_act,
+                        const float* logp, const float* target_value_r, const float* target_value_c,
+                        const float* adv_r, const float* adv_c, const long* perm, long M, int B,
+                        const float* lagrange, const osa_ppo_hparams* hp, int loss_kind, int nets_mask,
+                        float* step_stats, const osa_surrogate_ext* ext, const float* rec, int ld_rec,
+                        void* stream);
 typedef struct osa_pass_member {
   float* params;
   float* adam_m;
diff --git a/omnisafe_amd/_lib.py b/omnisafe_amd/_lib.py
--- a/omnisafe_amd/_lib.py
+++ b/omnisafe_amd/_lib.py
@@ -103,6 +103,10 @@
                                    _P, _P, _I, _I, _P, _P, _I, _P, _P]),
     'osa_ppo_pass_ext': (_I, [_I, _I, _I, _P, _P, _P, _P, _P, _I, _P, _I, _P, _P, _P, _P, _P, _P, _L, _I,
                               _P, _P, _I, _I, _P, _P, _P]),
+    'osa_pass_record_ld': (_I, [_I, _I]),
+    'osa_pack_pass_rows': (_I, [_I, _I, _P, _I, _P, _I, _P, _P, _P, _P, _P, _L, _P, _I, _P]),
+    'osa_ppo_pass_packed': (_I, [_I, _I, _I, _P, _P, _P, _P, _P, _I, _P, _I, _P, _P, _P, _P, _P, _P, _L, _I,
+                                 _P, _P, _I, _I, _P, _P, _P, _I, _P]),
     'osa_ppo_pass_group_ws_bytes': (C.c_size_t, [_I]),
     'osa_ppo_pass_group': (_I, [_I, _I, _I, _P, _I, _P, C.c_size_t, _P]),
     'osa_adam_apply': (_I, [_I, _I, _I, _P, _P, _P, _P, _P, _P, _I, _P]),
diff --git a/omnisafe_amd/csrc/buffer_kernels.hip b/omnisafe_amd/csrc/buffer_kernels.hip
--- a/omnisafe_amd/csrc/buffer_kernels.hip
+++ b/omnisafe_amd/csrc/buffer_kernels.hip
@@ -774,6 +774,40 @@
     hipLaunchKernelGGL(osa_get_rows_kernel, dim3((unsigned)((total + 255) / 256)), dim3(256), 0, st, src, ld_src,
                        dst, ld_dst, T, N, dim);
   }
+}
+
+__global__ __launch_bounds__(256) void osa_pack_pass_rows_kernel(int obs_dim, int act_dim, const float* __restrict__ obs,
+                                                                 int ld_obs, const float* __restrict__ act, int ld_act,
+                                                                 const float* __restrict__ logp,
+                                                                 const float* __restrict__ adv_r,
+                                                                 const float* __restrict__ adv_c,
+                                                                 const float* __restrict__ tgt_r,
+                                                                 const float* __restrict__ tgt_c, long M,
+                                                                 float* __restrict__ rec, int ld_rec) {
+  const int nq = ld_rec / 4, oq = nq - 2;
+  const long gid = (long)blockIdx.x * 256 + threadIdx.x;
+  if (gid >= M * nq) return;
+  const long r = gid / nq;
+  const int q = (int)(gid - r * nq);
+  float4 v = {0.f, 0.f, 0.f, 0.f};
+  if (q < oq) {
+    const float* x = obs + r * ld_obs;
+    const int c = 4 * q;
+    v.x = x[c];
+    if (c + 1 < obs_dim) v.y = x[c + 1];
+    if (c + 2 < obs_dim) v.z = x[c + 2];
+    if (c + 3 < obs_dim) v.w = x[c + 3];
+  } else if (q == oq) {
+    v.x = act[r * ld_act];
+    if (act_dim > 1) v.y = act[r * ld_act + 1];
+    v.z = logp[r];
+    v.w = adv_r[r];
+  } else {
+    v.x = adv_c[r];
+    v.y = tgt_r[r];
+    v.z = tgt_c[r];
+  }
+  *reinterpret_cast<float4*>(rec + r * ld_rec + 4 * q) = v;
 }
 
 extern "C" {
@@ -952,6 +986,21 @@
   return OSA_OK;
 }
 
+int osa_pack_pass_rows(int obs_dim, int act_dim, const float* obs, int ld_obs, const float* act, int ld_act,
+                       const float* logp, const float* adv_r, const float* adv_c, const float* target_value_r,
+                       const float* target_value_c, long M, float* rec, int ld_rec, void* stream) {
+  OSA_REQUIRE(obs && act && logp && adv_r && adv_c && target_value_r && target_value_c && rec && M > 0);
+  OSA_REQUIRE(obs_dim >= 1 && ld_obs >= obs_dim && act_dim >= 1 && ld_act >= act_dim);
+  if (act_dim > 2) return OSA_EUNSUPPORTED;
+  OSA_REQUIRE(ld_rec == ((obs_dim + 3) & ~3) + 8 && (reinterpret_cast<uintptr_t>(rec) & 15) == 0);
+  const long quads = M * (ld_rec / 4);
+  hipLaunchKernelGGL(osa_pack_pass_rows_kernel, dim3((unsigned)((quads + 255) / 256)), dim3(256), 0,
+                     osa_stream(stream), obs_dim, act_dim, obs, ld_obs, act, ld_act, logp, adv_r, adv_c,
+                     target_value_r, target_value_c, M, rec, ld_rec);
+  OSA_CHECK_LAUNCH();
+  return OSA_OK;
+}
+
 int osa_buffer_get(int T, int N, int obs_dim, int act_dim, const float* obs, int ld_obs,
                    const float* act, int ld_act, const float* logp, const float* target_value_r,
                    const float* target_value_c, const float* adv_r, const float* adv_c,
diff --git a/omnisafe_amd/csrc/ppo_pass_body.h b/omnisafe_amd/csrc/ppo_pass_body.h
--- a/omnisafe_amd/csrc/ppo_pass_body.h
+++ b/omnisafe_amd/csrc/ppo_pass_body.h
@@ -56,6 +56,8 @@
   unsigned p2p_seq0;
   long long p2p_timeout;
   int p2p_fence;
+  const float* rec;
+  int ld_rec;
 };
 #define OSA_P2P_HDR 256
 #define OSA_P2P_STICKY 240
@@ -93,6 +95,12 @@
   asm volatile("global_store_dword %0, %1, off sc0 sc1" : : "v"(p), "v"(v) : "memory");
 }
 
+__device__ __forceinline__ void osa_put_ls_terms(float* t, int d, float ls, bool real) {
+  t[d] = __builtin_amdgcn_exp2f(ls * -2.88539008177792681472f);
+  t[2 + d] = -ls - 0.91893853320467274178f;
+  t[4 + d] = real ? 1.41893853320467274178f + ls : 0.f;
+}
+
 __host__ __device__ constexpr int osa_pass_lds_floats(int KB, int OT) {
   return 64 * (16 * KB + PSPAD) + 64 * PSLD + 16 * OT * PSLD + 2 * 64 + 2 * 16 * OT + 4 * 64 * PSLD + 16 * KB * PSLD +
          2 * 16 * OT * PSLD + 64;
@@ -104,10 +112,16 @@
   return OSA_PASS_W2T != 0 && (osa_pass_lds_floats(KB, OT) + 64 * PSLD) * 4 <= 160 * 1024;
 }
 
-template <int KB, int OT, bool MULTI, bool COOP, bool EXT, bool HIER, bool DPS, bool SO, bool P2P = false>
+template <int KB, int OT, bool MULTI, bool COOP, bool EXT, bool HIER, bool DPS, bool SO, bool P2P = false,
+          bool REC = false>
 __device__ __forceinline__ void osa_ppo_pass_body(const OsaPassArgs& a, const int net, const int rk, const int pc0 = 0,
                                                   const int pn = 0) {
   static_assert(!P2P || (COOP && !HIER && !DPS && !EXT), "P2P is a form of the cooperative pass");
+  constexpr bool FAST = SO && !MULTI && !COOP && !DPS;
+  static_assert(!REC || (FAST && !EXT), "packed records: plain single-chunk pass, small outputs, plain surrogate");
+  constexpr bool LS_TAB = FAST;
+  constexpr bool BIAS_REG = FAST;
+  constexpr bool CLIP_FAST = FAST;
   extern __shared__ __attribute__((aligned(16))) float smem[];
   const OsaNet& nd = a.nd;
   constexpr bool coop = COOP;
@@ -216,6 +230,9 @@
       sB3[tid] = gp[nd.ob3 + tid];
       sLS[tid] = gp[nd.oLS + tid];
     }
+    if constexpr (LS_TAB) {
+      if (tid < 2) osa_put_ls_terms(red + 16, tid, gp[nd.oLS + tid], tid < nd.act_dim);
+    }
   }
   OSA_PART_MARK(8);
   f32x4 m2[HT], v2[HT], m1[KB], v1[KB], m3[OT], v3[OT];
@@ -226,6 +243,14 @@
   else if (tid < 2 * H) { boff = nd.ob2 + tid - H; sbias = sB2 + tid - H; }
   else if (tid < 2 * H + OUTP) { boff = nd.ob3 + tid - 2 * H; sbias = sB3 + tid - 2 * H; }
   else if (tid < 2 * H + 2 * OUTP) { boff = nd.oLS + tid - 2 * H - OUTP; sbias = sLS + tid - 2 * H - OUTP; }
+  if constexpr (BIAS_REG) {
+    boff = -1;
+    sbias = sB1;
+    if (g == 0) { boff = nd.ob1 + 16 * wave + i; sbias = sB1 + 16 * wave + i; }
+    else if (g == 1) { boff = nd.ob2 + 16 * wave + i; sbias = sB2 + 16 * wave + i; }
+    else if (wave == 0 && g == 2) { boff = nd.ob3 + i; sbias = sB3 + i; }
+    else if (wave == 0) { boff = nd.oLS + i; sbias = sLS + i; }
+  }
   if (critic && boff >= nd.oLS) boff = -1;
 #pragma unroll
   for (int ti = 0; ti < HT; ++ti)
@@ -283,7 +308,19 @@
     float old[EXT ? 4 * OT : 1];
     bool valid;
   };
+  const int P4 = (nd.obs_dim + 3) & ~3;
+  const int rec_pair = P4 + 4 + (net == 2 ? 2 : 0);
   auto fetch_x = [&](long rr, Pre& q) {
+    if constexpr (REC) {
+      const float* xrow = a.rec + (int)rr * a.ld_rec;
+#pragma unroll
+      for (int kb = 0; kb < KB; ++kb) {
+        const int col0 = 16 * kb + 4 * g;
+        const int cl = (col0 + 4 <= P4) ? col0 : P4 - 4;
+        q.x[kb] = *reinterpret_cast<const f32x4*>(xrow + cl);
+      }
+      return;
+    }
     const float* xrow = obs_p + (int)rr * a.ld_obs;
 #pragma unroll
     for (int kb = 0; kb < KB; ++kb) {
@@ -302,6 +339,15 @@
   };
   auto fetch_s = [&](long rr, Pre& q) {
     const int ri = (int)rr;
+    if constexpr (REC) {
+      const float* srow = a.rec + ri * a.ld_rec;
+      const f32x4 s0 = *reinterpret_cast<const f32x4*>(srow + P4);
+      const float2 s1 = *reinterpret_cast<const float2*>(srow + rec_pair);
+      q.act[0] = s0.x; q.act[1] = s0.y; q.act[2] = 0.f; q.act[3] = 0.f;
+      q.logp = s0.z; q.adv_r = s0.w;
+      q.adv_c = s1.x; q.tgt = s1.y;
+      return;
+    }
     if (is_actor) {
       const float* arow = act_p + ri * a.ld_act;
 #pragma unroll
@@ -418,6 +464,11 @@
   }
 
   const float invB_full = 1.f / (float)a.B;
+  const float inv_act = 1.f / (float)nd.act_dim;
+  const float ent_grad = a.hp.entropy_coef / (float)nd.act_dim;
+  float clip_thr = 0.f;
+  if (CLIP_FAST && a.hp.max_grad_norm >= 1e-3f && a.hp.max_grad_norm <= 1e18f)
+    clip_thr = 0.99f * a.hp.max_grad_norm * a.hp.max_grad_norm;
   for (int mb = a.mb0; mb < a.mb0 + a.nmb; ++mb) {
     const long mb_lo = (long)mb * a.B;
     const int Bcur = (int)(min(mb_lo + a.B, a.M) - mb_lo);
@@ -434,9 +485,11 @@
     const float step_size = bc_row[0], inv_bc2_sqrt = bc_row[1];
     float gb = 0.f, loss_part = 0.f, ratio_part = 0.f, ent_pre = 0.f;
     float cost_pen = 0.f;
-    if (is_actor && leader) {
-      for (int d = 0; d < nd.act_dim; ++d) ent_pre += 1.41893853320467274178f + sLS[d];
-      ent_pre /= (float)nd.act_dim;
+    if constexpr (!LS_TAB) {
+      if (is_actor && leader) {
+        for (int d = 0; d < nd.act_dim; ++d) ent_pre += 1.41893853320467274178f + sLS[d];
+        ent_pre /= (float)nd.act_dim;
+      }
     }
     for (int ch = 0; ch < nchunk; ++ch, ++cidx) {
     PTICK(0);
@@ -530,6 +583,8 @@
     }
     PUT_TILE(sH2, h2[2], 2);
     PUT_TILE(sH2, h2[3], 3);
+    f32x4 lstab = {0.f, 0.f, 0.f, 0.f};
+    float2 lsent = {0.f, 0.f};
     if (small_out) {
       float p0 = 0.f, p1 = 0.f;
       f32x4 w0[HT], w1[HT];
@@ -537,6 +592,10 @@
       for (int t = 0; t < HT; ++t) {
         w0[t] = *reinterpret_cast<const f32x4*>(sW3 + 16 * t + 4 * g);
         w1[t] = *reinterpret_cast<const f32x4*>(sW3 + PSLD + 16 * t + 4 * g);
+      }
+      if constexpr (LS_TAB) {
+        lstab = *reinterpret_cast<const f32x4*>(red + 16);
+        lsent = *reinterpret_cast<const float2*>(red + 20);
       }
       __builtin_amdgcn_sched_barrier(0);
 #pragma unroll
@@ -565,6 +624,20 @@
     if (is_actor) {
       float lp = 0.f;
       f32x4 zv[OT], ivar[OT];
+      if constexpr (LS_TAB) {
+        zv[0] = (f32x4){0.f, 0.f, 0.f, 0.f};
+        ivar[0] = (f32x4){0.f, 0.f, 0.f, 0.f};
+#pragma unroll
+        for (int r = 0; r < 2; ++r) {
+          const float dmr = dm[0][r];
+          const float iv = lstab[r] * dmr;
+          const float z = cur.act[r] - out[0][r];
+          zv[0][r] = z;
+          ivar[0][r] = iv;
+          lp += -0.5f * (z * z) * iv + lstab[2 + r] * dmr;
+        }
+        ent_pre = (lsent.x + lsent.y) * inv_act;
+      } else {
 #pragma unroll
       for (int o = 0; o < OT; ++o) {
         const f32x4 ls = *reinterpret_cast<const f32x4*>(sLS + 16 * o + 4 * g);
@@ -577,6 +650,7 @@
           ivar[o][r] = iv;
           lp += -0.5f * (z * z) * iv - ls[r] * dmr - 0.91893853320467274178f * dmr;
         }
+      }
       }
       lp = osa_sum_over_groups(lp);
       float kl = 0.f, mask = 1.f, mask_mean = 1.f, cost_w = 0.f;
@@ -653,7 +727,7 @@
 #pragma unroll
         for (int o = 0; o < OT; ++o) {
 #pragma unroll
-          for (int r = 0; r < 4; ++r) {
+          for (int r = 0; r < (LS_TAB ? 2 : 4); ++r) {
             const float z = zv[o][r], iv = ivar[o][r];
             dO[o][r] = dlogp * z * iv;
             dLS[o][r] = dlogp * (z * z * iv - dm[o][r]);
@@ -665,7 +739,7 @@
         }
       }
     } else if (valid) {
-      const float diff = out[0][0] - cur.tgt;
+      const float diff = out[0][0] - ((REC && net == 2) ? cur.adv_c : cur.tgt);
       if (g == 0) {
         loss_part += diff * diff;
         dO[0][0] = 2.f * diff * invB;
@@ -783,11 +857,14 @@
       }
       if (small_out) {
         float q0 = 0.f, q1 = 0.f;
+        f32x4 do0[4], do1[4];
 #pragma unroll
         for (int k = 0; k < 4; ++k) {
           const f32x4 hv = *reinterpret_cast<const f32x4*>(sH2 + (16 * wave + i) * PSLD + 16 * g + 4 * k);
           const f32x4 a0 = *reinterpret_cast<const f32x4*>(sDO + 16 * g + 4 * k);
           const f32x4 a1 = *reinterpret_cast<const f32x4*>(sDO + PSLD + 16 * g + 4 * k);
+          do0[k] = a0;
+          do1[k] = a1;
 #pragma unroll
           for (int r = 0; r < 4; ++r) {
             q0 = fmaf(a0[r], hv[r], q0);
@@ -799,6 +876,25 @@
         if (g == 0) {
           g3[0][0] += q0;
           g3[0][1] += q1;
+        }
+        if constexpr (BIAS_REG) {
+          f32x4 dl0[4], dl1[4];
+#pragma unroll
+          for (int k = 0; k < 4; ++k) {
+            dl0[k] = *reinterpret_cast<const f32x4*>(sDL + 16 * g + 4 * k);
+            dl1[k] = *reinterpret_cast<const f32x4*>(sDL + PSLD + 16 * g + 4 * k);
+          }
+          auto tree = [](const f32x4 (&v)[4]) {
+            const f32x4 t = (v[0] + v[1]) + (v[2] + v[3]);
+            return (t.x + t.y) + (t.z + t.w);
+          };
+          const float s1 = osa_sum_over_groups(tree(a1)), s2 = osa_sum_over_groups(tree(a2));
+          const float t0 = osa_sum_over_groups(tree(do0)), t1 = osa_sum_over_groups(tree(do1));
+          const float u0 = osa_sum_over_groups(tree(dl0)), u1 = osa_sum_over_groups(tree(dl1));
+          const float s3 = (i == 0) ? t0 : ((i == 1) ? t1 : 0.f);
+          const float sl = (i == 0) ? u0 : ((i == 1) ? u1 : 0.f);
+          const float rs = (g == 0) ? s1 : ((g == 1) ? s2 : ((g == 2) ? s3 : sl));
+          gb = (boff >= 0) ? rs : 0.f;
         }
       } else {
 #pragma unroll
@@ -816,7 +912,7 @@
       }
     }
     PTICK(5);
-    {
+    if constexpr (!BIAS_REG) {
       const float* srow = (tid < H) ? sZ1 + tid * PSLD
                           : (tid < 2 * H) ? sZ2 + (tid - H) * PSLD
                           : (tid < 2 * H + OUTP) ? sDO + (tid - 2 * H) * PSLD
@@ -842,7 +938,7 @@
     OSA_PART_MARK(6);
     if (boff >= 0 && is_actor && boff >= nd.oLS && (boff - nd.oLS) < nd.act_dim && a.hp.entropy_coef != 0.f && own_terms &&
         !part)
-      gb -= a.hp.entropy_coef / (float)nd.act_dim;
+      gb -= ent_grad;
     f32x4 w2r[HT], w1r[KB], w3r[OT];
 #pragma unroll
     for (int ti = 0; ti < HT; ++ti)
@@ -934,11 +1030,18 @@
     const float t_psq = red[1] + red[5] + red[9] + red[13];
     const float t_loss = red[2] + red[6] + red[10] + red[14];
     const float t_ratio = red[3] + red[7] + red[11] + red[15];
-    const float total_norm = sqrtf(t_gsq);
-    float coef = 1.f;
-    if (a.hp.use_max_grad_norm) {
-      coef = a.hp.max_grad_norm / (total_norm + 1e-6f);
-      coef = coef > 1.f ? 1.f : coef;
+    float total_norm = 0.f, coef = 1.f;
+    if constexpr (CLIP_FAST) {
+      if (a.hp.use_max_grad_norm && !(t_gsq < clip_thr)) {
+        coef = a.hp.max_grad_norm / (sqrtf(t_gsq) + 1e-6f);
+        coef = coef > 1.f ? 1.f : coef;
+      }
+    } else {
+      total_norm = sqrtf(t_gsq);
+      if (a.hp.use_max_grad_norm) {
+        coef = a.hp.max_grad_norm / (total_norm + 1e-6f);
+        coef = coef > 1.f ? 1.f : coef;
+      }
     }
     if (dp) {
       float* __restrict__ slab = a.dp_slabs + ((long)net * a.dp_world + rk) * (P + PNSTAT);
@@ -1316,11 +1419,16 @@
         *sbias = nb;
         mb_ = mv_;
         vb_ = vv_;
+        if constexpr (LS_TAB) {
+          const int d = BIAS_REG ? tid - 48 : tid - (2 * H + OUTP);
+          if (is_actor && d >= 0 && d < 2) osa_put_ls_terms(red + 16, d, nb, d < nd.act_dim);
+        }
       }
     }
     PTICK(8);
     if (leader && (P2P || rk == 0)) {
       float* st = a.stats + (long)(mb - a.mb0) * PNSTAT;
+      if constexpr (CLIP_FAST) st_norm = sqrtf(t_gsq);
       if (is_actor) {
         st[2] = st_loss;
         st[3] = st_ratio;
diff --git a/omnisafe_amd/csrc/ppo_pass_kernel.hip b/omnisafe_amd/csrc/ppo_pass_kernel.hip
--- a/omnisafe_amd/csrc/ppo_pass_kernel.hip
+++ b/omnisafe_amd/csrc/ppo_pass_kernel.hip
@@ -1,6 +1,7 @@
 #include "ppo_pass_body.h"
 
-template <int KB, int OT, bool MULTI, bool COOP, bool EXT, bool HIER = false, bool DPS = false, bool SO = false>
+template <int KB, int OT, bool MULTI, bool COOP, bool EXT, bool HIER = false, bool DPS = false, bool SO = false,
+          bool REC = false>
 __global__ __launch_bounds__(256, 1) void osa_ppo_pass_kernel(OsaPassArgs a) {
   int net_ = blockIdx.x, rk_ = blockIdx.y;
   if constexpr (!COOP) {
@@ -18,7 +19,7 @@
   }
   const int net = net_, rk = rk_;
   if (!((a.nets_mask >> net) & 1)) return;
-  osa_ppo_pass_body<KB, OT, MULTI, COOP, EXT, HIER, DPS, SO>(a, net, rk);
+  osa_ppo_pass_body<KB, OT, MULTI, COOP, EXT, HIER, DPS, SO, false, REC>(a, net, rk);
 }
 
 static long long* g_osa_pass_dbg = nullptr;
@@ -26,10 +27,11 @@
 long long* osa_pass_dbg_ptr() { return g_osa_pass_dbg; }
 
 template <int KB, int OT, bool MULTI, bool COOP = false, bool EXT = false, bool HIER = false, bool DPS = false,
-          bool SO = false>
+          bool SO = false, bool REC = false>
 static int osa_launch_pass(const OsaPassArgs& a, hipStream_t stream, int grid_y = 1) {
   const dim3 grid = (COOP && a.dp_local == 1) ? dim3(8 * grid_y) : ((!COOP && a.one_xcc) ? dim3(17) : dim3(3, grid_y));
-  return osa_launch_pass_kernel<osa_ppo_pass_kernel<KB, OT, MULTI, COOP, EXT, HIER, DPS, SO>, COOP>(a, grid, stream);
+  return osa_launch_pass_kernel<osa_ppo_pass_kernel<KB, OT, MULTI, COOP, EXT, HIER, DPS, SO, REC>, COOP>(a, grid,
+                                                                                                         stream);
 }
 
 template <int KB, int OT, bool MULTI, bool COOP = false, bool EXT = false, bool HIER = false>
@@ -69,6 +71,22 @@
                  const float* adv_r, const float* adv_c, const long* perm, long M, int B,
                  const float* lagrange, const osa_ppo_hparams* hp, int loss_kind, int nets_mask,
                  float* step_stats, const osa_surrogate_ext* ext, void* stream) {
+  return osa_ppo_pass_packed(obs_dim, act_dim, hidden, params, adam_m, adam_v, adam_step, obs, ld_obs, act, ld_act,
+                             logp, target_value_r, target_value_c, adv_r, adv_c, perm, M, B, lagrange, hp, loss_kind,
+                             nets_mask, step_stats, ext, nullptr, 0, stream);
+}
+
+int osa_pass_record_ld(int obs_dim, int act_dim) {
+  return (obs_dim >= 1 && act_dim >= 1 && act_dim <= 2) ? ((obs_dim + 3) & ~3) + 8 : 0;
+}
+
+int osa_ppo_pass_packed(int obs_dim, int act_dim, int hidden, float* params, float* adam_m, float* adam_v,
+                        int* adam_step, const float* obs, int ld_obs, const float* act, int ld_act,
+                        const float* logp, const float* target_value_r, const float* target_value_c,
+                        const float* adv_r, const float* adv_c, const long* perm, long M, int B,
+                        const float* lagrange, const osa_ppo_hparams* hp, int loss_kind, int nets_mask,
+                        float* step_stats, const osa_surrogate_ext* ext, const float* rec, int ld_rec,
+                        void* stream) {
   if (!osa_ppo_pass_supported(obs_dim, act_dim, hidden)) return OSA_EUNSUPPORTED;
   OsaPassArgs a;
   bool extended = false;
@@ -83,6 +101,21 @@
   }
   const int KB = a.nd.KB, OT = a.nd.OUTP / 16;
   hipStream_t st = osa_stream(stream);
+  if (rec) {
+    if (extended || B > 64 || ld_rec != osa_pass_record_ld(obs_dim, act_dim)) return OSA_EUNSUPPORTED;
+    if ((reinterpret_cast<uintptr_t>(rec) & 15) != 0 || (double)M * ld_rec >= 2147483647.0) return OSA_EUNSUPPORTED;
+    const char* sw = getenv("OSA_PASS_PACKED");
+    const bool packed = !(sw && sw[0] == '0');
+    if (packed) {
+      a.rec = rec;
+      a.ld_rec = ld_rec;
+      return osa_pass_shapes(KB, OT, [&](auto K, auto O) {
+        if constexpr (decltype(O)::value == 1)
+          return osa_launch_pass<decltype(K)::value, 1, false, false, false, false, false, true, true>(a, st);
+        return (int)OSA_EUNSUPPORTED;
+      });
+    }
+  }
   if (extended)
     return osa_pass_shapes(KB, OT, [&](auto K, auto O) { return osa_launch_pass_so<K, O, false, false, true>(a, st); });
   return osa_pass_shapes(KB, OT, [&](auto K, auto O) {
diff --git a/omnisafe_amd/update.py b/omnisafe_amd/update.py
--- a/omnisafe_amd/update.py
+++ b/omnisafe_amd/update.py
@@ -65,6 +65,9 @@
         self.generator: torch.Generator | None = None
         self.pass_submit = None
         self.last_group = 0
+        self._rec_buf: torch.Tensor | None = None
+        self._rec_rows: torch.Tensor | None = None
+        self.last_packed = False
         self._graphed_pass = False
         self._use_wide = False
         self._split_xch: int | None = None
@@ -418,10 +421,29 @@
         if self.pass_submit is not None:
             self.last_group = int(self.pass_submit(self, self._pass_member(ops, lagrange, stats_rows)))
         else:
-            _lib.check(self.lib.osa_ppo_pass_ext(
+            rec = self._rec_rows
+            _lib.check(self.lib.osa_ppo_pass_packed(
                 *ops, _lib.ptr(lagrange), C.byref(self.hp), self.loss_kind, self._nets_mask(), _lib.ptr(stats_rows),
-                ext, _lib.stream_ptr()), 'osa_ppo_pass_ext')
+                ext, _lib.ptr(rec), 0 if rec is None else rec.stride(0), _lib.stream_ptr()), 'osa_ppo_pass_packed')
+            self.last_packed = rec is not None and os.environ.get('OSA_PASS_PACKED', '1')[:1] != '0'
         self._profile_end(ev, 'osa_ppo_pass_kernel', M)
+
+    def _pack_rows(self, data: dict) -> None:
+        ac, M = self.ac, data['obs'].shape[0]
+        ld = self.lib.osa_pass_record_ld(ac.obs_dim, ac.act_dim)
+        self._rec_rows = None
+        if (ld == 0 or self.batch_size > 64 or self.ext is not None or self.pass_submit is not None
+                or M * ld >= 2 ** 31):
+            return
+        if self._rec_buf is None or self._rec_buf.shape[0] < M or self._rec_buf.shape[1] != ld:
+            self._rec_buf = torch.empty(M, ld, dtype=torch.float32, device=ac.device)
+        rec = self._rec_buf[:M]
+        _lib.check(self.lib.osa_pack_pass_rows(
+            ac.obs_dim, ac.act_dim, _lib.ptr(data['obs']), data['obs'].stride(0), _lib.ptr(data['act']),
+            data['act'].stride(0), _lib.ptr(data['logp']), _lib.ptr(data['adv_r']), _lib.ptr(data['adv_c']),
+            _lib.ptr(data['target_value_r']), _lib.ptr(data['target_value_c']), M, _lib.ptr(rec), ld,
+            _lib.stream_ptr()), 'osa_pack_pass_rows')
+        self._rec_rows = rec
 
     def _pass_member(self, ops: tuple, lagrange: torch.Tensor, stats_rows: torch.Tensor) -> PassMember:
         m = PassMember()
@@ -838,6 +860,9 @@
         W = dist.world_size()
         if not self.general:
             data = self._aligned_rows(data)
+        self._rec_rows, self.last_packed = None, False
+        if use_pass and not self._use_wide:
+            self._pack_rows(data)
         use_p2p = dist.collectives_active() and self._p2p_ok(data) and self._p2p_setup()
         self._mode = 'allreduce' if self.dp_mode == 'p2p' else self.dp_mode
         use_repl = (dist.collectives_active() and not self.general and self.ext is None and self.update_critics
```

New measurement: 178,500, median of 6. No clear change (+0.4%).
